# terra-render/Terra

Hardware: AMD Instinct MI355X
Metric: Msamples/s (higher is better)
Workload: dtype f32; 1 GPU; cornell_1080p_512spp; scene=cornell32, width=1920, height=1080, spp=512, bounces=8, integrator=simple, triangles=32, tree=auto, traversal=reference tree + leaf-box cull, tile=64, sample_split=8, parallelism=single

## Files before the change

### include/terra_amd.h

```cpp
#ifndef TERRA_AMD_H
#define TERRA_AMD_H

#include "Terra.h"

#ifdef __cplusplus
extern "C" {
#endif

typedef enum {
    kTerraAmdOk               = 0,
    kTerraAmdErrNoDevice      = -1,
    kTerraAmdErrNotCommitted  = -2,
    kTerraAmdErrUnsupported   = -3,
    kTerraAmdErrBadArgument   = -4,
    kTerraAmdErrLaunch        = -5
} TerraAmdStatus;

const char* terra_amd_last_error ( void );
void        terra_amd_clear_error ( void );
int         terra_amd_first_error ( char* buf, size_t capacity );
void        terra_amd_clear_first_error ( void );
size_t      terra_amd_thread_staging_bytes ( void );

int  terra_amd_init ( void );
void terra_amd_set_commit_timing ( int on );
int  terra_amd_set_build_threads ( int threads );
void terra_amd_set_azimuth_table ( int on );

int  terra_amd_device_count ( void );
int  terra_amd_set_device ( int device );
int  terra_amd_get_device ( void );

int  terra_amd_set_devices ( const int* devices, int count );
int  terra_amd_get_devices ( int* out, int capacity );
int  terra_amd_shard_owner ( size_t tile_index, int world );
int  terra_amd_render_multi ( const TerraCamera* camera, HTerraScene scene, const TerraFramebuffer* framebuffer,
                              size_t x, size_t y, size_t width, size_t height, size_t tile_size );
typedef struct {
    int      devices;
    int      device[16];
    int      replicas;
    uint64_t gathers;
    uint64_t last_gather_bytes;
    uint64_t process_collectives;
    int      rccl_version;
    int      communicator_ranks;
    char     rccl_library[64];
    uint64_t rehearsed_gathers;
} TerraAmdMultiInfo;
int  terra_amd_multi_info ( HTerraScene scene, TerraAmdMultiInfo* out );
int  terra_amd_debug_replicas_share_device ( int on );

int  terra_amd_scene_supported ( HTerraScene scene, char* why, size_t capacity );

void     terra_amd_set_frame_seed ( HTerraScene scene, uint64_t seed );
uint64_t terra_amd_get_frame_seed ( HTerraScene scene );

int  terra_amd_set_tree_mode ( HTerraScene scene, int mode );
int  terra_amd_get_tree_mode ( HTerraScene scene );
typedef struct {
    int   tree_mode;
    int   fast_tree;
    int   fast_tree_built_on_device;
    int   leaf_cull;
    int   lds_resident;
    float max_coordinate;
    float max_coordinate_allowed;
    char  note[256];
    int   last_call;
    float camera_limit;
} TerraAmdTraversalInfo;
typedef enum {
    kTerraAmdCallNone = 0,
    kTerraAmdCallReplica = 1,
    kTerraAmdCallLeafCull = 2,
    kTerraAmdCallFastTree = 3,
    kTerraAmdCallFastTreeReach = 4
} TerraAmdCallTraversal;
int  terra_amd_traversal_info ( HTerraScene scene, TerraAmdTraversalInfo* out );
int  terra_amd_set_tree_builder ( HTerraScene scene, int builder );
int  terra_amd_get_tree_builder ( HTerraScene scene );
int  terra_amd_debug_shrink_reference_boxes ( HTerraScene scene, float amount );
int  terra_amd_debug_pad_stack ( HTerraScene scene, int entries );
int  terra_amd_debug_fast_stack_lds ( HTerraScene scene, int entries );

int  terra_amd_set_sample_split ( HTerraScene scene, int split );
int  terra_amd_get_sample_split ( HTerraScene scene );
int  terra_amd_auto_sample_split ( size_t width, size_t height, size_t tile, int world, size_t spp, int job_ordered );

int  terra_amd_set_job_order ( HTerraScene scene, int on );
int  terra_amd_get_job_order ( HTerraScene scene );

int  terra_amd_set_empty_skip ( HTerraScene scene, int on );
int  terra_amd_get_empty_skip ( HTerraScene scene );
int  terra_amd_empty_skip_info ( HTerraScene scene, uint32_t out[2] );
int  terra_amd_empty_proof ( const float* cam_rot9, const float* cam_pos3, float tan_half_fov, float aspect, float jitter, uint32_t fb_w, uint32_t fb_h,
                             uint32_t x0, uint32_t y0, uint32_t x1, uint32_t y1, const float* tris9, size_t n_tris );

int  terra_amd_set_leaf_box_test ( HTerraScene scene, int on );
int  terra_amd_get_leaf_box_test ( HTerraScene scene );
int  terra_amd_leaf_box_info ( HTerraScene scene, uint32_t out[2] );
int  terra_amd_set_leaf_pairs ( HTerraScene scene, int on );
int  terra_amd_get_leaf_pairs ( HTerraScene scene );
int  terra_amd_leaf_pair_info ( HTerraScene scene, uint32_t out[2] );
int  terra_amd_set_leaf_nearest_first ( HTerraScene scene, int on );
int  terra_amd_get_leaf_nearest_first ( HTerraScene scene );

int  terra_amd_set_environment_lighting ( HTerraScene scene, int on );
int  terra_amd_get_environment_lighting ( HTerraScene scene );

// ... 283 lines not shown
TERRA_ABI_ASSERT ( sizeof ( TerraAmdAtlasTexel ) == 16 );
TERRA_ABI_ASSERT ( offsetof ( TerraAmdAtlasTexel, wb ) == 4 );
TERRA_ABI_ASSERT ( offsetof ( TerraAmdAtlasTexel, distance2 ) == 12 );
int terra_amd_atlas_points_device ( HTerraScene scene, const TerraAmdAtlas* atlas, const void* d_uvs, void* d_points, void* d_texels, void* stream );
int terra_amd_atlas_points ( HTerraScene scene, const TerraAmdAtlas* atlas, const float* uvs, TerraAmdPoint* points, TerraAmdAtlasTexel* texels );
int terra_amd_dilate_device ( void* d_data, int channels, void* d_valid, int width, int height, int passes, void* stream );
int terra_amd_dilate ( float* data, int channels, int* valid, int width, int height, int passes );

typedef struct {
    float c[9][3];
    int   cells;
} TerraAmdProbeSH;
typedef struct {
    float origin[3];
    int   nx;
    float spacing[3];
    int   ny, nz;
    int   reserved[3];
} TerraAmdProbeGrid;
TERRA_ABI_ASSERT ( sizeof ( TerraAmdProbeSH ) == 112 );
TERRA_ABI_ASSERT ( offsetof ( TerraAmdProbeSH, cells ) == 108 );
TERRA_ABI_ASSERT ( sizeof ( TerraAmdProbeGrid ) == 48 );
TERRA_ABI_ASSERT ( offsetof ( TerraAmdProbeGrid, nx ) == 12 );
TERRA_ABI_ASSERT ( offsetof ( TerraAmdProbeGrid, spacing ) == 16 );
TERRA_ABI_ASSERT ( offsetof ( TerraAmdProbeGrid, ny ) == 28 );
TERRA_ABI_ASSERT ( offsetof ( TerraAmdProbeGrid, nz ) == 32 );
TERRA_ABI_ASSERT ( offsetof ( TerraAmdProbeGrid, reserved ) == 36 );
int terra_amd_probe_rays_device ( const void* d_probes, size_t probes, int cells, const void* d_jitter, void* d_rays, void* stream );
int terra_amd_probe_rays ( const TerraAmdPoint* probes, size_t probes_n, int cells, const float* jitter, TerraAmdRay* rays );
int terra_amd_sh_project_device ( const void* d_results, const void* d_rays, size_t probes, int cells, int batch, void* d_sh, void* stream );
int terra_amd_sh_project ( const TerraFramebuffer* framebuffer, const TerraAmdRay* rays, size_t probes, int cells, int batch, TerraAmdProbeSH* sh );
int terra_amd_sh_irradiance_device ( const void* d_sh, size_t probes, const TerraAmdProbeGrid* grid, const void* d_points, const void* d_index, size_t n, void* d_out, void* stream );
int terra_amd_sh_irradiance ( const TerraAmdProbeSH* sh, size_t probes, const TerraAmdProbeGrid* grid, const TerraAmdPoint* points, const int* index, size_t n, float* out4 );
int terra_amd_probe_grid_points ( const TerraAmdProbeGrid* grid, TerraAmdPoint* out, int capacity );

int terra_amd_render_device_sharded ( const TerraCamera* camera, HTerraScene scene,
                                      void* d_pixels, void* d_results, size_t fb_width, size_t fb_height,
                                      size_t x, size_t y, size_t width, size_t height,
                                      size_t tile_size, int rank, int world,
                                      void* d_rand_calls, void* stream );

int    terra_amd_shard_tile_count ( size_t width, size_t height, size_t tile_size, int rank, int world );
size_t terra_amd_shard_packed_bytes ( size_t width, size_t height, size_t tile_size, int world );
int terra_amd_pack_tiles ( const void* d_pixels, const void* d_results, size_t fb_width, size_t fb_height,
                           size_t x, size_t y, size_t width, size_t height, size_t tile_size, int rank, int world,
                           void* d_packed, void* stream );
int terra_amd_unpack_tiles ( void* d_pixels, void* d_results, size_t fb_width, size_t fb_height,
                             size_t x, size_t y, size_t width, size_t height, size_t tile_size, int rank, int world,
                             const void* d_packed, void* stream );

int terra_amd_synchronize ( void* stream );

int terra_amd_time_render_device ( const TerraCamera* camera, HTerraScene scene,
                                   void* d_pixels, void* d_results, size_t fb_width, size_t fb_height,
                                   size_t x, size_t y, size_t width, size_t height,
                                   int launches, void* stream, float* ms_avg );


int terra_amd_unit_pcg ( const uint32_t* seeds, int nseeds, int n, float* out );
int terra_amd_unit_stream_keys ( uint64_t frame_seed, const uint64_t* pix, const uint64_t* samples_so_far, int n, uint64_t* out3 );
int terra_amd_unit_ray_aabb ( int n, const float* origins3, const float* dirs3, const float* boxes6, int* hit, float* tmin, float* tmax );
int terra_amd_unit_watertight ( int n, const float* origins3, const float* dirs3, const float* tris9, int* hit, float* out8 );
int terra_amd_unit_watertight_pair ( int n, const float* origins3, const float* dirs3, const float* quads12, int* hit2, float* depth2 );
int terra_amd_unit_moller_trumbore ( int n, const float* origins3, const float* dirs3, const float* tris9, int* hit, float* out4 );
int terra_amd_unit_bvh_traverse ( HTerraScene scene, int n, const float* origins3, const float* dirs3, int* found, uint32_t* prim, float* point3 );
int terra_amd_unit_bvh_traverse_fast ( HTerraScene scene, int n, const float* origins3, const float* dirs3, int* found, uint32_t* prim, float* point3, uint32_t* nodes_visited );
int terra_amd_unit_raycast ( HTerraScene scene, int n, const float* origins3, const float* dirs3, int* obj, int* tri, float* point3, float* surface47 );
int terra_amd_unit_trace ( HTerraScene scene, int n, const float* origins3, const float* dirs3, const uint64_t* stateB, const uint64_t* incB, float* radiance3, uint32_t* rand_calls );
int terra_amd_unit_bsdf ( int kind, int n, float* surfaces47, const float* e3, const float* wo3, float* wi3, float* pdf, float* f3 );
int terra_amd_unit_camera ( const TerraCamera* camera, size_t fb_width, size_t fb_height, int n, const uint32_t* xy2, float jitter, const float* r2, float* dirs3 );
int terra_amd_unit_tonemap ( int op, float gamma, int n, float* colors3 );
int terra_amd_unit_math ( int fn, int n, const float* x, const float* y, float* out );
int terra_amd_scene_lds_plan ( HTerraScene scene, uint32_t* out6 );
int terra_amd_unit_exact_div ( int op, const float* a, const float* b, const float* c, uint64_t first, uint64_t count, float denominator, float reciprocal, uint64_t seed,
                               uint32_t* helper_bits, uint32_t* plain_bits, uint64_t* mismatches, uint32_t* first_bad );
int terra_amd_unit_exact_sqrt ( int op, const float* a, const float* b, const float* c, uint64_t first, uint64_t count, uint64_t seed,
                                uint32_t* helper_bits, uint32_t* plain_bits, uint64_t* mismatches, uint32_t* first_bad );
int terra_amd_unit_half_outward ( const double* x, int n, int up, uint16_t* out );
int terra_amd_unit_stratified ( const uint32_t* seeds, int nseeds, int strata, int samples_per_stratum, int n, float* out2 );
int terra_amd_unit_halton ( int first, int n, float* out2 );
int terra_amd_unit_distribution_1d ( const float* f, size_t n, const float* e, int m, float* x, float* pdf, uint32_t* idx, float* cdf_out, float* integral_out );
int terra_amd_unit_distribution_2d ( const float* f, size_t nx, size_t ny, const float* e12, int m, float* xy2, float* pdf, float* marginal_cdf_out );
int terra_amd_unit_distribution_2d_pdf ( const float* f, size_t nx, size_t ny, const float* xy2, int m, float* pdf );
int terra_amd_unit_texture_sample ( const TerraTexture* texture, int n, const float* uv2, float* out3 );
int terra_amd_unit_texture_latlong ( const TerraTexture* texture, int n, const float* dir3, float* out3 );

#ifdef __cplusplus
}
#endif
#endif
```

### terra_amd/csrc/dev_math.h

```cpp
#pragma once
#include <stdint.h>
#include <math.h>

#if defined(__HIPCC__)
#define TDM_FN __host__ __device__ inline
#else
#define TDM_FN static inline
#endif

TDM_FN uint32_t tdm_bits ( float f ) { return __builtin_bit_cast ( uint32_t, f ); }
TDM_FN float    tdm_float ( uint32_t u ) { return __builtin_bit_cast ( float, u ); }
TDM_FN uint32_t tdm_top12 ( float f ) { return ( tdm_bits ( f ) >> 20 ) & 0x7ffu; }

TDM_FN float tdm_sincos_poly ( double x, double x2, int n, bool flip ) {
    if ( ( n & 1 ) == 0 ) {
        const double S1 = -0x1.555545995a603p-3, S2 = 0x1.1107605230bc4p-7, S3 = -0x1.994eb3774cf24p-13;
        double x3 = x * x2;
        double t = S2 + x2 * S3;
        double x7 = x3 * x2;
        double s = x + x3 * S1;
        return ( float ) ( s + x7 * t );
    }
    double k = flip ? -1.0 : 1.0;
    const double C0 = 0x1p0, C1 = -0x1.ffffffd0c621cp-2, C2 = 0x1.55553e1068f19p-5, C3 = -0x1.6c087e89a359dp-10, C4 = 0x1.99343027bf8c3p-16;
    double x4 = x2 * x2;
    double t2 = ( k * C3 ) + x2 * ( k * C4 );
    double t1 = ( k * C0 ) + x2 * ( k * C1 );
    double x6 = x4 * x2;
    double c = t1 + x4 * ( k * C2 );
    return ( float ) ( c + x6 * t2 );
}

TDM_FN float tdm_sincosf ( float y, int shift ) {
    double x = y;
    if ( tdm_top12 ( y ) < tdm_top12 ( 0x1.921FB6p-1f ) ) {
        if ( tdm_top12 ( y ) < tdm_top12 ( 0x1p-12f ) ) {
            return shift ? 1.0f : y;
        }
        return tdm_sincos_poly ( x, x * x, shift, false );
    }
    double r = x * 0x1.45F306DC9C883p+23;
    int n = ( ( int32_t ) r + 0x800000 ) >> 24;
    x = x - ( double ) n * 0x1.921FB54442D18p0;
    int m = n + shift;
    int q = m & 3;
    double sgn = ( q == 1 || q == 2 ) ? -1.0 : 1.0;
    return tdm_sincos_poly ( x * sgn, x * x, m, ( m & 2 ) != 0 );
}
TDM_FN void tdm_sincosf_pair ( float y, float& s, float& c ) {
    double x = y;
    if ( tdm_top12 ( y ) < tdm_top12 ( 0x1.921FB6p-1f ) ) {
        if ( tdm_top12 ( y ) < tdm_top12 ( 0x1p-12f ) ) { s = y; c = 1.0f; return; }
        double x2 = x * x;
        s = tdm_sincos_poly ( x, x2, 0, false );
        c = tdm_sincos_poly ( x, x2, 1, false );
        return;
    }
    double r = x * 0x1.45F306DC9C883p+23;
    int n = ( ( int32_t ) r + 0x800000 ) >> 24;
    x = x - ( double ) n * 0x1.921FB54442D18p0;
    double x2 = x * x;
    int qs = n & 3, m = n + 1, qc = m & 3;
    double sgn_s = ( qs == 1 || qs == 2 ) ? -1.0 : 1.0;
    double sgn_c = ( qc == 1 || qc == 2 ) ? -1.0 : 1.0;
    s = tdm_sincos_poly ( x * sgn_s, x2, n, ( n & 2 ) != 0 );
    c = tdm_sincos_poly ( x * sgn_c, x2, m, ( m & 2 ) != 0 );
}
TDM_FN float tdm_sinf ( float y ) { return tdm_sincosf ( y, 0 ); }
TDM_FN float tdm_cosf ( float y ) { return tdm_sincosf ( y, 1 ); }

TDM_FN uint64_t tdm_bits64 ( double f ) { return __builtin_bit_cast ( uint64_t, f ); }
TDM_FN double   tdm_double ( uint64_t u ) { return __builtin_bit_cast ( double, u ); }

TDM_FN double tdm_powf_log2 ( uint32_t ix ) {
    static const double T[16][2] = {
        { 0x1.661ec79f8f3bep+0, -0x1.efec65b963019p-2 }, { 0x1.571ed4aaf883dp+0, -0x1.b0b6832d4fca4p-2 },
        { 0x1.49539f0f010bp+0, -0x1.7418b0a1fb77bp-2 }, { 0x1.3c995b0b80385p+0, -0x1.39de91a6dcf7bp-2 },
        { 0x1.30d190c8864a5p+0, -0x1.01d9bf3f2b631p-2 }, { 0x1.25e227b0b8eap+0, -0x1.97c1d1b3b7afp-3 },
        { 0x1.1bb4a4a1a343fp+0, -0x1.2f9e393af3c9fp-3 }, { 0x1.12358f08ae5bap+0, -0x1.960cbbf788d5cp-4 },
        { 0x1.0953f419900a7p+0, -0x1.a6f9db6475fcep-5 }, { 0x1p+0, 0x0p+0 },
        { 0x1.e608cfd9a47acp-1, 0x1.338ca9f24f53dp-4 }, { 0x1.ca4b31f026aap-1, 0x1.476a9543891bap-3 },
        { 0x1.b2036576afce6p-1, 0x1.e840b4ac4e4d2p-3 }, { 0x1.9c2d163a1aa2dp-1, 0x1.40645f0c6651cp-2 },
        { 0x1.886e6037841edp-1, 0x1.88e9c2c1b9ff8p-2 }, { 0x1.767dcf5534862p-1, 0x1.ce0a44eb17bccp-2 } };
    const double A0 = 0x1.27616c9496e0bp-2, A1 = -0x1.71969a075c67ap-2, A2 = 0x1.ec70a6ca7baddp-2, A3 = -0x1.7154748bef6c8p-1, A4 = 0x1.71547652ab82bp0;
    uint32_t tmp = ix - 0x3f330000u;
    int i = ( int ) ( ( tmp >> 19 ) % 16u );
    uint32_t top = tmp & 0xff800000u;
    uint32_t iz = ix - top;
    int k = ( int32_t ) top >> 23;
    double z = ( double ) tdm_float ( iz );
    double r = z * T[i][0] - 1.0;
    double y0 = T[i][1] + ( double ) k;
    double r2 = r * r;
    double y = A0 * r + A1;
    double p = A2 * r + A3;
    double r4 = r2 * r2;
    double q = A4 * r + y0;
    q = p * r2 + q;
    return y * r4 + q;
}
TDM_FN float tdm_powf_exp2 ( double xd, uint32_t sign_bias ) {
    static const uint64_t T[32] = {
        0x3ff0000000000000ull, 0x3fefd9b0d3158574ull, 0x3fefb5586cf9890full, 0x3fef9301d0125b51ull,
        0x3fef72b83c7d517bull, 0x3fef54873168b9aaull, 0x3fef387a6e756238ull, 0x3fef1e9df51fdee1ull,
        0x3fef06fe0a31b715ull, 0x3feef1a7373aa9cbull, 0x3feedea64c123422ull, 0x3feece086061892dull,
        0x3feebfdad5362a27ull, 0x3feeb42b569d4f82ull, 0x3feeab07dd485429ull, 0x3feea47eb03a5585ull,
        0x3feea09e667f3bcdull, 0x3fee9f75e8ec5f74ull, 0x3feea11473eb0187ull, 0x3feea589994cce13ull,
        0x3feeace5422aa0dbull, 0x3feeb737b0cdc5e5ull, 0x3feec49182a3f090ull, 0x3feed503b23e255dull,
        0x3feee89f995ad3adull, 0x3feeff76f2fb5e47ull, 0x3fef199bdd85529cull, 0x3fef3720dcef9069ull,
        0x3fef5818dcfba487ull, 0x3fef7c97337b9b5full, 0x3fefa4afa2a490daull, 0x3fefd0765b6e4540ull };
    const double C0 = 0x1.c6af84b912394p-5, C1 = 0x1.ebfce50fac4f3p-3, C2 = 0x1.62e42ff0c52d6p-1, SHIFT = 0x1.8p+47;
    double kd = xd + SHIFT;
    uint64_t ki = tdm_bits64 ( kd );
    kd = kd - SHIFT;
    double r = xd - kd;
    uint64_t t = T[ki % 32u];
    uint64_t ski = ki + sign_bias;
    t += ski << 47;
    double s = tdm_double ( t );
    double z = C0 * r + C1;
    double r2 = r * r;
    double y = C2 * r + 1.0;
    y = z * r2 + y;
    y = y * s;
    return ( float ) y;
}
TDM_FN int tdm_powf_checkint ( uint32_t iy ) {
    int e = ( int ) ( iy >> 23 & 0xff );
    if ( e < 0x7f ) return 0;
    if ( e > 0x7f + 23 ) return 2;
    if ( iy & ( ( 1u << ( 0x7f + 23 - e ) ) - 1 ) ) return 0;
    if ( iy & ( 1u << ( 0x7f + 23 - e ) ) ) return 1;
    return 2;
}
TDM_FN bool tdm_zeroinfnan ( uint32_t ix ) { return 2 * ix - 1 >= 2u * 0x7f800000u - 1; }

TDM_FN float tdm_powf ( float x, float y ) {
    uint32_t sign_bias = 0;
    uint32_t ix = tdm_bits ( x ), iy = tdm_bits ( y );
    if ( ix - 0x00800000u >= 0x7f800000u - 0x00800000u || tdm_zeroinfnan ( iy ) ) {
        if ( tdm_zeroinfnan ( iy ) ) {
            if ( 2 * iy == 0 ) return 1.0f;
            if ( ix == 0x3f800000u ) return 1.0f;
            if ( 2 * ix > 2u * 0x7f800000u || 2 * iy > 2u * 0x7f800000u ) return x + y;
            if ( 2 * ix == 2 * 0x3f800000u ) return 1.0f;
            if ( ( 2 * ix < 2 * 0x3f800000u ) == ! ( iy & 0x80000000u ) ) return 0.0f;
            return y * y;
        }
        if ( tdm_zeroinfnan ( ix ) ) {
            float x2 = x * x;
            if ( ( ix & 0x80000000u ) && tdm_powf_checkint ( iy ) == 1 ) x2 = -x2;
            return ( iy & 0x80000000u ) ? 1 / x2 : x2;
// ... 118 lines not shown
```

### terra_amd/csrc/integrators_device.h

```cpp
#pragma once
#include "shading_device.h"

TD float randf ( Pcg32& b, Counters& c, int count ) { if ( count == 2 ) ++c.rand_calls; return trng_b_float ( b ); }
TD uint32_t randf_bits ( Pcg32& b, Counters& c, int count ) { if ( count == 2 ) ++c.rand_calls; return trng_b_bits ( b ); }

TD float triangle_area ( V3 a, V3 b, V3 cc ) { return length ( cross ( b - a, cc - a ) ) / 2; }

struct LightSample { uint32_t light_object; uint32_t tri_in_object; uint32_t tri; float pick_pdf; V3 pos, norm; };

template <int COUNT, int MODE = 0>
TD LightSample draw_light_sample ( const DevScene& sc, Pcg32& rb, Counters& c, const Tracer* T = nullptr ) {
    LightSample ls;
    float e = ( float ) ( ( double ) randf ( rb, c, COUNT ) - 1e-4 );
    double xl = ( double ) e * ( double ) sc.n_lights;
    uint32_t li = xl < 0 ? 0u : ( uint32_t ) xl;
    ls.pick_pdf = 1.f / ( float ) sc.lights_triangles_count;
    DevLight l = ( MODE == 1 && T ) ? T->l_lights[li] : sc.lights[li];
    float e_t = randf ( rb, c, COUNT );
    uint32_t k = ( uint32_t ) ( e_t * ( float ) l.tri_count );
    if ( k >= l.tri_count ) k = l.tri_count - 1;
    ls.light_object = l.object; ls.tri_in_object = k; ls.tri = l.first_tri + k;
    float e1 = randf ( rb, c, COUNT ), e2 = randf ( rb, c, COUNT );
    const float4* tris = ( MODE == 1 && T ) ? reinterpret_cast<const float4*> ( T->l_tris ) : reinterpret_cast<const float4*> ( sc.tris );
    const float4* props = ( MODE == 1 && T ) ? T->l_props : reinterpret_cast<const float4*> ( sc.props );
// ... 46 lines not shown
    float p_row = 0.f, p_col = 0.f; uint32_t row = 0, col = 0;
    DevDistribution1D rows = { sc.env_row_f, sc.env_row_cdf, sc.env_ny, sc.env_integral, sc.env_monotone };
    const float sv = distribution_sample ( rows, e1, &p_row, &row );
    if ( sv == FLT_MAX ) return zero;
    DevDistribution1D cols = { sc.env_f + ( size_t ) sc.env_nx * row, sc.env_cdf + ( size_t ) sc.env_nx * row, sc.env_nx, sc.env_row_f[row], sc.env_monotone };
    const float su = distribution_sample ( cols, e2, &p_col, &col );
    if ( su == FLT_MAX ) return zero;
    const float theta = sv * TERRA_PI_F, phi = su * ( 2 * TERRA_PI_F ) - TERRA_PI_F;
    const float st = tdm_sinf ( theta ), ct = tdm_cosf ( theta ), sp = tdm_sinf ( phi ), cp = tdm_cosf ( phi );
    if ( ! ( st > 0.f ) ) return zero;
    const V3 wi = v3 ( st * cp, ct, st * sp );
    const float cosine = dot ( wi, sf.normal );
    if ( ! ( cosine > 0.f ) ) return zero;
    const float pdf = ( p_row * p_col ) * ( ( float ) sc.env_nx * ( float ) sc.env_ny ) / ( 2 * TERRA_PI_F * TERRA_PI_F * st );
    if ( ! ( pdf > 0.f ) ) return zero;
    Surface lsf;
    Ray r = surface_ray ( sf, p, wi );
    RaycastResult h = scene_raycast<COUNT, MODE, KINDS> ( T, r, lsf, c );
    if ( h.hit ) return zero;
    const V3 L = texture_read ( sc.textures[sc.env_tex], col, row );
    const V3 f = bsdf_eval<KINDS> ( sf, wi, wo );
    if constexpr ( MIS && ( KINDS & TERRA_KIND_ENV_MIS ) != 0 ) if ( !bsdf_is_singular<KINDS> ( sf ) ) {
        const float b = bsdf_pdf<KINDS> ( sf, wi, wo ), bpdf = b > 0.f ? b : 0.f;
        const float r = bpdf / pdf, weight = 1.f / ( 1.f + r * r );
        return had ( L, f ) * ( cosine * weight / pdf );
    }
    return had ( L, f ) * ( cosine / pdf );
}

template <int COUNT, int MODE, int KINDS>
TD V3 integrate_direct ( const Tracer& T, Surface& sf, V3 p, V3 wo, V3 throughput, uint32_t bounce, Pcg32& rb, Counters& c ) {
    const DevScene& sc = T.sc;
    V3 Lo = v3 ( 0, 0, 0 );
    if ( bounce == 0 && dot ( wo, sf.normal ) > 0 ) Lo = Lo + sf.emissive;
    LightSample ls = draw_light_sample<COUNT, MODE> ( sc, rb, c, &T );
    V3 p_to_light = ls.pos - p;
    V3 wi = normalize ( p_to_light );
    Surface lsf;
    Ray r = surface_ray ( sf, p, wi );
    RaycastResult h = scene_raycast<COUNT, MODE, KINDS> ( T, r, lsf, c );
    if ( h.hit && h.object == ls.light_object && h.tri_in_object == ls.tri_in_object ) {
        float cosv = dot ( neg ( wi ), ls.norm );
        if ( cosv > 0 ) {
            V3 f = bsdf_eval<KINDS> ( sf, wi, wo );
            float pdf = dot ( p_to_light, p_to_light ) / fabsf ( cosv * T.l_area[h.tri] );
            V3 Ld = had ( lsf.emissive, f );
            Ld = Ld * ( dot ( wi, sf.normal ) / ( pdf * ls.pick_pdf ) );
            Lo = Lo + Ld;
        }
    }
    if constexpr ( ( KINDS & TERRA_KIND_SAMPLER ) != 0 ) { if ( env_sampling_active ( sc ) ) Lo = Lo + environment_light_sample<COUNT, MODE, KINDS> ( T, sf, p, wo, rb, c ); }
    return had ( Lo, throughput );
}

struct DirectPending { V3 vis, hid; uint32_t expected; };
template <int COUNT, int KINDS, int MODE = 0>
TD DirectPending direct_prepare ( const Tracer& T, Surface& sf, V3 p, V3 wo, V3 throughput, uint32_t bounce, Pcg32& rb, Counters& c, Ray& shadow_ray ) {
    const DevScene& sc = T.sc;
    V3 Lo = v3 ( 0, 0, 0 );
    if ( bounce == 0 && dot ( wo, sf.normal ) > 0 ) Lo = Lo + sf.emissive;
    LightSample ls = draw_light_sample<COUNT, MODE> ( sc, rb, c, &T );
    V3 p_to_light = ls.pos - p;
    V3 wi = normalize ( p_to_light );
    shadow_ray = surface_ray ( sf, p, wi );
    DirectPending d;
    d.hid = had ( Lo, throughput ); d.vis = d.hid; d.expected = ls.tri;
    float cosv = dot ( neg ( wi ), ls.norm );
    if ( cosv > 0 ) {
        V3 f = bsdf_eval<KINDS> ( sf, wi, wo );
        float pdf = dot ( p_to_light, p_to_light ) / fabsf ( cosv * T.l_area[ls.tri] );
        V3 Ld = had ( v3p ( T.l_mats[ls.light_object].emissive ), f );
        Ld = Ld * ( dot ( wi, sf.normal ) / ( pdf * ls.pick_pdf ) );
        d.vis = had ( Lo + Ld, throughput );
    }
    return d;
}

struct MisPending { V3 a_vis, a_hid; uint32_t expected; V3 f2; float bpdf2, cos2; V3 p; uint32_t light_object; V3 t_before; };
template <int COUNT, int KINDS, int MODE = 0>
TD MisPending mis_prepare ( const Tracer& T, Surface& sf, V3 p, V3 wo, V3 throughput, uint32_t bounce, Pcg32& rb, Counters& c, Ray& ray_a, V3& dir_b ) {
    const DevScene& sc = T.sc;
    V3 Lo = v3 ( 0, 0, 0 );
    if ( bounce == 0 && dot ( wo, sf.normal ) > 0 ) Lo = Lo + sf.emissive;
    float e1 = randf ( rb, c, COUNT ), e2 = randf ( rb, c, COUNT ), e3 = randf ( rb, c, COUNT );
    V3 bsdf_dir = bsdf_sample<KINDS> ( sf, e1, e2, e3, wo, azimuth_fetch ( sc.sincos24, e2 ) );
    LightSample ls = draw_light_sample<COUNT, MODE> ( sc, rb, c, &T );
    MisPending m;
    m.a_hid = Lo; m.a_vis = Lo; m.expected = ls.tri; m.p = p; m.light_object = ls.light_object; m.t_before = throughput;
    {
        V3 p_to_light = ls.pos - p;
        V3 wi = normalize ( p_to_light );
        ray_a = surface_ray ( sf, p, wi );
        float cosv = dot ( ls.norm, neg ( wi ) );
        if ( cosv > 0 ) {
            float bpdf = bsdf_pdf<KINDS> ( sf, wi, wo );
            float lpdf = dot ( p_to_light, p_to_light ) / fabsf ( cosv * T.l_area[ls.tri] );
            float weight = ( lpdf * lpdf ) / ( lpdf * lpdf + bpdf * bpdf );
            if ( lpdf != 0 ) {
                V3 f = bsdf_eval<KINDS> ( sf, wi, wo );
                V3 L = had ( v3p ( T.l_mats[ls.light_object].emissive ), f );
                L = L * ( dot ( wi, sf.normal ) * weight / ( lpdf * ls.pick_pdf ) );
                m.a_vis = Lo + L;
            }
        }
    }
    dir_b = bsdf_dir;
    m.f2 = bsdf_eval<KINDS> ( sf, bsdf_dir, wo );
    m.bpdf2 = bsdf_pdf<KINDS> ( sf, bsdf_dir, wo );
    m.cos2 = dot ( bsdf_dir, sf.normal );
    return m;
}
template <int MODE>
TD V3 mis_finish_b ( const Tracer& T, const MisPending& m, V3 Lo, bool hit, uint32_t hit_object, uint32_t hit_tri, V3 hit_point, const Surface& lsf, V3 wi ) {
    if ( hit && hit_object == m.light_object ) {
        float NoW = dot ( lsf.normal, neg ( wi ) );
        if ( NoW > 0 ) {
            V3 dl = m.p - hit_point;
            float dist = dot ( dl, dl );
            const float4* tris = MODE == 1 ? reinterpret_cast<const float4*> ( T.l_tris ) : reinterpret_cast<const float4*> ( T.sc.tris );
            V3 ta, tb, tc; tri_vertices ( tris, hit_tri, ta, tb, tc );
            float area = triangle_area ( ta, tb, tc );
            float lpdf = dist / ( NoW * area );
            float weight = ( m.bpdf2 * m.bpdf2 ) / ( lpdf * lpdf + m.bpdf2 * m.bpdf2 );
            if ( m.bpdf2 != 0 ) {
                V3 L = had ( lsf.emissive, m.f2 );
                L = L * ( m.cos2 * weight / m.bpdf2 );
                Lo = Lo + L;
            }
        }
    }
    return had ( Lo, m.t_before );
}

template <int COUNT, int MODE, int KINDS, bool DEBUG_WEIGHTS>
TD V3 integrate_mis ( const Tracer& T, Surface& sf, V3 p, V3 wo, V3 throughput, uint32_t bounce, Pcg32& rb, Counters& c ) {
    const DevScene& sc = T.sc;
    V3 Lo = v3 ( 0, 0, 0 );
    if ( DEBUG_WEIGHTS ) { if ( bounce != 0 ) return Lo; }
    else if ( bounce == 0 && dot ( wo, sf.normal ) > 0 ) Lo = Lo + sf.emissive;
    float e1 = randf ( rb, c, COUNT ), e2 = randf ( rb, c, COUNT ), e3 = randf ( rb, c, COUNT );
    V3 bsdf_dir = bsdf_sample<KINDS> ( sf, e1, e2, e3, wo, azimuth_fetch ( sc.sincos24, e2 ) );
    LightSample ls = draw_light_sample<COUNT, MODE> ( sc, rb, c, &T );
    {
        V3 p_to_light = ls.pos - p;
        V3 wi = normalize ( p_to_light );
        Surface lsf;
        Ray r = surface_ray ( sf, p, wi );
        RaycastResult h = scene_raycast<COUNT, MODE, KINDS> ( T, r, lsf, c );
        if ( h.hit && h.object == ls.light_object && h.tri_in_object == ls.tri_in_object ) {
            float cosv = dot ( ls.norm, neg ( wi ) );
            if ( cosv > 0 ) {
                float bpdf = bsdf_pdf<KINDS> ( sf, wi, wo );
                float lpdf = dot ( p_to_light, p_to_light ) / fabsf ( cosv * T.l_area[h.tri] );
                if ( DEBUG_WEIGHTS ) {
                    float weight = ( bpdf * bpdf ) / ( lpdf * lpdf + bpdf * bpdf );
                    Lo = Lo + v3 ( 0, 0, weight );
                } else {
                    float weight = ( lpdf * lpdf ) / ( lpdf * lpdf + bpdf * bpdf );
                    if ( lpdf != 0 ) {
                        V3 f = bsdf_eval<KINDS> ( sf, wi, wo );
                        V3 L = had ( lsf.emissive, f );
                        L = L * ( dot ( wi, sf.normal ) * weight / ( lpdf * ls.pick_pdf ) );
                        Lo = Lo + L;
                    }
                }
            }
        }
    }
    {
        V3 wi = bsdf_dir;
        V3 f = bsdf_eval<KINDS> ( sf, wi, wo );
        float bpdf = bsdf_pdf<KINDS> ( sf, wi, wo );
        V3 light_wo = neg ( wi );
        Surface lsf;
        Ray r = surface_ray ( sf, p, wi );
        RaycastResult h = scene_raycast<COUNT, MODE, KINDS> ( T, r, lsf, c );
        if ( h.hit && h.object == ls.light_object ) {
            float NoW = dot ( lsf.normal, light_wo );
            if ( NoW > 0 ) {
                V3 dl = p - h.point;
                float dist = dot ( dl, dl );
                const float4* tris = reinterpret_cast<const float4*> ( sc.tris );
                V3 ta, tb, tc; tri_vertices ( tris, h.tri, ta, tb, tc );
                float area = triangle_area ( ta, tb, tc );
                float lpdf = dist / ( NoW * area );
                float weight = ( bpdf * bpdf ) / ( lpdf * lpdf + bpdf * bpdf );
                if ( DEBUG_WEIGHTS ) {
                    Lo = Lo + v3 ( weight, 0, 0 );
                } else if ( bpdf != 0 ) {
                    V3 L = had ( lsf.emissive, f );
                    L = L * ( dot ( wi, sf.normal ) * weight / bpdf );
                    Lo = Lo + L;
                }
            }
        }
        if constexpr ( ( KINDS & TERRA_KIND_ENV_MIS ) != 0 && !DEBUG_WEIGHTS ) {
            if ( !h.hit && bpdf > 0.f ) {
                uint32_t col, row; float st;
                environment_texel ( sc, wi, col, row, st );
                const float epdf = ( !bsdf_is_singular<KINDS> ( sf ) && dot ( wi, sf.normal ) > 0 ) ? environment_texel_pdf ( sc, col, row, st ) : 0.f;
                const float r = epdf / bpdf, weight = 1.f / ( 1.f + r * r );
                V3 L = had ( texture_read ( sc.textures[sc.env_tex], col, row ), f );
                L = L * ( dot ( wi, sf.normal ) * weight / bpdf );
                Lo = Lo + L;
            }
        }
    }
    if constexpr ( ( KINDS & TERRA_KIND_SAMPLER ) != 0 && !DEBUG_WEIGHTS ) { if ( env_sampling_active ( sc ) ) Lo = Lo + environment_light_sample<COUNT, MODE, KINDS, true> ( T, sf, p, wo, rb, c ); }
    return had ( Lo, throughput );
}

TD V3 integrate_debug_normals ( const Surface& sf, uint32_t bounce ) {
    if ( bounce != 0 ) return v3 ( 0, 0, 0 );
    V3 n = sf.normal;
    V3 pp = v3 ( sel_min ( n.x > 0 ? n.x : 0.f, 1.f ), sel_min ( n.y > 0 ? n.y : 0.f, 1.f ), sel_min ( n.z > 0 ? n.z : 0.f, 1.f ) );
    V3 nn = v3 ( sel_min ( n.x > -1 ? n.x : -1.f, 0.f ), sel_min ( n.y > -1 ? n.y : -1.f, 0.f ), sel_min ( n.z > -1 ? n.z : -1.f, 0.f ) );
    nn = nn * -1.f;
    V3 col = v3 ( 0, 0, 0 );
    col = col + v3 ( 1, 0, 0 ) * pp.x;
    col = col + v3 ( 0, 1, 0 ) * pp.y;
    col = col + v3 ( 0, 0, 1 ) * pp.z;
    col = col + v3 ( 0, 1, 1 ) * nn.x;
    col = col + v3 ( 1, 0, 1 ) * nn.y;
    col = col + v3 ( 1, 1, 0 ) * nn.z;
    return col;
}

template <int INTEGRATOR, int COUNT, int MODE, int KINDS>
TD V3 integrate ( const Tracer& T, const Ray& ray, Surface& sf, V3 p, V3 wo, V3 throughput, uint32_t bounce, Pcg32& rb, Counters& c ) {
    if ( INTEGRATOR == 0 ) {
        if ( dot ( wo, sf.normal ) > 0 ) return had ( sf.emissive, throughput );
        return v3 ( 0, 0, 0 );
    } else if ( INTEGRATOR == 1 ) {
        return integrate_direct<COUNT, MODE, KINDS> ( T, sf, p, wo, throughput, bounce, rb, c );
    } else if ( INTEGRATOR == 2 ) {
        return integrate_mis<COUNT, MODE, KINDS, false> ( T, sf, p, wo, throughput, bounce, rb, c );
    } else if ( INTEGRATOR == 3 ) {
        return bounce != 0 ? v3 ( 0, 0, 0 ) : v3 ( 1, 1, 1 );
    } else if ( INTEGRATOR == 4 ) {
        if ( bounce != 0 ) return v3 ( 0, 0, 0 );
        float d = length ( ray.o - p ) / 500.f;
        return v3 ( d, d, d );
    } else if ( INTEGRATOR == 5 ) {
        return integrate_debug_normals ( sf, bounce );
    } else {
        return integrate_mis<COUNT, MODE, KINDS, true> ( T, sf, p, wo, throughput, bounce, rb, c );
    }
}

template <int COUNT, bool INDEX>
TD PathDraws path_draw ( const float2* sincos24, Pcg32& rb, Counters& c ) {
    PathDraws d;
    if constexpr ( INDEX ) {
        d.e0 = randf ( rb, c, COUNT );
        const uint32_t k1 = randf_bits ( rb, c, COUNT );
        d.e1 = trng_b_from_bits ( k1 );
        d.e2 = randf ( rb, c, COUNT );
        d.az = azimuth_fetch_index ( sincos24, k1 );
        d.e3 = randf ( rb, c, COUNT );
    } else {
        d.e0 = randf ( rb, c, COUNT ); d.e1 = randf ( rb, c, COUNT ); d.e2 = randf ( rb, c, COUNT );
        d.az = azimuth_fetch ( sincos24, d.e1 );
        d.e3 = randf ( rb, c, COUNT );
    }
    return d;
}
template <int KINDS>
TD bool path_continue ( Surface& sf, V3 wo, V3& throughput, uint32_t& bounce, uint32_t max_bounces, const PathDraws& d, V3& wi ) {
    wi = bsdf_sample<KINDS> ( sf, d.e0, d.e1, d.e2, wo, d.az );
    float pdf = sel_max ( bsdf_pdf<KINDS> ( sf, wi, wo ), ( float ) 1e-4 );
    V3 f = bsdf_eval<KINDS> ( sf, wi, wo ) * rcp_exact ( pdf );
    throughput = had ( throughput, f );
    throughput = throughput * dot ( sf.normal, wi );
    float pr = sel_max ( throughput.x, sel_max ( throughput.y, throughput.z ) );
    if ( d.e3 > pr ) return false;
        throughput = throughput * roulette_scale ( pr );
    ++bounce;
    return bounce <= max_bounces;
}
struct SamplerPair { float u0, u1; bool on; };
TD SamplerPair sampler_pair_none() { SamplerPair s; s.u0 = s.u1 = 0.f; s.on = false; return s; }
TD void path_apply_sampler ( PathDraws& d, const SamplerPair& sp, uint32_t bounce ) {
    if ( sp.on && bounce == 0 ) { d.e0 = sp.u0; d.e1 = sp.u1; d.az = azimuth_none(); }
}
TD SamplerPair sampler_pair_draw ( uint32_t mode, uint32_t strata, uint64_t n, Pcg32& stream_a ) {
    SamplerPair s = sampler_pair_none();
    if ( mode == 1 ) { s.u0 = radical_inverse ( 3, n ); s.u1 = radical_inverse ( 2, n ); s.on = true; }
    else if ( mode == 2 && strata > 0 ) {
        const uint64_t cap = ( uint64_t ) strata * strata * 16ull, m = n % cap, stratum = m / 16ull;
        const float stratum_size = 1.f / ( float ) strata;
        s.u0 = sd_below_one ( ( ( float ) ( uint32_t ) ( stratum % strata ) + trng_a_float ( stream_a ) ) * stratum_size );
        s.u1 = sd_below_one ( ( ( float ) ( uint32_t ) ( stratum / strata ) + trng_a_float ( stream_a ) ) * stratum_size );
        s.on = true;
    }
    return s;
}
template <int COUNT, int KINDS>
TD bool path_continue ( const DevScene& sc, Surface& sf, V3 wo, V3& throughput, uint32_t& bounce, uint32_t max_bounces, Pcg32& rb, Counters& c, V3& wi, const SamplerPair& sp = sampler_pair_none() ) {
    PathDraws d = path_draw<COUNT> ( sc.sincos24, rb, c );
    if ( KINDS & TERRA_KIND_SAMPLER ) path_apply_sampler ( d, sp, bounce );
    return path_continue<KINDS> ( sf, wo, throughput, bounce, max_bounces, d, wi );
}

template <int INTEGRATOR, int COUNT, int MODE, int KINDS>
TD V3 trace_path ( const Tracer& T, Ray ray, uint32_t bounces, Pcg32& rb, Counters& c ) {
    V3 Lo = v3 ( 0, 0, 0 ), throughput = v3 ( 1, 1, 1 );
    for ( uint32_t bounce = 0; bounce <= bounces; ++bounce ) {
        Surface sf;
        RaycastResult h = scene_raycast<COUNT, MODE, KINDS> ( T, ray, sf, c );
        if ( !h.hit ) {
            if ( ( KINDS & TERRA_KIND_ENV ) && T.sc.env_mode && !env_reaches_by_samples<INTEGRATOR, KINDS> ( T.sc, bounce ) ) { throughput = had ( throughput, environment_eval ( T.sc, ray.d ) ); Lo = Lo + throughput; }
            break;
        }
        V3 wo = neg ( ray.d );
        Lo = Lo + integrate<INTEGRATOR, COUNT, MODE, KINDS> ( T, ray, sf, h.point, wo, throughput, bounce, rb, c );
        V3 wi;
        uint32_t next_bounce = bounce;
        if ( !path_continue<COUNT, KINDS> ( T.sc, sf, wo, throughput, next_bounce, bounces, rb, c, wi ) ) break;
        ray = surface_ray ( sf, h.point, wi );
    }
    return Lo;
}

TD V3 uncharted2 ( V3 x ) {
    const float A = 0.15f, B = 0.5f, C = 0.1f, D = 0.2f, E = 0.02f, F = 0.3f;
    V3 r;
    r.x = ( ( x.x * ( A * x.x + C * B ) + D * E ) / ( x.x * ( A * x.x + B ) + D * F ) ) - E / F;
    r.y = ( ( x.y * ( A * x.y + C * B ) + D * E ) / ( x.y * ( A * x.y + B ) + D * F ) ) - E / F;
    r.z = ( ( x.z * ( A * x.z + C * B ) + D * E ) / ( x.z * ( A * x.z + B ) + D * F ) ) - E / F;
    return r;
}
TD V3 powv ( V3 c, float e ) { return v3 ( tdm_powf ( c.x, e ), tdm_powf ( c.y, e ), tdm_powf ( c.z, e ) ); }
TD V3 tonemap ( V3 c, int op, float gamma ) {
    switch ( op ) {
        case 1: c = powv ( c, 1.f / gamma ); break;
        case 2:
            c.x = c.x / ( 1.f + c.x ); c.y = c.y / ( 1.f + c.y ); c.z = c.z / ( 1.f + c.z );
            c = powv ( c, 1.f / gamma ); break;
        case 3: {
            V3 x = v3 ( sel_max ( 0.f, c.x - 0.004f ), sel_max ( 0.f, c.y - 0.004f ), sel_max ( 0.f, c.z - 0.004f ) );
            c.x = ( x.x * ( 6.2f * x.x + 0.5f ) ) / ( x.x * ( 6.2f * x.x + 1.7f ) + 0.06f );
            c.y = ( x.y * ( 6.2f * x.y + 0.5f ) ) / ( x.y * ( 6.2f * x.y + 1.7f ) + 0.06f );
            c.x = ( x.z * ( 6.2f * x.z + 0.5f ) ) / ( x.z * ( 6.2f * x.z + 1.7f ) + 0.06f );
            break;
        }
        case 4: {
            V3 ws = uncharted2 ( v3 ( 11.2f, 11.2f, 11.2f ) );
// ... 10 lines not shown
```

### terra_amd/csrc/kernels.h

```cpp
#pragma once
#include <hip/hip_runtime.h>
#include "dev_types.h"

hipError_t terra_launch_render ( const DevRenderParams& p, hipStream_t stream );
hipError_t terra_launch_job_streams ( const DevRenderParams& p, hipStream_t stream );
hipError_t terra_launch_block_order ( const DevRenderParams& p, uint32_t* cls, hipStream_t stream, const DevLaunchMask* mask, bool classify, bool prove );
hipError_t terra_launch_render_mode0 ( const DevRenderParams& p, size_t lds, hipStream_t stream );
hipError_t terra_launch_render_mode1 ( const DevRenderParams& p, size_t lds, hipStream_t stream );
hipError_t terra_launch_render_mode2 ( const DevRenderParams& p, size_t lds, hipStream_t stream );
hipError_t terra_launch_render_mode3 ( const DevRenderParams& p, size_t lds, hipStream_t stream );
hipError_t terra_launch_render_rays ( const DevRenderParams& p, const void* rays, hipStream_t stream );
hipError_t terra_launch_render_rays_mode0 ( const DevRayRenderParams& p, size_t lds, hipStream_t stream );
hipError_t terra_launch_render_rays_mode1 ( const DevRayRenderParams& p, size_t lds, hipStream_t stream );
hipError_t terra_launch_render_rays_mode2 ( const DevRayRenderParams& p, size_t lds, hipStream_t stream );
hipError_t terra_launch_render_rays_mode3 ( const DevRayRenderParams& p, size_t lds, hipStream_t stream );
hipError_t terra_launch_render_lens ( const DevRenderParams& p, const DevLens& lens, hipStream_t stream );
hipError_t terra_launch_render_lens_mode0 ( const DevLensRenderParams& p, size_t lds, hipStream_t stream );
hipError_t terra_launch_render_lens_mode1 ( const DevLensRenderParams& p, size_t lds, hipStream_t stream );
hipError_t terra_launch_render_lens_mode2 ( const DevLensRenderParams& p, size_t lds, hipStream_t stream );
hipError_t terra_launch_render_lens_mode3 ( const DevLensRenderParams& p, size_t lds, hipStream_t stream );
hipError_t terra_launch_render_points ( const DevRenderParams& p, const void* points, const DevPointSampling& sampling, hipStream_t stream );
hipError_t terra_launch_render_points_mode0 ( const DevPointRenderParams& p, size_t lds, hipStream_t stream );
hipError_t terra_launch_render_points_mode1 ( const DevPointRenderParams& p, size_t lds, hipStream_t stream );
hipError_t terra_launch_render_points_mode2 ( const DevPointRenderParams& p, size_t lds, hipStream_t stream );
hipError_t terra_launch_render_points_mode3 ( const DevPointRenderParams& p, size_t lds, hipStream_t stream );
hipError_t terra_launch_resolve ( const DevRenderParams& p, hipStream_t stream, const uint32_t* live_blocks );
hipError_t terra_launch_tiles ( bool pack, float* pixels, void* results, uint32_t fb_w, uint32_t x, uint32_t y, uint32_t w, uint32_t h,
                                uint32_t tile, uint32_t rank, uint32_t world, float* packed, hipStream_t stream );

hipError_t terra_launch_aov ( DevRenderParams p, void* aov, hipStream_t stream, const uint32_t* mask );
hipError_t terra_launch_aov_rays ( DevRenderParams p, const void* rays, void* aov, hipStream_t stream );
hipError_t terra_launch_aov_lens ( DevRenderParams p, const DevLens& lens, void* aov, hipStream_t stream );
hipError_t terra_launch_aov_points ( DevRenderParams p, const void* points, const DevPointSampling& sampling, void* aov, hipStream_t stream );

hipError_t terra_launch_denoise ( const void* results, const void* aov, uint32_t fb_w, uint32_t x, uint32_t y, uint32_t w, uint32_t h, int iterations,
                                  float exposure, int op, float gamma, float* radiance, float* pixels, hipStream_t stream );
hipError_t terra_launch_denoise_variance ( const void* results, const void* aov, const void* moments, uint32_t fb_w, uint32_t x, uint32_t y, uint32_t w, uint32_t h, int iterations,
                                           float exposure, int op, float gamma, float* radiance, float* pixels, hipStream_t stream );

hipError_t terra_launch_moments_accumulate ( const void* results, void* moments, uint32_t fb_w, uint32_t x, uint32_t y, uint32_t w, uint32_t h, hipStream_t stream );
hipError_t terra_launch_tile_error ( const void* moments, uint32_t fb_w, uint32_t x, uint32_t y, uint32_t w, uint32_t h, uint32_t tile, float* errors, hipStream_t stream );
hipError_t terra_launch_error_mask ( const float* errors, uint32_t w, uint32_t h, uint32_t tile, float target, int all, uint32_t* mask, hipStream_t stream );

struct DevTemporalParams {
    float cam_pos[3], cam_rot[9], tan_half_fov, aspect;
    float prev_pos[3], prev_rot[9], prev_tan_half_fov;
    uint32_t fb_w, fb_h, x, y, w, h;
    float alpha, depth_tolerance, normal_cos, max_length;
    uint32_t same_camera;
    float inv_fb_w, inv_fb_h;
};
hipError_t terra_launch_temporal_reproject ( const DevTemporalParams& p, const void* results, const void* aov, const void* history_in, void* history_out,
                                             void* out_results, void* out_moments, hipStream_t stream );

struct DevQueryParams {
    DevScene scene;
    uint32_t fast, stack_depth, leaf_cap, spill_cap, leaf_cull;
    float    origin_limit;
};
hipError_t terra_launch_query ( DevQueryParams p, const void* rays, size_t n, void* out, bool anyhit, hipStream_t stream );

struct DevAtlas {
    uint32_t width, height;
    float    uv_scale[2], uv_offset[2], margin;
};
hipError_t terra_launch_atlas_points ( const DevScene& sc, const DevAtlas& atlas, const float* uvs, void* points, void* texels, hipStream_t stream );
hipError_t terra_launch_dilate ( float* data, int channels, int* valid, uint32_t width, uint32_t height, int passes, hipStream_t stream );

struct DevProbeGrid {
    int32_t on;
    int32_t count[3];
    float   origin[3], spacing[3];
};
hipError_t terra_launch_probe_rays ( const void* probes, uint32_t count, uint32_t cells, const float* jitter, void* rays, hipStream_t stream );
hipError_t terra_launch_sh_project ( const void* results, const void* rays, uint32_t count, uint32_t cells, int batch, void* sh, hipStream_t stream );
hipError_t terra_launch_sh_irradiance ( const void* sh, uint32_t probes, const DevProbeGrid& grid, const void* points, const int* index, uint32_t n, void* out, hipStream_t stream );

hipError_t terra_fill_sincos24 ( float2* table, hipStream_t stream );

hipError_t terra_unit_pcg ( const uint32_t* seeds, int nseeds, int n, float* out );
hipError_t terra_unit_stream_keys ( uint64_t frame_seed, const uint64_t* pix, const uint64_t* k, int n, uint64_t* out3 );
hipError_t terra_unit_ray_aabb ( int n, const float* o, const float* d, const float* boxes, int* hit, float* tmin, float* tmax );
hipError_t terra_unit_watertight ( int n, const float* o, const float* d, const float* tris, int* hit, float* out8 );
hipError_t terra_unit_watertight_pair ( int n, const float* o, const float* d, const float* quads, int* hit, float* depth );
hipError_t terra_unit_moller_trumbore ( int n, const float* o, const float* d, const float* tris, int* hit, float* out4 );
hipError_t terra_unit_bvh_traverse ( const DevScene& sc, int n, const float* o, const float* d, int* found, uint32_t* prim, float* point );
hipError_t terra_unit_bvh_traverse_fast ( const DevScene& sc, int n, const float* o, const float* d, int* found, uint32_t* prim, float* point, uint32_t* nodes_visited );
hipError_t terra_unit_raycast ( const DevScene& sc, int n, const float* o, const float* d, int* obj, int* tri, float* point, float* surface47 );
hipError_t terra_unit_trace ( const DevScene& sc, int integrator, uint32_t bounces, int n, const float* o, const float* d,
                              const uint64_t* stateB, const uint64_t* incB, float* radiance, uint32_t* rand_calls );
hipError_t terra_unit_bsdf ( int kind, int n, float* surfaces47, const float* e3, const float* wo3, float* wi3, float* pdf, float* f3 );
hipError_t terra_unit_camera ( const DevRenderParams& p, int n, const uint32_t* xy2, const float* r2, float* dirs3 );
hipError_t terra_unit_lens_rays ( const DevRenderParams& p, const DevLens& lens, int n, const uint32_t* xy2, const float* r4, float* rays8 );
hipError_t terra_unit_point_rays ( const DevPointSampling& sampling, int n, const float* points8, const float* g2, float* rays8 );
hipError_t terra_unit_tonemap ( int op, float gamma, int n, float* colors3 );
hipError_t terra_unit_math ( int fn, int n, const float* x, const float* y, float* out );
hipError_t terra_unit_exact_div ( int op, const float* a, const float* b, const float* c, uint64_t first, uint64_t count, float D, float R, uint64_t seed,
                                  uint32_t* helper_bits, uint32_t* plain_bits, unsigned long long* mismatches, uint32_t* first_bad );
hipError_t terra_unit_exact_sqrt ( int op, const float* a, const float* b, const float* c, uint64_t first, uint64_t count, uint64_t seed,
                                   uint32_t* helper_bits, uint32_t* plain_bits, unsigned long long* mismatches, uint32_t* first_bad );
hipError_t terra_unit_texture_sample ( const DevTexture* t, int n, const float* uv2, float* out3 );
hipError_t terra_unit_texture_latlong ( const DevTexture* t, int n, const float* dir3, float* out3 );
hipError_t terra_unit_stratified ( const uint32_t* seeds, int nseeds, int strata, int samples, int n, float* out2 );
hipError_t terra_unit_halton ( int first, int n, float* out2 );
hipError_t terra_unit_distribution_1d ( const float* f, uint32_t n, float* cdf, float* integral, uint32_t* monotone, const float* e, int m, float* x, float* pdf, uint32_t* idx );
hipError_t terra_unit_distribution_2d ( const float* f, uint32_t nx, uint32_t ny, float* cdf, float* integrals, float* mcdf, uint32_t* monotone, const float* e12, int m, float* xy2, float* pdf );
hipError_t terra_unit_distribution_2d_pdf ( const float* f, uint32_t nx, uint32_t ny, float* cdf, float* integrals, float* mcdf, uint32_t* monotone, const float* xy2, int m, float* pdf );
hipError_t terra_build_fast_tree_device ( const DevTri* tris, const uint32_t* rank, uint32_t n, float extra_margin, DevNode* out_nodes, DevTri* out_tris, uint32_t* n_nodes_out, int* max_stack_out, hipStream_t stream );
```

### terra_amd/csrc/render_kernels.hip

```cpp
#include <hip/hip_runtime.h>
#include "trace_device.h"
#include "kernels.h"
#include "launch_plan.h"
#include "empty_proof.h"

#ifdef TERRA_TU
#define TERRA_TU_HAS(k) ( TERRA_TU == ( k ) )
#define TERRA_TU_MODE(k) ( TERRA_TU == ( k ) || TERRA_TU == ( k ) + 4 || TERRA_TU == ( k ) + 8 || TERRA_TU == ( k ) + 12 )
#else
#define TERRA_TU_HAS(k) ( !TERRA_RAY_SOURCE )
#define TERRA_TU_MODE(k) 1
#endif
#if TERRA_RAY_SOURCE == 3
typedef DevPointRenderParams RenderKernelParams;
#elif TERRA_RAY_SOURCE == 2
typedef DevLensRenderParams RenderKernelParams;
#elif TERRA_RAY_SOURCE == 1
typedef DevRayRenderParams RenderKernelParams;
#else
typedef DevRenderParams RenderKernelParams;
#endif

struct DevResult { float acc[3]; int samples; };

// ... 489 lines not shown
                        cont = path_continue<COUNT, KINDS> ( T.sc, sf, wo, throughput, bounce, p.bounces, rs.b, c, cont_d, sp );
                        cont_o = surface_origin ( sf, point );
                        ro = ray_a.o; rd = ray_a.d; job = 1; start = true;
                    } else {
                        if ( ( KINDS & TERRA_KIND_ENV ) && T.sc.env_mode ) { throughput = had ( throughput, environment_eval ( T.sc, ray.d ) ); Lo = Lo + throughput; }
                        deposit ( acc_lds, Lo ); have_ray = false;
                    }
                }
                if ( !start ) {
                    if ( jb.s == p.chunk_spp ) { TERRA_JOB_NEXT(); if ( jb.exhausted ) done = true; }
                    if ( jb.s != p.chunk_spp ) {
                        float r1 = trng_a_float ( rs.a ), r2 = trng_a_float ( rs.a );
                        TERRA_PRIMARY_RAY ( ro, rd, r1, r2 );
                        if constexpr ( ( KINDS & TERRA_KIND_SAMPLER ) != 0 ) sp = sampler_pair_draw ( p.sampler_mode, p.sampler_strata, ( uint64_t ) jb.base + jb.s, rs.a );
                        TERRA_LENS_RAY ( ro, rd, r1, r2 );
                        Lo = v3 ( 0, 0, 0 ); throughput = v3 ( 1, 1, 1 ); bounce = 0; ++jb.s; job = 0; start = true;
                    }
                }
                if ( start ) { ray = make_ray ( ro, rd ); lane_traversal_start<COUNT, MODE> ( T, ray, lt, c ); have_ray = true; }
            }
            if ( !lane_traversal_run<COUNT, MODE> ( T, ray, lt, c ) && __all ( done ) ) break;
        }
    } else if constexpr ( terra_decoupled_direct ( INTEGRATOR, MODE, KINDS ) ) {
        LaneTraversal lt = lane_traversal_idle ( T, ray );
        bool done = false, have_ray = false, shadow = false, cont = false;
        DirectPending pend; pend.vis = pend.hid = v3 ( 0, 0, 0 ); pend.expected = 0;
        V3 cont_o = v3 ( 0, 0, 0 ), cont_d = v3 ( 0, 0, 1 );
        for ( ;; ) {
            if ( !lt.traversing && !done && ! ( have_ray && lane_traversal_recheck<MODE> ( T, ray, lt ) ) ) {
                bool start = false;
                V3 ro = v3 ( 0, 0, 0 ), rd = v3 ( 0, 0, 1 );
                if ( have_ray && shadow ) {
                    const uint32_t tri_s = ( MODE == 2 && COUNT == 0 && lt.best.tri == TERRA_TRI_EXPECTED ) ? pend.expected : hit_soup_index<MODE> ( T, lt.best.tri );
                    if ( tri_s != 0xffffffffu ) {
                        if ( COUNT ) ++c.hits;
                        if ( COUNT == 2 ) { const float4 t0 = reinterpret_cast<const float4*> ( T.sc.tris ) [3 * tri_s]; c.attr_fetches += T.sc.mats[__float_as_uint ( t0.w )].attributes_count + 1; }
                    }
                    Lo = Lo + ( tri_s == pend.expected ? pend.vis : pend.hid );
                    shadow = false;
                    if ( cont ) { ro = cont_o; rd = cont_d; start = true; }
                    else { deposit ( acc_lds, Lo ); have_ray = false; }
                } else if ( have_ray ) {
                    if ( lt.best.tri != 0xffffffffu ) {
                        Surface sf;
                        V3 point = shade_surface<COUNT, MODE, KINDS> ( T, ray, lt.best, sf, c );
                        V3 wo = neg ( ray.d );
                        Ray shadow_ray;
                        pend = direct_prepare<COUNT, KINDS, MODE> ( T, sf, point, wo, throughput, bounce, rs.b, c, shadow_ray );
                        cont = path_continue<COUNT, KINDS> ( T.sc, sf, wo, throughput, bounce, p.bounces, rs.b, c, cont_d, sp );
                        cont_o = surface_origin ( sf, point );
                        ro = shadow_ray.o; rd = shadow_ray.d; shadow = true; start = true;
                    } else {
                        if ( ( KINDS & TERRA_KIND_ENV ) && T.sc.env_mode ) { throughput = had ( throughput, environment_eval ( T.sc, ray.d ) ); Lo = Lo + throughput; }
                        deposit ( acc_lds, Lo ); have_ray = false;
                    }
                }
                if ( !start ) {
                    if ( jb.s == p.chunk_spp ) { TERRA_JOB_NEXT(); if ( jb.exhausted ) done = true; }
                    if ( jb.s != p.chunk_spp ) {
                        float r1 = trng_a_float ( rs.a ), r2 = trng_a_float ( rs.a );
                        TERRA_PRIMARY_RAY ( ro, rd, r1, r2 );
                        if constexpr ( ( KINDS & TERRA_KIND_SAMPLER ) != 0 ) sp = sampler_pair_draw ( p.sampler_mode, p.sampler_strata, ( uint64_t ) jb.base + jb.s, rs.a );
                        TERRA_LENS_RAY ( ro, rd, r1, r2 );
                        Lo = v3 ( 0, 0, 0 ); throughput = v3 ( 1, 1, 1 ); bounce = 0; ++jb.s; start = true;
                    }
                }
                if ( start ) {
                    ray = make_ray ( ro, rd ); lane_traversal_start<COUNT, MODE> ( T, ray, lt, c ); have_ray = true;
                    if ( shadow ) lane_traversal_expect<COUNT, MODE> ( T, ray, lt, pend.expected );
                }
            }
            if ( !lane_traversal_run<COUNT, MODE> ( T, ray, lt, c ) && __all ( done ) ) break;
        }
    } else if constexpr ( terra_decoupled ( INTEGRATOR, MODE ) ) {
        LaneTraversal lt = lane_traversal_idle ( T, ray );
        bool done = false, have_ray = false;
        for ( ;; ) {
            if ( !lt.traversing && !done && ! ( have_ray && lane_traversal_recheck<MODE> ( T, ray, lt ) ) ) {
                bool next = false;
                V3 ro = v3 ( 0, 0, 0 ), rd = v3 ( 0, 0, 1 );
                if ( have_ray ) {
                    if ( lt.best.tri != 0xffffffffu ) {
                        Surface sf;
                        PathDraws pd = path_draw<COUNT> ( T.sc.sincos24, rs.b, c );
                        if constexpr ( ( KINDS & TERRA_KIND_SAMPLER ) != 0 ) path_apply_sampler ( pd, sp, bounce );
                        V3 point = shade_surface<COUNT, MODE, KINDS> ( T, ray, lt.best, sf, c );
                        V3 wo = neg ( ray.d ), wi;
                        Lo = Lo + integrate<INTEGRATOR, COUNT, MODE, KINDS> ( T, ray, sf, point, wo, throughput, bounce, rs.b, c );
                        next = path_continue<KINDS> ( sf, wo, throughput, bounce, p.bounces, pd, wi );
                        if ( next ) { ro = surface_origin ( sf, point ); rd = wi; }
                    } else if ( ( KINDS & TERRA_KIND_ENV ) && T.sc.env_mode ) {
                        throughput = had ( throughput, environment_eval ( T.sc, ray.d ) );
                        Lo = Lo + throughput;
                    }
                    if ( !next ) { deposit ( acc_lds, Lo ); have_ray = false; }
                }
                if ( !next ) {
                    if ( jb.s == p.chunk_spp ) { TERRA_JOB_NEXT(); if ( jb.exhausted ) done = true; }
                    if ( jb.s != p.chunk_spp ) {
                        float r1 = trng_a_float ( rs.a ), r2 = trng_a_float ( rs.a );
                        TERRA_PRIMARY_RAY ( ro, rd, r1, r2 );
                        if constexpr ( ( KINDS & TERRA_KIND_SAMPLER ) != 0 ) sp = sampler_pair_draw ( p.sampler_mode, p.sampler_strata, ( uint64_t ) jb.base + jb.s, rs.a );
                        TERRA_LENS_RAY ( ro, rd, r1, r2 );
                        Lo = v3 ( 0, 0, 0 ); throughput = v3 ( 1, 1, 1 ); bounce = 0; ++jb.s; next = true;
                    }
                }
                if ( next ) { ray = make_ray ( ro, rd ); lane_traversal_start<COUNT, MODE> ( T, ray, lt, c ); have_ray = true; }
            }
            if ( !lane_traversal_run<COUNT, MODE> ( T, ray, lt, c ) && __all ( done ) ) break;
        }
    } else {
    bool alive = false;
    V3 ro = v3 ( 0, 0, 0 ), rd = v3 ( 0, 0, 1 );
    constexpr bool LO_LDS = MODE == 1;
    float* lo_lds = acc_lds + 6 * 256;
    auto lo_reset = [&] () { if ( LO_LDS ) { lo_lds[0] = 0.f; lo_lds[256] = 0.f; lo_lds[512] = 0.f; } else Lo = v3 ( 0, 0, 0 ); };
    auto lo_add = [&] ( V3 t ) {
        if ( LO_LDS ) { if ( t.x != 0.f || t.y != 0.f || t.z != 0.f ) { lo_lds[0] = lo_lds[0] + t.x; lo_lds[256] = lo_lds[256] + t.y; lo_lds[512] = lo_lds[512] + t.z; } }
        else Lo = Lo + t;
    };
    auto lo_deposit = [&] () { if ( LO_LDS ) deposit ( acc_lds, v3 ( lo_lds[0], lo_lds[256], lo_lds[512] ) ); else deposit ( acc_lds, Lo ); };
#ifndef TERRA_REGEN_MIN
#define TERRA_REGEN_MIN 1
#endif
    while ( true ) {
        const bool any_alive = __any ( alive );
        if ( !alive && ( TERRA_REGEN_MIN <= 1 || !any_alive || __popcll ( __ballot ( !alive ) ) >= TERRA_REGEN_MIN ) ) {
            if ( jb.s == p.chunk_spp && ( TERRA_JOB_FETCH_MIN <= 1 || !any_alive || __popcll ( __ballot ( jb.s == p.chunk_spp ) ) >= TERRA_JOB_FETCH_MIN ) ) TERRA_JOB_NEXT();
            if ( jb.exhausted ) break;
            if ( jb.s != p.chunk_spp ) {
                PS_WAVE ( c, kPsCamIter ); PS_LANE ( c, kPsCamLanes );
                float r1 = trng_a_float ( rs.a ), r2 = trng_a_float ( rs.a );
                TERRA_PRIMARY_RAY ( ro, rd, r1, r2 );
                if constexpr ( ( KINDS & TERRA_KIND_SAMPLER ) != 0 ) sp = sampler_pair_draw ( p.sampler_mode, p.sampler_strata, ( uint64_t ) jb.base + jb.s, rs.a );
                TERRA_LENS_RAY ( ro, rd, r1, r2 );
                lo_reset(); throughput = v3 ( 1, 1, 1 ); bounce = 0; alive = true; ++jb.s;
            }
        }
        if ( alive ) {
            bool guarded = false;
            if constexpr ( ray_start_masks_for ( COUNT, MODE, KINDS ) ) ray = make_ray_guarded ( ro, rd, guarded ); else
            ray = make_ray ( ro, rd );
            Surface sf;
            PS_WAVE ( c, kPsRayIter ); PS_LANE ( c, kPsRayLanes );
            constexpr bool pre_draw = !TERRA_IS_LIGHT ( INTEGRATOR );
            PathDraws pd;
            RaycastResult h = scene_raycast<COUNT, MODE, KINDS> ( T, ray, sf, c, pre_draw ? &pd : nullptr, pre_draw ? &rs.b : nullptr, guarded );
            bool end = !h.hit;
            if ( h.hit ) {
                PS_WAVE ( c, kPsShadeIter ); PS_LANE ( c, kPsShadeLanes );
                V3 wo = neg ( ray.d ), wi;
                constexpr bool SPLIT_DIRECT = INTEGRATOR == 1 && ( KINDS & ( TERRA_KIND_TEX | TERRA_KIND_SAMPLER ) ) == 0;
                if constexpr ( SPLIT_DIRECT ) {
                    Ray shadow_ray;
                    const DirectPending pend = direct_prepare<COUNT, KINDS, MODE> ( T, sf, h.point, wo, throughput, bounce, rs.b, c, shadow_ray );
                    pd = path_draw<COUNT, ray_start_masks_for ( COUNT, MODE, KINDS )> ( T.sc.sincos24, rs.b, c );
                    end = !path_continue<KINDS> ( sf, wo, throughput, bounce, p.bounces, pd, wi );
                    if ( !end ) { ro = surface_origin ( sf, h.point ); rd = wi; }
                    const uint32_t tri = scene_raycast_triangle<COUNT, MODE, ray_start_masks_for ( COUNT, MODE, KINDS )> ( T, shadow_ray, c, pend.expected );
                    lo_add ( tri == pend.expected ? pend.vis : pend.hid );
                } else if constexpr ( INTEGRATOR == 2 && ( KINDS & ( TERRA_KIND_TEX | TERRA_KIND_SAMPLER ) ) == 0 ) {
                    Ray ray_a; V3 b_d;
                    const MisPending pend = mis_prepare<COUNT, KINDS, MODE> ( T, sf, h.point, wo, throughput, bounce, rs.b, c, ray_a, b_d );
                    const V3 next_o = surface_origin ( sf, h.point );
                    end = !path_continue<COUNT, KINDS> ( T.sc, sf, wo, throughput, bounce, p.bounces, rs.b, c, wi, sp );
                    if ( !end ) { ro = next_o; rd = wi; }
                    const uint32_t tri_a = scene_raycast_triangle<COUNT, MODE, ray_start_masks_for ( COUNT, MODE, KINDS )> ( T, ray_a, c, pend.expected );
                    const V3 lo_a = tri_a == pend.expected ? pend.a_vis : pend.a_hid;
                    Surface lsf;
                    const RaycastResult hb = scene_raycast<COUNT, MODE, KINDS> ( T, make_ray ( next_o, b_d ), lsf, c );
                    lo_add ( mis_finish_b<MODE> ( T, pend, lo_a, hb.hit, hb.object, hb.tri, hb.point, lsf, b_d ) );
                } else {
                lo_add ( integrate<INTEGRATOR, COUNT, MODE, KINDS> ( T, ray, sf, h.point, wo, throughput, bounce, rs.b, c ) );
                if ( !pre_draw ) pd = path_draw<COUNT, ray_start_masks_for ( COUNT, MODE, KINDS )> ( T.sc.sincos24, rs.b, c );
                if constexpr ( ( KINDS & TERRA_KIND_SAMPLER ) != 0 ) path_apply_sampler ( pd, sp, bounce );
                end = !path_continue<KINDS> ( sf, wo, throughput, bounce, p.bounces, pd, wi );
                if ( !end ) { ro = surface_origin ( sf, h.point ); rd = wi; }
                }
            } else if ( ( KINDS & TERRA_KIND_ENV ) && T.sc.env_mode && !env_reaches_by_samples<INTEGRATOR, KINDS> ( T.sc, bounce ) ) {
                throughput = had ( throughput, environment_eval ( T.sc, ray.d ) );
                lo_add ( throughput );
            }
            if ( end ) { lo_deposit(); alive = false; }
        }
    }
    }

    if ( COUNT ) wave_flush_counters ( c, p.counters );
    if ( COUNT == 2 && p.leaf_cull ) {
        unsigned long long x = c.tri_culled;
        for ( int off = 32; off > 0; off >>= 1 ) x += __shfl_xor ( x, off, 64 );
        if ( ( threadIdx.x & 63 ) == 0 && x ) atomicAdd ( &p.counters[kCtrTriCulled], x );
    }
#if TERRA_PHASE_STATS
    for ( int k = 0; k < 16; ++k ) {
        unsigned long long x = c.ps[k];
        for ( int off = 32; off > 0; off >>= 1 ) x += __shfl_xor ( x, off, 64 );
        if ( ( threadIdx.x & 63 ) == 0 && x ) atomicAdd ( &p.counters[kCtrDbg0 + k], x );
    }
#endif
}


static uint32_t resident_blocks ( const void* fn, size_t lds ) {
    struct Key { const void* fn; size_t lds; int dev; uint32_t blocks; };
    static thread_local Key cache[8]; static thread_local int used = 0;
    int dev = 0; ( void ) hipGetDevice ( &dev );
    for ( int i = 0; i < used; ++i ) if ( cache[i].fn == fn && cache[i].lds == lds && cache[i].dev == dev ) return cache[i].blocks;
    int per_cu = 0;
    if ( hipOccupancyMaxActiveBlocksPerMultiprocessor ( &per_cu, fn, 256, lds ) != hipSuccess || per_cu < 1 ) { ( void ) hipGetLastError(); per_cu = 1; }
    const uint32_t blocks = ( uint32_t ) per_cu * terra_cu_count();
    Key& k = cache[used < 8 ? used++ : 7]; k.fn = fn; k.lds = lds; k.dev = dev; k.blocks = blocks;
    return blocks;
}
template <int I, int COUNT, int MODE, int KINDS>
static hipError_t launch_instance ( const RenderKernelParams& p, size_t lds, hipStream_t stream ) {
    auto fn = terra_render_kernel<I, COUNT, MODE, KINDS>;
    if ( lds > ( size_t ) 64 * 1024 ) {
        if ( lds > terra_lds_block_limit() ) return hipErrorInvalidValue;
        static thread_local size_t opted[8] = { 0 }; int dev = 0; ( void ) hipGetDevice ( &dev );
        if ( opted[dev & 7] < lds ) {
            const hipError_t e = hipFuncSetAttribute ( reinterpret_cast<const void*> ( fn ), hipFuncAttributeMaxDynamicSharedMemorySize, ( int ) lds );
            if ( e != hipSuccess ) return e;
            opted[dev & 7] = lds;
        }
    }
    uint32_t grid = p.job_blocks;
    if ( p.job_queue ) { const uint32_t cap = resident_blocks ( reinterpret_cast<const void*> ( fn ), lds ); if ( grid > cap ) grid = cap; }
    if ( MODE >= 2 && p.spill_cap && ( !p.stack_spill || terra_spill_bytes ( grid, p.spill_cap ) > terra_fast_spill_bytes ( p ) ) ) return hipErrorInvalidValue;
    hipLaunchKernelGGL ( fn, dim3 ( grid ), dim3 ( 256 ), lds, stream, p );
    return hipGetLastError();
}
template <int I, int MODE, int KINDS>
static hipError_t launch_kinds ( const RenderKernelParams& p, size_t lds, hipStream_t stream ) {
    if ( p.count_level == 0 ) return launch_instance<I, 0, MODE, KINDS> ( p, lds, stream );
    return launch_instance<I, 2, MODE, KINDS> ( p, lds, stream );
}
template <int I, int MODE>
static hipError_t launch_mode ( const RenderKernelParams& p, size_t lds, hipStream_t stream ) {
    if ( p.bsdf_kinds == 1 ) return launch_kinds<I, MODE, 1> ( p, lds, stream );
    if ( ( p.bsdf_kinds & ~3u ) == 0 ) return launch_kinds<I, MODE, 3> ( p, lds, stream );
    if constexpr ( I <= 2 && MODE != 0 ) {
        if ( ( p.bsdf_kinds & ~15u ) == 0 ) return launch_kinds<I, MODE, 15> ( p, lds, stream );
    }
    if ( ( p.bsdf_kinds & TERRA_KIND_SAMPLER ) == 0 ) return launch_kinds<I, MODE, TERRA_KINDS_ALL & ~TERRA_KIND_SAMPLER> ( p, lds, stream );
    if constexpr ( I == 2 ) {
        if ( p.bsdf_kinds & TERRA_KIND_ENV_MIS ) return launch_kinds<I, MODE, TERRA_KINDS_ALL | TERRA_KIND_ENV_MIS> ( p, lds, stream );
    }
    return launch_kinds<I, MODE, TERRA_KINDS_ALL> ( p, lds, stream );
}
template <int MODE>
static hipError_t launch_integrator ( const RenderKernelParams& p, size_t lds, hipStream_t stream ) {
    switch ( p.integrator ) {
        case 0: return launch_mode<0, MODE> ( p, lds, stream );
        case 1: return launch_mode<1, MODE> ( p, lds, stream );
        case 2: return launch_mode<2, MODE> ( p, lds, stream );
        case 3: return launch_mode<3, MODE> ( p, lds, stream );
// ... 252 lines not shown
```

### terra_amd/csrc/scene_host.cpp

```cpp
#include <hip/hip_runtime.h>
#include <algorithm>
#include <cfloat>
#include <cmath>
#include <cstdarg>
#include <cstdio>
#include <cstdlib>
#include <cstring>
#include <mutex>
#include <string>
#include <unordered_set>
#include <atomic>
#include <chrono>
#include <vector>

#include "../../include/terra_amd.h"
#include "../../include/TerraPresets.h"
#include "dev_types.h"
#include "kernels.h"
#include "launch_plan.h"
#include "empty_proof.h"
#include "tree_build.h"
#include "multi_gpu.h"

static thread_local std::string g_last_error;
// ... 205 lines not shown
extern "C" void terra_framebuffer_destroy ( TerraFramebuffer* fb ) {
    if ( !fb ) return;
    fb_free ( fb->results ); fb_free ( fb->pixels );
    fb->results = nullptr; fb->pixels = nullptr;
}

struct HostLight { uint32_t object; float area; TerraFloat3 power; };

#ifndef TERRA_REACH_CAMERA_FACTOR
#define TERRA_REACH_CAMERA_FACTOR 8.f
#endif
#define TERRA_REACH_MAX_COORD 1e6f
#define TERRA_CULL_MAX_COORD 13.0f
#ifndef TERRA_SCRATCH_MAX_GB
#define TERRA_SCRATCH_MAX_GB 64
#endif
#define TERRA_FAST_STACK_MAX 2048
struct TreeChoice {
    bool use_fast = false;
    bool fast_on_device = false;
    bool cull_ok = false;
    bool reach = false;
    bool reach_cull = false;
    float reach_limit = 0.f;
    float coord_max = 0.f;
    uint32_t fast_nodes = 0; int fast_max_stack = 1;
    std::string note;
    bool resident = false;
    float reach_margin = 0.f, fast_extra = 0.f, fast_scale = 1.f;
};
static float shortcut_limit ( const TreeChoice& c ) { return ( c.reach || c.reach_cull ) ? c.reach_limit : TERRA_CULL_MAX_COORD; }
enum { kSecNodes, kSecTris, kSecProps, kSecMats, kSecLights, kSecArea, kSecFastBin, kSecFastWide, kSecFastTris, kSecReplay, kSecLeafParent, kSecLeafMask, kSecLeafBoxes, kSecLeafPairs, kSecTexDesc, kSecTextures };
struct Section { size_t offset = 0, bytes = 0; const void* host = nullptr; size_t host_bytes = 0; };
struct BlobLayout { std::vector<Section> sec; std::vector<DevTexture> tdesc; size_t total = 0; };
struct Staging {
    int device = -1; hipStream_t stream = nullptr; void* d_pixels = nullptr; void* d_results = nullptr; size_t cap_px = 0;
    int prepare ( int dev, size_t npx ) {
        int current = -1;
        if ( hipGetDevice ( &current ) != hipSuccess || current != dev ) HIP_TRY ( hipSetDevice ( dev ), kTerraAmdErrNoDevice );
        if ( device != dev ) { if ( device >= 0 ) { release(); HIP_TRY ( hipSetDevice ( dev ), kTerraAmdErrNoDevice ); } device = dev; }
        if ( !stream ) HIP_TRY ( hipStreamCreateWithFlags ( &stream, hipStreamNonBlocking ), kTerraAmdErrNoDevice );
        if ( cap_px < npx ) {
            if ( d_pixels ) ( void ) hipFree ( d_pixels );
            if ( d_results ) ( void ) hipFree ( d_results );
            d_pixels = d_results = nullptr; cap_px = 0;
            HIP_TRY ( hipMalloc ( &d_pixels, npx * 12 ), kTerraAmdErrNoDevice );
            HIP_TRY ( hipMalloc ( &d_results, npx * 16 ), kTerraAmdErrNoDevice );
            cap_px = npx;
        }
        return 0;
    }
    void release() {
        if ( device >= 0 && hipSetDevice ( device ) == hipSuccess ) {
            if ( stream ) { ( void ) hipStreamSynchronize ( stream ); ( void ) hipStreamDestroy ( stream ); }
            if ( d_pixels ) ( void ) hipFree ( d_pixels );
            if ( d_results ) ( void ) hipFree ( d_results );
        }
        device = -1; stream = nullptr; d_pixels = d_results = nullptr; cap_px = 0;
    }
};
struct Scene {
    TerraSceneOptions opts, new_opts;
    TerraObject* objects = nullptr; size_t objects_pop = 0, objects_cap = 0;
    bool dirty_objects = true, dirty_lights = true, committed = false, device_ok = false;
    uint64_t frame_seed = 0x5EED0001ull;
    std::vector<HostNode> nodes; int max_stack = 1;
    std::vector<HostLight> lights; size_t lights_triangles_count = 0;
    std::vector<uint32_t> first_tri;
    struct Replica {
        int device = -1; DevScene dev {}; void* d_blob = nullptr; unsigned long long* d_counters = nullptr; float* d_env_dist = nullptr;
        Staging staging; float* d_packed = nullptr; size_t packed_floats = 0; float* d_recv = nullptr; size_t recv_floats = 0;
    };
    std::vector<Replica> replicas;
    BlobLayout blob; size_t d_bytes = 0, env_dist_floats = 0;
    std::mutex multi_lock;
    uint64_t gathers = 0, last_gather_bytes = 0;
    std::atomic<uint64_t> launches { 0 }, stat_pixels { 0 }, stat_samples { 0 };
    int uniform_attr_count = -1;
    uint32_t bsdf_kinds = 0;
    int tree_mode = 2;
    int tree_builder = 0;
    TreeChoice tree;
    std::atomic<int> last_call { 0 };
    uint32_t sample_split = 1;
    bool env_lighting = false;
    bool work_counters = false;
    bool env_sampling = false;
    bool env_mis = false;
    int job_order = 1;
    int empty_skip = 1;
    std::atomic<uint32_t> skip_last_blocks { 0 }; std::atomic<int> skip_last_device { -1 };
    int leaf_box_test = 1;
    std::vector<DevLeafBox> leaf_boxes;
    std::atomic<uint32_t> flat_last { 0 };
    int leaf_pair_form = 1;
    std::vector<uint32_t> leaf_pairs;
    std::atomic<uint32_t> pairs_last { 0 };
    int leaf_nearest_first = 1;
    bool pair_per_box = false;
    bool sampler_integration = false;
    std::string commit_error;
    std::atomic<bool> warned_camera { false };
    int test_pad_stack = 0;
    int test_fast_stack_lds = 0;
    float test_shrink_reference_boxes = 0.f;
};

static Scene* S ( HTerraScene h ) { return ( Scene* ) h; }
static const Scene::Replica& primary ( const Scene* s ) { static const Scene::Replica none; return s->replicas.empty() ? none : s->replicas[0]; }
static std::vector<int> devices_of ( const Scene* s ) { std::vector<int> d; for ( const Scene::Replica& r : s->replicas ) d.push_back ( r.device ); return d; }

static std::atomic<bool> g_commit_timing { false };
static bool timing_on() { return g_commit_timing.load ( std::memory_order_relaxed ); }
bool terra_commit_timing_on() { return timing_on(); }
extern "C" void terra_amd_set_commit_timing ( int on ) { g_commit_timing.store ( on != 0, std::memory_order_relaxed ); }
static std::atomic<int> g_build_threads { 0 };
int terra_build_threads() { return g_build_threads.load ( std::memory_order_relaxed ); }
extern "C" int terra_amd_set_build_threads ( int threads ) {
    if ( threads < 0 || threads > 256 ) return fail ( kTerraAmdErrBadArgument, "build threads must be 0 (automatic) .. 256" );
    g_build_threads.store ( threads, std::memory_order_relaxed );
    return 0;
}
static double now_s() { return std::chrono::duration<double> ( std::chrono::steady_clock::now().time_since_epoch() ).count(); }
static void phase ( const char* what, double& t0 ) { if ( !timing_on() ) return; double t = now_s(); fprintf ( stderr, "[terra_amd timing] %-28s %8.2f ms\n", what, ( t - t0 ) * 1e3 ); t0 = t; }

extern "C" HTerraScene terra_scene_create ( void ) {
    Scene* s = new Scene();
    memset ( &s->opts, 0, sizeof s->opts ); memset ( &s->new_opts, 0, sizeof s->new_opts );
    s->objects_cap = 64;
    s->objects = ( TerraObject* ) malloc ( sizeof ( TerraObject ) * s->objects_cap );
    return s;
}
extern "C" TerraObject* terra_scene_add_object ( HTerraScene h, size_t n ) {
    Scene* s = S ( h );
    if ( s->objects_pop == s->objects_cap ) {
        s->objects_cap *= 2;
        s->objects = ( TerraObject* ) realloc ( s->objects, sizeof ( TerraObject ) * s->objects_cap );
    }
    TerraObject* o = &s->objects[s->objects_pop++];
    memset ( o, 0, sizeof *o );
    o->triangles = ( TerraTriangle* ) malloc ( sizeof ( TerraTriangle ) * ( n ? n : 1 ) );
    o->properties = ( TerraTriangleProperties* ) malloc ( sizeof ( TerraTriangleProperties ) * ( n ? n : 1 ) );
    o->triangles_count = n;
    s->dirty_objects = true; s->dirty_lights = true; s->committed = false;
    return o;
}
extern "C" size_t terra_scene_count_objects ( HTerraScene h ) { return S ( h )->objects_pop; }
extern "C" TerraSceneOptions* terra_scene_get_options ( HTerraScene h ) { return &S ( h )->new_opts; }
extern "C" int terra_amd_set_tree_mode ( HTerraScene h, int mode ) {
    if ( mode != 0 && mode != 1 && mode != 2 ) return fail ( kTerraAmdErrBadArgument, "tree mode %d (0 = reference tree, 1 = fast tree, 2 = automatic)", mode );
    Scene* s = S ( h );
    if ( s->tree_mode != mode ) { s->tree_mode = mode; s->dirty_objects = true; s->committed = false; }
    return 0;
}
extern "C" int terra_amd_get_tree_mode ( HTerraScene h ) { return S ( h )->tree_mode; }
extern "C" int terra_amd_set_tree_builder ( HTerraScene h, int builder ) {
    if ( builder != 0 && builder != 1 ) return fail ( kTerraAmdErrBadArgument, "tree builder %d (0 = host binned SAH, 1 = device LBVH)", builder );
    Scene* s = S ( h );
    if ( s->tree_builder != builder ) { s->tree_builder = builder; s->dirty_objects = true; s->committed = false; }
    return 0;
}
extern "C" int terra_amd_get_tree_builder ( HTerraScene h ) { return S ( h )->tree_builder; }
extern "C" int terra_amd_debug_shrink_reference_boxes ( HTerraScene h, float amount ) {
    if ( ! ( amount >= 0.f ) ) return fail ( kTerraAmdErrBadArgument, "shrink amount must be >= 0" );
    Scene* s = S ( h );
    if ( s->test_shrink_reference_boxes != amount ) { s->test_shrink_reference_boxes = amount; s->dirty_objects = true; s->committed = false; }
// ... 236 lines not shown
            const uint32_t t1 = flip ? j : i, t2 = flip ? i : j;
            if ( !fan ( t1, t2 ) ) continue;
            std::vector<uint32_t> rest;
            for ( size_t m = 1; m < left.size(); ++m ) if ( m != k ) rest.push_back ( left[m] );
            out.push_back ( DevLeafPair { { t1, t2 }, { tris[t1].pad, tris[t2].pad } } );
            if ( match_fans ( tris, rest, out ) ) return true;
            out.pop_back();
        }
    }
    return false;
}
static std::vector<uint32_t> leaf_pair_table ( const std::vector<DevLeafBox>& boxes, const std::vector<DevTri>& tris, size_t ntri ) {
    const size_t kPairBoxMax = 8;
    std::vector<uint32_t> none;
    if ( ntri == 0 || ntri > TERRA_LEAF_RANK_MAX || ( ntri & 1 ) || boxes.empty() ) return none;
    std::vector<uint32_t> tri_of_rank ( ntri, 0u );
    for ( size_t i = 0; i < ntri; ++i ) { if ( tris[i].pad >= ntri ) return none; tri_of_rank[tris[i].pad] = ( uint32_t ) i; }
    std::vector<DevLeafPair> pairs; std::vector<uint32_t> box_of_pair;
    for ( size_t b = 0; b < boxes.size(); ++b ) {
        std::vector<uint32_t> left;
        for ( uint32_t r = 0; r < ntri; ++r ) if ( boxes[b].mask >> r & 1u ) left.push_back ( tri_of_rank[r] );
        if ( left.empty() || ( left.size() & 1 ) || left.size() > kPairBoxMax ) return none;
        if ( !match_fans ( tris, left, pairs ) ) return none;
        box_of_pair.resize ( pairs.size(), ( uint32_t ) b );
    }
    if ( pairs.size() * 2 != ntri ) return none;
    std::vector<uint32_t> order ( pairs.size() );
    for ( size_t e = 0; e < order.size(); ++e ) order[e] = ( uint32_t ) e;
    auto low = [&] ( uint32_t e ) { return std::min ( pairs[e].rank[0], pairs[e].rank[1] ); };
    std::sort ( order.begin(), order.end(), [&] ( uint32_t x, uint32_t y ) { return low ( x ) < low ( y ); } );
    std::vector<uint32_t> t ( terra_leaf_pair_words_masks ( ( uint32_t ) ntri ) + boxes.size(), 0u );
    for ( size_t e = 0; e < order.size(); ++e ) {
        const DevLeafPair& p = pairs[order[e]];
        memcpy ( &t[4 * e], &p, sizeof p );
        t[terra_leaf_pair_words_entry_of ( ( uint32_t ) ntri ) + p.tri[0]] = ( uint32_t ) e; t[terra_leaf_pair_words_entry_of ( ( uint32_t ) ntri ) + p.tri[1]] = ( uint32_t ) e;
        t[terra_leaf_pair_words_masks ( ( uint32_t ) ntri ) + box_of_pair[order[e]]] |= 1u << e;
    }
    return t;
}
static bool leaf_pairs_one_per_box ( const std::vector<uint32_t>& table, size_t n_boxes, size_t ntri ) {
    if ( table.empty() || n_boxes * 2 != ntri ) return false;
    for ( size_t k = 0; k < n_boxes; ++k ) if ( table[terra_leaf_pair_words_masks ( ( uint32_t ) ntri ) + k] != 1u << k ) return false;
    return true;
}

struct ReachTables { std::vector<DevReplay> replay; std::vector<uint32_t> leaf_parent, leaf_mask; uint64_t levels = 0, replayed = 0; };
static void build_reach_tables ( const std::vector<DevNode>& nodes, const std::vector<DevTri>& tris, const std::vector<uint32_t>& soup_of_fast, float margin, ReachTables& out ) {
    const size_t nn = nodes.size(), nt = soup_of_fast.size();
    out.replay.assign ( nn ? nn : 1, DevReplay{} );
    std::vector<uint32_t> leaf_parent_of_soup ( tris.size(), 0u );
    for ( size_t k = 0; k < nn; ++k ) for ( int c = 0; c < 2; ++c ) {
        const uint32_t w = nodes[k].child[c];
        if ( w == DEV_CHILD_EMPTY ) continue;
        if ( w & DEV_CHILD_LEAF ) { leaf_parent_of_soup[w & 0x7fffffffu] = ( uint32_t ) k; continue; }
        DevReplay& r = out.replay[w];
        memcpy ( r.bmin, c ? nodes[k].min1 : nodes[k].min0, 12 ); memcpy ( r.bmax, c ? nodes[k].max1 : nodes[k].max0, 12 );
        r.parent = ( uint32_t ) k; r.pad = 0;
    }
    auto contains = [&] ( const DevReplay & outer, const DevReplay & inner ) {
        bool ok = true;
        for ( int a = 0; a < 3; ++a ) ok = ok && outer.bmin[a] <= inner.bmin[a] && outer.bmax[a] >= inner.bmax[a];
        return ok;
    };
    out.leaf_parent.resize ( nt ); out.leaf_mask.resize ( nt );
    for ( size_t k = 0; k < nt; ++k ) {
        const uint32_t soup = soup_of_fast[k];
        out.leaf_parent[k] = leaf_parent_of_soup[soup];
        float lo[3], hi[3];
        for ( int a = 0; a < 3; ++a ) { lo[a] = std::min ( tris[soup].a[a], std::min ( tris[soup].b[a], tris[soup].c[a] ) ); hi[a] = std::max ( tris[soup].a[a], std::max ( tris[soup].b[a], tris[soup].c[a] ) ); }
        uint32_t mask = 0, level = 0, below = 0;
        for ( uint32_t q = leaf_parent_of_soup[soup]; q != 0u; ++level ) {
            const DevReplay& r = out.replay[q];
            bool clear = true;
            for ( int a = 0; a < 3; ++a ) clear = clear && ( lo[a] - r.bmin[a] >= margin ) && ( r.bmax[a] - hi[a] >= margin );
            if ( !clear && level > 0 ) clear = contains ( r, out.replay[below] );
            if ( !clear ) { mask |= 1u << ( level < 31u ? level : 31u ); ++out.replayed; }
            ++out.levels;
            below = q; q = r.parent;
        }
        out.leaf_mask[k] = mask;
    }
}

static std::atomic<bool> g_azimuth_table { true };
extern "C" void terra_amd_set_azimuth_table ( int on ) { g_azimuth_table.store ( on != 0, std::memory_order_relaxed ); }
static const float2* sincos_table_of ( int device ) {
    static std::mutex lock; static const float2* tables[64]; static bool tried[64];
    if ( device < 0 || device >= 64 || !g_azimuth_table.load ( std::memory_order_relaxed ) ) return nullptr;
    std::lock_guard<std::mutex> g ( lock );
    if ( tried[device] ) return tables[device];
    tried[device] = true;
    float2* t = nullptr;
    if ( hipMalloc ( ( void** ) &t, sizeof ( float2 ) << 24 ) != hipSuccess ) { ( void ) hipGetLastError(); return nullptr; }
    if ( terra_fill_sincos24 ( t, nullptr ) != hipSuccess || hipDeviceSynchronize() != hipSuccess ) { ( void ) hipGetLastError(); ( void ) hipFree ( t ); return nullptr; }
    tables[device] = t;
    return t;
}


static std::string format ( const char* fmt, ... ) {
    char buf[512];
    va_list a; va_start ( a, fmt ); vsnprintf ( buf, sizeof buf, fmt, a ); va_end ( a );
    return buf;
}
static bool texture_ok ( const TerraTexture* t ) { return t->pixels && t->width && t->height && ( t->depth == 1 || t->depth == 4 ) && t->components != 0; }
static int check_materials ( const Scene* s, const TerraSceneOptions& opts, std::string& why ) {
    if ( s->objects_pop > 256 ) { why = format ( "%zu objects: the primitive reference holds 8 bits of object index (include/Terra.h:195-198)", s->objects_pop ); return kTerraAmdErrUnsupported; }
    for ( size_t j = 0; j < s->objects_pop; ++j ) {
        const TerraMaterial& m = s->objects[j].material;
        if ( ! ( is_diffuse ( m.bsdf ) || is_phong ( m.bsdf ) || is_ggx ( m.bsdf ) || is_glass ( m.bsdf ) ) ) {
            why = format ( "object %zu: BSDF function pointers are not a terra_bsdf_*_init preset of this library; host callbacks cannot run on the device", j ); return kTerraAmdErrUnsupported;
        }
        if ( m.attributes_count > TERRA_MATERIAL_MAX_ATTRIBUTES ) { why = format ( "object %zu: attributes_count %zu > %d", j, m.attributes_count, TERRA_MATERIAL_MAX_ATTRIBUTES ); return kTerraAmdErrBadArgument; }
        for ( size_t i = 0; i <= m.attributes_count; ++i ) {
            const TerraAttribute& at = i == 0 ? m.emissive : m.attributes[i - 1];
            if ( at.state == nullptr ) continue;
            const std::string what = i == 0 ? "emissive" : format ( "attribute %zu", i - 1 );
            if ( at.eval != terra_texture_sample ) { why = format ( "object %zu %s: attribute callbacks other than terra_texture_sample cannot run on the device (lat-long lookups of a material attribute read past the texcoord in the reference, src/Terra.c:468-471)", j, what.c_str() ); return kTerraAmdErrUnsupported; }
            if ( !texture_ok ( ( const TerraTexture* ) at.state ) ) { why = format ( "object %zu %s: invalid texture", j, what.c_str() ); return kTerraAmdErrBadArgument; }
        }
    }
    const TerraAttribute& env = opts.environment_map;
    if ( s->env_lighting && env.state != nullptr ) {
        if ( env.eval != terra_texture_sample_latlong ) { why = "environment: with environment lighting on, the attribute must be a constant or terra_attribute_init_cubemap (a lat-long lookup by direction)"; return kTerraAmdErrUnsupported; }
        if ( !texture_ok ( ( const TerraTexture* ) env.state ) ) { why = "environment: invalid texture"; return kTerraAmdErrBadArgument; }
    }
    return 0;
}
extern "C" int terra_amd_scene_supported ( HTerraScene h, char* why, size_t capacity ) {
    std::string w;
    int st = check_materials ( S ( h ), S ( h )->new_opts, w );
    if ( st == 0 && terra_amd_device_count() <= 0 ) { w = "no HIP device visible"; st = kTerraAmdErrNoDevice; }
    if ( why && capacity ) snprintf ( why, capacity, "%s", w.c_str() );
    return st;
}

struct Flat {
    size_t ntri = 0;
    std::vector<DevMaterial> mats; std::vector<DevTri> tris; std::vector<DevProps> props; std::vector<DevLight> lights; std::vector<float> tri_area;
    std::vector<DevNode> nodes; std::vector<uint32_t> rank;
    std::vector<DevLeafBox> leaf_boxes;
    std::vector<uint32_t> leaf_pairs;
    std::vector<const TerraTexture*> textures;
    int32_t env_mode = 0, env_tex = -1; float env_color[3] = { 0.f, 0.f, 0.f };
};
static int32_t texture_slot ( std::vector<const TerraTexture*>& textures, const void* state ) {
    auto it = std::find ( textures.begin(), textures.end(), ( const TerraTexture* ) state );
    if ( it == textures.end() ) it = textures.insert ( it, ( const TerraTexture* ) state );
    return ( int32_t ) ( it - textures.begin() );
}
static void flatten_materials ( Scene* s, Flat& f ) {
    const size_t nobj = s->objects_pop;
    f.mats.resize ( nobj ? nobj : 1 );
    memset ( f.mats.data(), 0, f.mats.size() * sizeof ( DevMaterial ) );
    s->bsdf_kinds = 0;
    for ( size_t j = 0; j < nobj; ++j ) {
        const TerraMaterial& m = s->objects[j].material;
        DevMaterial& d = f.mats[j];
        d.bsdf = is_diffuse ( m.bsdf ) ? kDevBsdfDiffuse : is_phong ( m.bsdf ) ? kDevBsdfPhong : is_ggx ( m.bsdf ) ? kDevBsdfGGX : kDevBsdfGlass;
        for ( int a = 0; a <= TERRA_DEV_MAX_ATTR; ++a ) d.tex[a] = -1;
        if ( m.emissive.state ) { d.tex[TERRA_DEV_MAX_ATTR] = texture_slot ( f.textures, m.emissive.state ); d.any_texture = 1; }
        for ( size_t a = 0; a < m.attributes_count; ++a ) {
            if ( m.attributes[a].state ) { d.tex[a] = texture_slot ( f.textures, m.attributes[a].state ); d.any_texture = 1; }
            d.attributes[a][0] = m.attributes[a].value.x; d.attributes[a][1] = m.attributes[a].value.y; d.attributes[a][2] = m.attributes[a].value.z;
        }
        d.attributes_count = ( uint32_t ) m.attributes_count;
        d.ior = m.ior;
        d.first_tri = s->first_tri[j]; d.tri_count = ( uint32_t ) s->objects[j].triangles_count;
// ... 520 lines not shown
    s->launches = 0; s->stat_pixels = 0; s->stat_samples = 0;
    return 0;
}

static uint32_t effective_spp ( const TerraSceneOptions& o ) {
    size_t spp = o.samples_per_pixel;
    if ( o.sampling_method == kTerraSamplingMethodStratified ) {
        size_t cur = o.strata * o.strata;
        while ( spp > cur && cur > 1 ) cur *= cur;
        if ( cur >= spp ) spp = cur;
    }
    return ( uint32_t ) spp;
}

static void fill_camera ( const TerraCamera* cam, size_t fb_w, size_t fb_h, DevRenderParams& p ) {
    TerraFloat3 z = terra_normf3 ( &cam->direction );
    TerraFloat3 xa = terra_crossf3 ( &cam->up, &z ); xa = terra_normf3 ( &xa );
    TerraFloat3 ya = terra_crossf3 ( &z, &xa );
    p.cam_rot[0] = xa.x; p.cam_rot[1] = ya.x; p.cam_rot[2] = z.x;
    p.cam_rot[3] = xa.y; p.cam_rot[4] = ya.y; p.cam_rot[5] = z.y;
    p.cam_rot[6] = xa.z; p.cam_rot[7] = ya.z; p.cam_rot[8] = z.z;
    p.cam_pos[0] = cam->position.x; p.cam_pos[1] = cam->position.y; p.cam_pos[2] = cam->position.z;
    p.tan_half_fov = ( float ) tan ( ( double ) ( ( cam->fov * 0.0174533f ) / 2 ) );
    p.aspect = ( float ) fb_w / ( float ) fb_h;
    p.inv_fb_w = 1.f / ( float ) fb_w; p.inv_fb_h = 1.f / ( float ) fb_h;
}

static int scene_check ( const Scene* s ) {
    if ( !s->committed ) return fail ( kTerraAmdErrNotCommitted, "terra_scene_commit has not run since the scene changed" );
    if ( !s->device_ok ) return fail ( kTerraAmdErrNoDevice, "scene has no device replica: %s", s->commit_error.c_str() );
    return 0;
}
static void apply_stack_hooks ( const Scene* s, DevRenderParams& p ) {
    if ( s->test_fast_stack_lds > 0 && p.lds_mode == 2 ) {
        const uint32_t need = p.stack_depth + p.spill_cap;
        p.stack_depth = need < ( uint32_t ) s->test_fast_stack_lds ? need : ( uint32_t ) s->test_fast_stack_lds; p.spill_cap = need - p.stack_depth;
    }
    if ( s->test_pad_stack > 0 && p.lds_mode != 1 ) {
        p.stack_depth += ( uint32_t ) s->test_pad_stack;
        p.leaf_cap = terra_clamp_leaf_cap ( p.stack_depth, p.leaf_cap, terra_lds_bytes ( p ) - ( size_t ) ( p.stack_depth + p.leaf_cap ) * 1024 );
    }
}
static int fill_params ( Scene* s, const Scene::Replica& r, const TerraCamera* cam, size_t fb_w, size_t fb_h, size_t x, size_t y, size_t w, size_t h,
                         size_t tile, int rank, int world, DevRenderParams& p, const bool* ray_origins_ok = nullptr ) {
    if ( int rc = scene_check ( s ) ) return rc;
    if ( ( !cam && !ray_origins_ok ) || w == 0 || h == 0 || x + w > fb_w || y + h > fb_h ) return fail ( kTerraAmdErrBadArgument, "bad tile rectangle %zu,%zu %zux%zu in %zux%zu", x, y, w, h, fb_w, fb_h );
    if ( tile == 0 || tile % 16 != 0 ) return fail ( kTerraAmdErrBadArgument, "tile_size %zu must be a positive multiple of 16", tile );
    if ( world < 1 || rank < 0 || rank >= world ) return fail ( kTerraAmdErrBadArgument, "bad shard %d/%d", rank, world );
    memset ( &p, 0, sizeof p );
    p.scene = r.dev;
    if ( cam ) fill_camera ( cam, fb_w, fb_h, p );
    p.jitter = s->opts.subpixel_jitter; p.exposure = s->opts.manual_exposure; p.gamma = s->opts.gamma;
    p.fb_w = ( uint32_t ) fb_w; p.fb_h = ( uint32_t ) fb_h;
    p.x = ( uint32_t ) x; p.y = ( uint32_t ) y; p.w = ( uint32_t ) w; p.h = ( uint32_t ) h;
    p.tile_size = ( uint32_t ) tile; p.rank = ( uint32_t ) rank; p.world = ( uint32_t ) world;
    p.st_x = 0; p.st_y = 0; p.st_pitch = ( uint32_t ) fb_w;
    p.spp = effective_spp ( s->opts );
    p.split = 1; p.split_log2 = 0; p.chunk_spp = p.spp; p.partials = nullptr; p.job_blocks = 0; p.job_queue = nullptr;
    p.bounces = ( uint32_t ) s->opts.bounces;
    p.integrator = ( int32_t ) s->opts.integrator; p.tonemap = ( int32_t ) s->opts.tonemapping_operator;
    if ( p.integrator < 0 || p.integrator > 6 ) return fail ( kTerraAmdErrBadArgument, "unknown integrator %d", p.integrator );
    if ( ( p.integrator == kTerraIntegratorDirect || p.integrator == kTerraIntegratorDirectMis || p.integrator == kTerraIntegratorDebugMisWeights ) && s->lights.empty() )
        return fail ( kTerraAmdErrBadArgument, "integrator %d needs at least one emissive object (the reference asserts, src/Terra.c:1617)", p.integrator );
    p.frame_seed = s->frame_seed;
    p.counters = r.d_counters;
    terra_plan_lds ( p );
    const TreeChoice& c = s->tree;
    const bool cam_ok = ray_origins_ok ? *ray_origins_ok : ( c.reach || c.reach_cull ) ? ( fabsf ( p.cam_pos[0] ) <= c.reach_limit && fabsf ( p.cam_pos[1] ) <= c.reach_limit && fabsf ( p.cam_pos[2] ) <= c.reach_limit ) : coords_within_margin ( p.cam_pos, 3 );
    if ( c.use_fast && r.dev.fast_nodes_h && ( s->tree_mode == 1 || cam_ok ) ) terra_plan_fast_tree ( p );
    else if ( ( c.use_fast || c.cull_ok ) && !cam_ok && !ray_origins_ok && !s->warned_camera.exchange ( true ) )
        fprintf ( stderr, "[terra_amd] warning: camera at (%g, %g, %g) lies outside the range (+-%g) for which this scene's traversal shortcut is proven: this call runs the reference "
                  "tree's replica traversal (same image, typically 10-20 x slower on large scenes); terra_amd_traversal_info() reports camera_limit and last_call\n",
                  ( double ) p.cam_pos[0], ( double ) p.cam_pos[1], ( double ) p.cam_pos[2], ( double ) shortcut_limit ( c ) );
    apply_stack_hooks ( s, p );
    p.leaf_cull = ( c.cull_ok && cam_ok && p.lds_mode != 2 ) ? 1u : 0u;
    p.fused_slab = ( p.leaf_cull && !c.reach_cull ) ? 1u : 0u;
    if ( s->leaf_box_test && r.d_blob && terra_leaf_boxes_fit ( p, ( uint32_t ) s->leaf_boxes.size() ) ) {
        p.leaf_boxes = ( const DevLeafBox* ) ( ( const char* ) r.d_blob + s->blob.sec[kSecLeafBoxes].offset ); p.n_leaf_boxes = ( uint32_t ) s->leaf_boxes.size();
    }
    p.leaf_pairs = 0;
    if ( s->leaf_pair_form && r.d_blob && !s->leaf_pairs.empty() && p.lds_mode == 1 && p.leaf_rank ) p.leaf_pairs = ( uint32_t ) ( s->blob.sec[kSecLeafPairs].offset - s->blob.sec[kSecTris].offset );
    if ( p.leaf_pairs && ! ( p.leaf_pairs & 3u ) && p.n_leaf_boxes && s->leaf_nearest_first && s->pair_per_box ) p.leaf_pairs |= TERRA_LEAF_PAIRS_NEAREST;
    if ( p.lds_mode != 1 ) p.scene.sincos24 = nullptr;
    s->last_call.store ( p.lds_mode == 2 ? ( r.dev.reach ? kTerraAmdCallFastTreeReach : kTerraAmdCallFastTree ) : ( p.leaf_cull ? kTerraAmdCallLeafCull : kTerraAmdCallReplica ), std::memory_order_relaxed );
    p.bsdf_kinds = s->bsdf_kinds;
    p.sampler_mode = 0; p.sampler_strata = ( uint32_t ) s->opts.strata;
    if ( s->sampler_integration && s->opts.sampling_method == kTerraSamplingMethodHalton ) p.sampler_mode = 1;
    if ( s->sampler_integration && s->opts.sampling_method == kTerraSamplingMethodStratified && s->opts.strata > 0 ) p.sampler_mode = 2;
    if ( p.sampler_mode ) p.bsdf_kinds |= TERRA_KIND_SAMPLER;
    if ( r.dev.env_nx && ( p.integrator == kTerraIntegratorDirect || p.integrator == kTerraIntegratorDirectMis ) ) p.bsdf_kinds |= TERRA_KIND_SAMPLER;
    else { p.scene.env_nx = 0; p.scene.env_ny = 0; }
    if ( s->env_mis && p.scene.env_nx && p.scene.env_monotone && p.integrator == kTerraIntegratorDirectMis ) p.bsdf_kinds |= TERRA_KIND_ENV_MIS;
    p.count_level = s->work_counters ? 2 : 0;
    return 0;
}

static uint64_t shard_pixels ( const DevRenderParams& p ) {
    uint64_t n = 0;
    const uint32_t tx = ( p.w + p.tile_size - 1 ) / p.tile_size, ty = ( p.h + p.tile_size - 1 ) / p.tile_size;
    for ( uint32_t t = p.rank; t < tx * ty; t += p.world ) {
        uint32_t x0 = ( t % tx ) * p.tile_size, y0 = ( t / tx ) * p.tile_size;
        n += ( uint64_t ) std::min ( p.tile_size, p.w - x0 ) * std::min ( p.tile_size, p.h - y0 );
    }
    return n;
}
static void account_launch ( Scene* s, const DevRenderParams& p ) {
    uint64_t px = shard_pixels ( p );
    s->launches.fetch_add ( 1, std::memory_order_relaxed ); s->stat_pixels.fetch_add ( px, std::memory_order_relaxed ); s->stat_samples.fetch_add ( px * p.spp, std::memory_order_relaxed );
}

struct ThreadSlot;
static void* slot_scratch ( ThreadSlot* slot, size_t bytes );
static uint32_t auto_sample_split ( uint32_t blocks, uint32_t spp, bool ordered ) {
    const uint64_t enough = ordered ? 61440u : 245760u;
    uint32_t split = 1;
    while ( split < 32 && ( uint64_t ) blocks * split < enough && spp / ( split * 2 ) >= 16 ) split *= 2;
    return split;
}
static uint32_t launch_split ( const Scene* s, DevRenderParams& p, uint32_t blocks, bool ray_source = false ) {
    uint32_t split = s->sample_split;
    p.job_blocks = blocks;
    if ( split == 0 ) split = auto_sample_split ( blocks, p.spp, s->job_order && terra_block_order_bytes ( p, s->job_order == 2, ray_source ) != 0 );
    while ( split > 1 && p.spp % split ) split >>= 1;
    if ( split < 1 ) split = 1;
    return split;
}
struct RaySource {
    enum Kind { kCamera = 0, kRays = 1, kLens = 2, kPoints = 3 };
    Kind kind;
    const void* d_records;
    DevLens lens = {};
    DevPointSampling points = {};
    RaySource ( Kind k = kCamera, const void* d = nullptr ) : kind ( k ), d_records ( d ) {}
    bool camera() const { return kind == kCamera; }
};
static int masked_plan_check ( const void* d_mask, const DevRenderParams& p ) {
    if ( d_mask && p.lds_mode != 1 )
        return fail ( kTerraAmdErrUnsupported, "masked rendering needs an LDS-resident launch (TerraAmdTraversalInfo::lds_resident, terra_amd_set_tree_mode other than 1): this scene's kernels key their streams in place and cannot skip pixel blocks" );
    return 0;
}
static int launch_render ( Scene* s, DevRenderParams& p, int device, hipStream_t stream, const RaySource& src, ThreadSlot* slot = nullptr, const uint32_t* d_mask = nullptr ) {
    const uint32_t blocks = terra_render_blocks ( p );
    if ( blocks == 0 ) return 0;
    if ( p.count_level != 0 || p.rand_calls ) { p.leaf_boxes = nullptr; p.n_leaf_boxes = 0; p.leaf_pairs = 0; }
    const bool ray_source = !src.camera();
    const uint32_t split = launch_split ( s, p, blocks, ray_source );
    static thread_local uint64_t pool_kept = 0;
    if ( device < 64 && ! ( pool_kept >> device & 1ull ) ) {
        hipMemPool_t pool;
        if ( hipDeviceGetDefaultMemPool ( &pool, device ) == hipSuccess ) { uint64_t keep = ~0ull; ( void ) hipMemPoolSetAttribute ( pool, hipMemPoolAttrReleaseThreshold, &keep ); }
        pool_kept |= 1ull << device;
    }
    const size_t header = d_mask ? 512 : 256;
    const size_t partial_bytes = ( size_t ) split * blocks * 256 * sizeof ( float4 );
    p.job_blocks = blocks * split;
    const size_t stream_bytes = terra_job_streams_bytes ( p );
    if ( stream_bytes && ( p.fb_w > 65535u || p.fb_h > 65535u ) ) return fail ( kTerraAmdErrBadArgument, "framebuffer of %u x %u: at most 65,535 pixels per side (the job table packs a pixel into 32 bits)", p.fb_w, p.fb_h );
    const size_t spill_bytes = terra_fast_spill_bytes ( p );
    const size_t order_own = s->job_order ? terra_block_order_bytes ( p, s->job_order == 2, ray_source ) : 0;
    if ( d_mask && ray_source ) return fail ( kTerraAmdErrUnsupported, "masked launches: camera launches only" );
    if ( int rc = masked_plan_check ( d_mask, p ) ) return rc;
    const size_t order_bytes = d_mask ? ( ( size_t ) blocks * 3 * sizeof ( uint32_t ) + 255 ) & ~size_t ( 255 ) : order_own;
    const size_t scratch_bytes = header + partial_bytes + stream_bytes + spill_bytes + order_bytes;
    if ( scratch_bytes > ( size_t ) TERRA_SCRATCH_MAX_GB << 30 )
        return fail ( kTerraAmdErrBadArgument, "this launch needs %.1f GB of scratch (%u blocks x sample split %u: 16 B of job sums%s per job), more than the %d GB a launch may take: lower terra_amd_set_sample_split or render the frame in several calls",
                      ( double ) scratch_bytes / ( 1 << 30 ), blocks, split, stream_bytes ? " + 32 B of job streams" : "", TERRA_SCRATCH_MAX_GB );
// ... 1362 lines not shown
extern "C" int terra_amd_unit_math ( int fn, int n, const float* x, const float* y, float* out ) {
    if ( need_device() ) return kTerraAmdErrNoDevice;
    Unit u; auto a = u.in ( x, n ); auto b = u.in ( y ? y : x, n ); auto o = u.out ( out, n );
    return u.finish ( u.ok ? terra_unit_math ( fn, n, a, b, o ) : hipSuccess );
}
extern "C" int terra_amd_unit_exact_div ( int op, const float* a, const float* b, const float* c, uint64_t first, uint64_t count, float denominator, float reciprocal, uint64_t seed,
                                           uint32_t* helper_bits, uint32_t* plain_bits, uint64_t* mismatches, uint32_t* first_bad ) {
    if ( need_device() ) return kTerraAmdErrNoDevice;
    if ( op < 0 || op > 4 || !mismatches || !first_bad ) return fail ( kTerraAmdErrBadArgument, "exact_div unit: op %d, or no place for the mismatch count and records", op );
    const bool explicit_set = a != nullptr;
    if ( explicit_set && ( op == 3 || !helper_bits || !plain_bits || ( ( op == 2 || op == 4 ) && !b ) || ( op == 4 && !c ) || count > ( 1ull << 28 ) ) )
        return fail ( kTerraAmdErrBadArgument, "exact_div unit: the explicit form of op %d needs its input and output arrays (op 3 has none), at most 2^28 elements", op );
    const size_t n = explicit_set ? ( size_t ) count : 0, per = op == 4 ? 3 : 1;
    Unit u;
    const float* da = explicit_set ? u.in ( a, n ) : nullptr; const float* db = explicit_set && ( op == 2 || op == 4 ) ? u.in ( b, n ) : nullptr; const float* dc = explicit_set && op == 4 ? u.in ( c, n ) : nullptr;
    uint32_t* dh = explicit_set ? u.out ( helper_bits, per * n ) : nullptr; uint32_t* dp = explicit_set ? u.out ( plain_bits, per * n ) : nullptr;
    *mismatches = 0;
    unsigned long long* dm = reinterpret_cast<unsigned long long*> ( u.inout ( mismatches, 1 ) ); uint32_t* dr = u.out ( first_bad, 9 * 16 );
    return u.finish ( u.ok ? terra_unit_exact_div ( op, da, db, dc, first, count, denominator, reciprocal, seed, dh, dp, dm, dr ) : hipSuccess );
}
extern "C" int terra_amd_unit_exact_sqrt ( int op, const float* a, const float* b, const float* c, uint64_t first, uint64_t count, uint64_t seed,
                                            uint32_t* helper_bits, uint32_t* plain_bits, uint64_t* mismatches, uint32_t* first_bad ) {
    if ( need_device() ) return kTerraAmdErrNoDevice;
    if ( op < 0 || op > 4 || !mismatches || !first_bad ) return fail ( kTerraAmdErrBadArgument, "exact_sqrt unit: op %d, or no place for the mismatch count and records", op );
    const bool explicit_set = a != nullptr, three = op == 2 || op == 4;
    if ( explicit_set && ( !helper_bits || !plain_bits || ( three && ( !b || !c ) ) || count > ( 1ull << 26 ) ) )
        return fail ( kTerraAmdErrBadArgument, "exact_sqrt unit: the explicit form of op %d needs its input and output arrays, at most 2^26 elements", op );
    const size_t n = explicit_set ? ( size_t ) count : 0, per = op == 2 ? 9 : ( op == 4 ? 3 : 1 );
    Unit u;
    const float* da = explicit_set ? u.in ( a, n ) : nullptr; const float* db = explicit_set && three ? u.in ( b, n ) : nullptr; const float* dc = explicit_set && three ? u.in ( c, n ) : nullptr;
    uint32_t* dh = explicit_set ? u.out ( helper_bits, per * n ) : nullptr; uint32_t* dp = explicit_set ? u.out ( plain_bits, per * n ) : nullptr;
    *mismatches = 0;
    unsigned long long* dm = reinterpret_cast<unsigned long long*> ( u.inout ( mismatches, 1 ) ); uint32_t* dr = u.out ( first_bad, 21 * 16 );
    return u.finish ( u.ok ? terra_unit_exact_sqrt ( op, da, db, dc, first, count, seed, dh, dp, dm, dr ) : hipSuccess );
}

extern "C" int terra_amd_unit_half_outward ( const double* x, int n, int up, uint16_t* out ) {
    if ( n < 0 || ( n && ( !x || !out ) ) ) return fail ( kTerraAmdErrBadArgument, "null array" );
    for ( int i = 0; i < n; ++i ) out[i] = fastbvh::half_outward ( x[i], up != 0 );
    return 0;
}

extern "C" int terra_amd_unit_stratified ( const uint32_t* seeds, int nseeds, int strata, int samples_per_stratum, int n, float* out2 ) {
    if ( need_device() ) return kTerraAmdErrNoDevice;
    if ( nseeds < 0 || n < 0 || strata < 1 || samples_per_stratum < 1 ) return fail ( kTerraAmdErrBadArgument, "stratified sampler: strata and samples per stratum must be positive" );
    if ( ( long long ) n > ( long long ) strata * strata * samples_per_stratum ) return fail ( kTerraAmdErrBadArgument, "stratified sampler: %d pairs requested but strata^2 * samples = %lld (the reference asserts, src/Terra.c:716)", n, ( long long ) strata * strata * samples_per_stratum );
    Unit u; auto ds = u.in ( seeds, nseeds ); auto o = u.out ( out2, ( size_t ) nseeds * n * 2 );
    return u.finish ( u.ok ? terra_unit_stratified ( ds, nseeds, strata, samples_per_stratum, n, o ) : hipSuccess );
}
extern "C" int terra_amd_unit_halton ( int first, int n, float* out2 ) {
    if ( need_device() ) return kTerraAmdErrNoDevice;
    if ( first < 0 || n < 0 ) return fail ( kTerraAmdErrBadArgument, "halton: negative index" );
    Unit u; auto o = u.out ( out2, ( size_t ) n * 2 );
    return u.finish ( u.ok ? terra_unit_halton ( first, n, o ) : hipSuccess );
}
extern "C" int terra_amd_unit_distribution_1d ( const float* f, size_t n, const float* e, int m, float* x, float* pdf, uint32_t* idx, float* cdf_out, float* integral_out ) {
    if ( need_device() ) return kTerraAmdErrNoDevice;
    if ( n == 0 || n > 0x7fffffffu || m < 0 ) return fail ( kTerraAmdErrBadArgument, "distribution: empty table" );
    std::vector<float> cdf_tmp ( cdf_out ? 0 : n ); float integral_tmp = 0.f; uint32_t mono = 0;
    Unit u; auto df = u.in ( f, n ); auto de = u.in ( e, ( size_t ) m );
    auto dc = u.out ( cdf_out ? cdf_out : cdf_tmp.data(), n ); auto di = u.out ( integral_out ? integral_out : &integral_tmp, 1 ); auto dm = u.out ( &mono, 1 );
    auto dx = u.out ( x, ( size_t ) m ); auto dp = u.out ( pdf, ( size_t ) m ); auto dk = u.out ( idx, ( size_t ) m );
    return u.finish ( u.ok ? terra_unit_distribution_1d ( df, ( uint32_t ) n, dc, di, dm, de, m, dx, dp, dk ) : hipSuccess );
}
extern "C" int terra_amd_unit_distribution_2d ( const float* f, size_t nx, size_t ny, const float* e12, int m, float* xy2, float* pdf, float* marginal_cdf_out ) {
    if ( need_device() ) return kTerraAmdErrNoDevice;
    if ( nx == 0 || ny == 0 || nx * ny > 0x7fffffffu || m < 0 ) return fail ( kTerraAmdErrBadArgument, "distribution: empty table" );
    std::vector<float> cdf ( nx * ny ), integrals ( ny + 1 ), mcdf_tmp ( marginal_cdf_out ? 0 : ny ); std::vector<uint32_t> mono ( ny + 1 );
    Unit u; auto df = u.in ( f, nx * ny ); auto de = u.in ( e12, ( size_t ) m * 2 );
    auto dc = u.out ( cdf.data(), nx * ny ); auto di = u.out ( integrals.data(), ny + 1 ); auto dmc = u.out ( marginal_cdf_out ? marginal_cdf_out : mcdf_tmp.data(), ny ); auto dm = u.out ( mono.data(), ny + 1 );
    auto dxy = u.out ( xy2, ( size_t ) m * 2 ); auto dp = u.out ( pdf, ( size_t ) m );
    return u.finish ( u.ok ? terra_unit_distribution_2d ( df, ( uint32_t ) nx, ( uint32_t ) ny, dc, di, dmc, dm, de, m, dxy, dp ) : hipSuccess );
}
extern "C" int terra_amd_unit_distribution_2d_pdf ( const float* f, size_t nx, size_t ny, const float* xy2, int m, float* pdf ) {
    if ( need_device() ) return kTerraAmdErrNoDevice;
    if ( nx == 0 || ny == 0 || nx * ny > 0x7fffffffu || m < 0 ) return fail ( kTerraAmdErrBadArgument, "distribution: empty table" );
    std::vector<float> cdf ( nx * ny ), integrals ( ny + 1 ), mcdf ( ny ); std::vector<uint32_t> mono ( ny + 1 );
    Unit u; auto df = u.in ( f, nx * ny ); auto dxy = u.in ( xy2, ( size_t ) m * 2 );
    auto dc = u.out ( cdf.data(), nx * ny ); auto di = u.out ( integrals.data(), ny + 1 ); auto dmc = u.out ( mcdf.data(), ny ); auto dm = u.out ( mono.data(), ny + 1 );
    auto dp = u.out ( pdf, ( size_t ) m );
    return u.finish ( u.ok ? terra_unit_distribution_2d_pdf ( df, ( uint32_t ) nx, ( uint32_t ) ny, dc, di, dmc, dm, dxy, m, dp ) : hipSuccess );
}

static int unit_texture ( const TerraTexture* t, int n, const float* in, int in_width, float* out3, hipError_t ( *launch ) ( const DevTexture*, int, const float*, float* ) ) {
    if ( need_device() ) return kTerraAmdErrNoDevice;
    if ( !t || !texture_ok ( t ) || n < 0 || ( n && ( !in || !out3 ) ) ) return fail ( kTerraAmdErrBadArgument, "unit texture lookup: invalid texture or null array" );
    BlobLayout L { std::vector<Section> ( kSecTextures + 1 ), std::vector<DevTexture> ( 1 ) };
    layout_textures ( L, { t } );
    void* d_blob = nullptr;
    int rc = new_blob ( L, &d_blob );
    if ( !rc ) {
        Unit u; auto a = u.in ( in, ( size_t ) in_width * n ); auto o = u.out ( out3, 3 * ( size_t ) n );
        rc = u.finish ( u.ok ? launch ( ( const DevTexture* ) ( ( char* ) d_blob + L.sec[kSecTexDesc].offset ), n, a, o ) : hipSuccess );
    }
    ( void ) hipFree ( d_blob );
    return rc;
}
extern "C" int terra_amd_unit_texture_sample ( const TerraTexture* t, int n, const float* uv2, float* out3 ) { return unit_texture ( t, n, uv2, 2, out3, terra_unit_texture_sample ); }
extern "C" int terra_amd_unit_texture_latlong ( const TerraTexture* t, int n, const float* dir3, float* out3 ) { return unit_texture ( t, n, dir3, 3, out3, terra_unit_texture_latlong ); }
```

### terra_amd/csrc/shading_device.h

```cpp
#pragma once
#include "traverse_fast.h"

TD float texture_coord ( float u ) { return u > -1.f ? fminf ( u, 4294967040.f ) : 0.f; }
TD V3 texture_read ( const DevTexture& t, uint32_t x, uint32_t y ) {
    const uint32_t W = t.width, H = t.height;
    if ( t.address_mode == 2 ) { x = x < W - 1 ? x : W - 1; y = y < H - 1 ? y : H - 1; }
    else if ( t.address_mode == 0 ) { x %= W; y %= H; }
    else if ( ( x / W ) % 2 == 0 ) { x %= W; y %= H; }
    else { x = W - ( x % W ); y = H - ( y % H ); x = x < W - 1 ? x : W - 1; y = y < H - 1 ? y : H - 1; }
    const size_t e = ( ( size_t ) y * W + x ) * t.components;
    if ( t.depth == 1 ) {
        const uint8_t* p = reinterpret_cast<const uint8_t*> ( t.data ) + e;
        return v3 ( p[0] / 255.f, p[1] / 255.f, p[2] / 255.f );
    }
    const float* p = reinterpret_cast<const float*> ( t.data ) + e;
    return v3 ( p[0], p[1], p[2] );
}
TD V3 texture_sample ( const DevTexture& t, float u, float v ) {
    u = texture_coord ( u ); v = texture_coord ( v );
    uint32_t ix = ( uint32_t ) u, iy = ( uint32_t ) v;
    if ( t.filter == 0 ) return texture_read ( t, ix, iy );
    if ( t.filter != 1 ) return v3 ( 0, 0, 0 );
    uint32_t x2 = ix + 1 < t.width - 1 ? ix + 1 : t.width - 1, y2 = iy + 1 < t.height - 1 ? iy + 1 : t.height - 1;
    V3 n1 = texture_read ( t, ix, iy ), n2 = texture_read ( t, x2, iy ), n3 = texture_read ( t, ix, y2 ), n4 = texture_read ( t, x2, y2 );
// ... 3 lines not shown
                ( n1.z * wou + n2.z * wu ) * wov + ( n3.z * wou + n4.z * wu ) * wv );
}

#define TERRA_PI_F 3.1416926535f
#define TERRA_INV_PI_F 0x1.45f06p-2f
static_assert ( TERRA_INV_PI_F == 1.f / TERRA_PI_F, "the literal is the compiler's own correctly rounded quotient" );
TD V3 environment_eval ( const DevScene& sc, V3 dir ) {
    if ( sc.env_mode == 1 ) return v3 ( sc.env_color[0], sc.env_color[1], sc.env_color[2] );
    const DevTexture& t = sc.textures[sc.env_tex];
    V3 d = normalize ( dir );
    float theta = tdm_acosf ( d.y );
    float phi = tdm_atan2f ( d.z, d.x ) + TERRA_PI_F;
    uint32_t u = ( uint32_t ) texture_coord ( ( phi / ( 2 * TERRA_PI_F ) ) * ( float ) t.width );
    uint32_t v = ( uint32_t ) texture_coord ( ( theta / TERRA_PI_F ) * ( float ) t.height );
    return texture_read ( t, u, v );
}

struct Surface {
    V3    normal;
    V3    emissive;
    V3    attr[4];
    float ior;
    int   bsdf;
};

template <int MODE, int KINDS>
TD void surface_init ( const Tracer& T, uint32_t ti, V3 point, Surface& sf, uint32_t& object_out, uint32_t& tri_in_object_out, uint32_t& nattr_out ) {
    float4 t0, t1, t2, p0, p1, p2, p3x;
    if ( MODE == 1 ) {
        const float4* lt = reinterpret_cast<const float4*> ( T.l_tris );
        t0 = lt[3 * ti]; t1 = lt[3 * ti + 1]; t2 = lt[3 * ti + 2];
        p0 = T.l_props[4 * ti]; p1 = T.l_props[4 * ti + 1]; p2 = T.l_props[4 * ti + 2]; p3x = T.l_props[4 * ti + 3];
    } else {
        const float4* tris = reinterpret_cast<const float4*> ( MODE >= 2 ? T.sc.fast_tris : T.sc.tris );
        const float4* props = reinterpret_cast<const float4*> ( T.sc.props );
        t0 = tris[3 * ti]; t1 = tris[3 * ti + 1]; t2 = tris[3 * ti + 2];
        uint32_t pi = ti;
        if ( MODE >= 2 ) pi = T.sc.mats[__float_as_uint ( t0.w )].first_tri + __float_as_uint ( t1.w );
        p0 = props[4 * pi]; p1 = props[4 * pi + 1]; p2 = props[4 * pi + 2]; p3x = props[4 * pi + 3];
    }
    uint32_t object = __float_as_uint ( t0.w );
    object_out = object; tri_in_object_out = __float_as_uint ( t1.w );
    float u, v;
    if ( MODE == 1 && T.l_consts ) {
        const float4 c0 = T.l_consts[3 * ti], c1 = T.l_consts[3 * ti + 1], c2 = T.l_consts[3 * ti + 2];
        const V3 e0 = v3 ( c0.x, c0.y, c0.z ), e1 = v3 ( c0.w, c1.x, c1.y ), p = point - v3 ( t0.x, t0.y, t0.z );
        const float d00 = c1.z, d11 = c1.w, d01 = c2.x, div = c2.y;
        const float dp0 = dot ( p, e0 ), dp1 = dot ( p, e1 );
        const float nu = d11 * dp0 - d01 * dp1, nv = d00 * dp1 - d01 * dp0;
        if ( ( int ) __float_as_uint ( c2.w ) & xd_in_range ( nu ) & xd_in_range ( nv ) ) { u = xd_div_short ( nu, div, c2.z ); v = xd_div_short ( nv, div, c2.z ); }
        else { u = nu / div; v = nv / div; }
    } else {
        V3 ta, tb, tc; tri_vertices ( t0, t1, t2, ta, tb, tc );
        V3 e0 = tb - ta, e1 = tc - ta, p = point - ta;
        float d00 = dot ( e0, e0 ), d11 = dot ( e1, e1 ), d01 = dot ( e0, e1 );
        float dp0 = dot ( p, e0 ), dp1 = dot ( p, e1 );
        float div = d00 * d11 - d01 * d01;
        div2_exact ( d11 * dp0 - d01 * dp1, d00 * dp1 - d01 * dp0, div, u, v );
    }
    float w = 1 - u - v;
    V3 na = v3 ( p0.x, p0.y, p0.z ), nb = v3 ( p0.w, p1.x, p1.y ), nc = v3 ( p1.z, p1.w, p2.x );
    sf.normal = normalize ( ( nc * v + nb * u ) + na * w );
    const DevMaterial& m = T.l_mats[object];
    sf.emissive = v3p ( m.emissive );
    #pragma unroll
    for ( int i = 0; i < 4; ++i ) sf.attr[i] = v3p ( m.attributes[i] );
    if ( ( KINDS & TERRA_KIND_TEX ) && m.any_texture ) {
        V3 pa2 = v3 ( p2.y, p2.z, 0.f );
        V3 pb2 = v3 ( p2.w, p3x.x, 0.f );
        V3 pc2 = v3 ( p3x.y, p3x.z, 0.f );
        float tx = ( pc2.x * v + pb2.x * u ) + pa2.x * w;
        float ty = ( pc2.y * v + pb2.y * u ) + pa2.y * w;
        #pragma unroll
        for ( int i = 0; i < 4; ++i ) if ( m.tex[i] >= 0 ) sf.attr[i] = texture_sample ( T.sc.textures[m.tex[i]], tx, ty );
        if ( m.tex[TERRA_DEV_MAX_ATTR] >= 0 ) sf.emissive = texture_sample ( T.sc.textures[m.tex[TERRA_DEV_MAX_ATTR]], tx, ty );
    }
    sf.bsdf = m.bsdf;
    sf.ior = m.ior;
    nattr_out = m.attributes_count;
}

struct RaycastResult { bool hit; uint32_t object, tri_in_object, tri; V3 point; };

struct Azimuth { float sn, cs; bool have; };
struct PathDraws { float e0, e1, e2, e3; Azimuth az; };
template <int COUNT, bool INDEX = false> TD PathDraws path_draw ( const float2* sincos24, Pcg32& rb, Counters& c );

template <int COUNT, int MODE, int KINDS>
TD RaycastResult scene_raycast ( const Tracer& T, const Ray& in, Surface& sf, Counters& c, PathDraws* pre = nullptr, Pcg32* rb = nullptr, bool guarded = false ) {
    Ray r = in;
    r.o = r.o + r.d * 0.001f;
    constexpr bool MASKS = ray_start_masks_for ( COUNT, MODE, KINDS );
    if ( COUNT ) ++c.rays;
    Closest best;
    if constexpr ( MASKS ) { V3 o_perm; const RayStateMasks st = ray_start_masks ( r, o_perm ); best = bvh_traverse_from<COUNT, MODE> ( T, r, st, o_perm, c, __all ( guarded ) != 0 ); }
    else {
    RayState st = ray_state_init ( r );
    if ( MODE >= 2 ) { ClosestRanked b2 = bvh_traverse_fast<COUNT, MODE == 3> ( T, r, st, c ); best.depth = b2.depth; best.tri = b2.tri; }
    else best = bvh_traverse<COUNT, MODE> ( T, r, st, c );
    }
    RaycastResult res; res.hit = best.tri != 0xffffffffu; res.tri = best.tri; res.object = 0; res.tri_in_object = 0;
    res.point = res.hit ? r.o + r.d * best.depth : v3 ( FLT_MAX, FLT_MAX, FLT_MAX );
    if ( res.hit ) {
        uint32_t nattr;
        if ( pre ) *pre = path_draw<COUNT, MASKS> ( T.sc.sincos24, *rb, c );
        surface_init<MODE, KINDS> ( T, best.tri, res.point, sf, res.object, res.tri_in_object, nattr );
        if ( MODE >= 2 ) res.tri = T.sc.mats[res.object].first_tri + res.tri_in_object;
        if ( COUNT ) ++c.hits;
        if ( COUNT == 2 ) c.attr_fetches += nattr + 1;
    }
    return res;
}

template <int COUNT, int MODE, bool MASKS = false>
TD uint32_t scene_raycast_triangle ( const Tracer& T, const Ray& in, Counters& c, uint32_t expected ) {
    Ray r = in;
    r.o = r.o + r.d * 0.001f;
    V3 o_masks = v3 ( 0, 0, 0 );
    const auto st = [&] { if constexpr ( MASKS ) return ray_start_masks ( r, o_masks ); else return ray_state_init ( r ); } ();
    if ( COUNT ) ++c.rays;
    if constexpr ( MODE == 2 && COUNT == 0 ) {
        const V3 o_perm = permuted ( r.o, st );
        ClosestRanked best;
        if ( !fast_expect ( T, st, o_perm, expected, best ) ) return 0xffffffffu;
        int* top = T.stack; uint32_t hand = TERRA_FAST_ROOT_IN_HAND, held = 0u;
        traverse_fast_resume<COUNT> ( T, r, st, o_perm, best, top, hand, held, 0, c, false, true );
        return best.tri == TERRA_TRI_EXPECTED ? expected : 0xffffffffu;
    }
    if constexpr ( MODE == 1 && COUNT == 0 ) {
        const V3 o_perm = MASKS ? o_masks : permuted ( r.o, st );
        float depth;
        if ( !watertight_permuted ( tri_perm_lds ( T.l_tris + 12 * expected, st ), o_perm, st, depth ) ) return 0xffffffffu;
        Closest best; best.depth = __uint_as_float ( __float_as_uint ( depth + 0.f ) + 1u ); best.tri = 0xffffffffu;
        if ( T.pairs ) { best.depth = depth; best.tri = terra_pair_key ( __float_as_uint ( T.l_tris[12 * expected + 11] ), expected ); }
        if ( T.fused && __all ( ray_is_tame ( r ) ) ) traverse_loops<COUNT, MODE, true, true, true> ( T, r, st, o_perm, best, c, expected );
        else if ( __all ( ray_is_regular ( r ) ) ) traverse_loops<COUNT, MODE, true, false, true> ( T, r, st, o_perm, best, c, expected );
        else traverse_loops<COUNT, MODE, false, false, true> ( T, r, st, o_perm, best, c, expected );
        if ( T.pairs ) return best.tri != 0u ? expected : 0xffffffffu;
        return best.tri;
    }
    uint32_t tri;
    if ( MODE >= 2 ) { const ClosestRanked b2 = bvh_traverse_fast<COUNT, MODE == 3> ( T, r, st, c ); tri = b2.tri; }
    else tri = bvh_traverse<COUNT, MODE> ( T, r, st, c ).tri;
    if ( tri == 0xffffffffu ) return tri;
    uint32_t object;
    if ( MODE == 1 ) object = __float_as_uint ( T.l_tris[12 * tri + 3] );
    else {
        const float4* tris = reinterpret_cast<const float4*> ( MODE >= 2 ? T.sc.fast_tris : T.sc.tris );
        const float4 t0 = tris[3 * tri];
        object = __float_as_uint ( t0.w );
        if ( MODE >= 2 ) tri = T.sc.mats[object].first_tri + __float_as_uint ( tris[3 * tri + 1].w );
    }
    if ( COUNT ) ++c.hits;
    if ( COUNT == 2 ) c.attr_fetches += T.l_mats[object].attributes_count + 1;
    return tri;
}

TD V3 surface_origin ( const Surface& sf, V3 p ) { return p + sf.normal * 0.0001f; }
TD Ray surface_ray ( const Surface& sf, V3 p, V3 d ) { return make_ray ( surface_origin ( sf, p ), d ); }


TD Azimuth azimuth_none() { Azimuth a; a.sn = 0.f; a.cs = 1.f; a.have = false; return a; }
TD Azimuth azimuth_fetch ( const float2* tab, float e ) {
    Azimuth a = azimuth_none();
    const float x = e * 16777216.f;
    if ( tab && e >= 0.f && x < 16777216.f ) {
        const uint32_t k = ( uint32_t ) x;
        if ( ( float ) k == x ) { const float2 v = tab[k]; a.cs = v.x; a.sn = v.y; a.have = true; }
    }
    return a;
}
TD Azimuth azimuth_fetch_index ( const float2* tab, uint32_t k ) {
    Azimuth a = azimuth_none();
    if ( tab ) { const float2 v = tab[k]; a.cs = v.x; a.sn = v.y; a.have = true; }
    return a;
}
TD void azimuth_sincos ( const Azimuth& az, float e, float& sn, float& cs ) {
    if ( az.have ) { sn = az.sn; cs = az.cs; }
    else tdm_sincosf_pair ( 2 * TERRA_PI_F * e, sn, cs );
}

TD V3 diffuse_sample ( const Surface& sf, float e1, float e2, const Azimuth& az ) {
    float r = sqrt_exact ( e1 );
    float sn, cs;
    azimuth_sincos ( az, e2, sn, cs );
    float x = r * cs;
    float z = r * sn;
    V3 wi = v3 ( x, sqrt_exact ( sel_max ( 0.f, 1 - e1 ) ), z );
    return normalize ( basis_apply ( make_basis ( sf.normal ), wi ) );
}
TD float diffuse_pdf ( const Surface& sf, V3 wi ) { return div_exact_rk ( sel_max ( 0.f, dot ( sf.normal, wi ) ), TERRA_PI_F, TERRA_INV_PI_F ); }
TD V3 diffuse_eval ( const Surface& sf ) { return sf.attr[0] * ( float ) ( 1. / ( double ) TERRA_PI_F ); }

TD void phong_kd_ks ( const Surface& sf, float& kd, float& ks ) {
    V3 al = sf.attr[1], sp = sf.attr[0];
    float diffuse = sel_max ( al.x + al.y + al.z, ( float ) 1e-4 );
    float specular = sp.x + sp.y + sp.z;
    if ( specular > diffuse ) { kd = 0.5f * diffuse / specular; ks = 1.f - kd; }
    else { ks = 0.5f * specular / diffuse; kd = 1.f - ks; }
}
TD V3 phong_reflect ( const Surface& sf, V3 wo ) { return sf.normal * ( 2.f * dot ( wo, sf.normal ) ) - wo; }

TD V3 phong_sample ( Surface& sf, float e1, float e2, float e3, V3 wo, const Azimuth& az ) {
    float kd, ks; phong_kd_ks ( sf, kd, ks );
    if ( e3 < kd ) { sf.attr[3].x = 1.f; return diffuse_sample ( sf, e1, e2, az ); }
    sf.attr[3].x = -1.f;
    V3 wr = phong_reflect ( sf, wo );
    Basis b = make_basis ( wr );
    float phi = 2 * TERRA_PI_F * e1;
    float theta = tdm_acosf ( tdm_powf ( 1.f - e2, 1.f / ( sf.attr[2].x + 1 ) ) );
    float sin_theta = tdm_sinf ( theta );
    V3 wi = v3 ( sin_theta * tdm_cosf ( phi ), tdm_cosf ( theta ), sin_theta * tdm_sinf ( phi ) );
    return normalize ( basis_apply ( b, wi ) );
}
TD float phong_pdf ( const Surface& sf, V3 wi, V3 wo ) {
    if ( sf.attr[3].x == 1.f ) return diffuse_pdf ( sf, wi );
    V3 wr = phong_reflect ( sf, wo );
    float cos_alpha = dot ( wi, wr );
    float n = sf.attr[2].x;
    return ( n + 1 ) / ( 2 * TERRA_PI_F ) * tdm_powf ( cos_alpha, n );
}
TD V3 phong_eval ( const Surface& sf, V3 wi, V3 wo ) {
    float kd, ks; phong_kd_ks ( sf, kd, ks );
    float n = sf.attr[2].x;
    V3 diffuse_term = sf.attr[1] * ( kd * 1.f / TERRA_PI_F );
    V3 wr = phong_reflect ( sf, wo );
    float cos_alpha = dot ( wi, wr );
    float cos_n_alpha = tdm_powf ( cos_alpha, n );
    V3 specular_term = sf.attr[0] * ( ks * cos_n_alpha * ( n + 2 ) / ( 2 * TERRA_PI_F ) );
    return diffuse_term + specular_term;
}

TD float ggx_D ( float NoH, float alpha2 ) {
    if ( NoH <= 0.f ) return 0.f;
    float NoH2 = NoH * NoH;
    float den = NoH2 * alpha2 + ( 1 - NoH2 );
    return alpha2 / ( TERRA_PI_F * den * den );
}
TD float ggx_G1 ( V3 v, V3 n, V3 h, float alpha2 ) {
    float VoH = dot ( v, h ), VoN = dot ( v, n );
    if ( VoH / VoN <= 0.f ) return 0.f;
    float VoN2 = VoN * VoN;
    float tan2 = ( 1.f - VoN2 ) / VoN2;
    return 2.f / ( sqrt_exact ( 1 + alpha2 * tan2 ) + 1 );
}
TD V3 ggx_sample ( const Surface& sf, float e1, float e2, V3 wo, const Azimuth& az ) {
    float alpha = sf.attr[1].x;
    float t2 = alpha * alpha * e1 / ( 1.f - e1 );
    float cos_t = 1.f / sqrt_exact ( 1.f + t2 );
    float sin_t = sqrt_exact ( sel_max ( 0.f, 1.f - cos_t * cos_t ) );
    float sn, cs;
    azimuth_sincos ( az, e2, sn, cs );
    V3 h = v3 ( sin_t * cs, cos_t, sin_t * sn );
    h = normalize ( basis_apply ( make_basis ( sf.normal ), h ) );
    float HoV = sel_max ( 0.f, dot ( h, wo ) );
    return h * ( 2 * HoV ) - wo;
}
TD float ggx_pdf ( const Surface& sf, V3 wi, V3 wo ) {
    float alpha = sf.attr[1].x;
    V3 h = normalize ( wi + wo );
    float NoH = dot ( sf.normal, h ), HoV = dot ( h, wo );
// ... 73 lines not shown
```

### terra_amd/csrc/unit_kernels.hip

```cpp
#include <hip/hip_runtime.h>
#include "trace_device.h"
#include "sampling_device.h"
#include "kernels.h"

#define UNIT_GRID(n) dim3 ( ( ( n ) + 255 ) / 256 ), dim3 ( 256 )

__global__ void k_pcg ( const uint32_t* seeds, int nseeds, int n, float* out ) {
    int i = blockIdx.x * blockDim.x + threadIdx.x;
    if ( i >= nseeds ) return;
    Pcg32 a; a.state = 0; a.inc = 1;
    trng_next ( a ); a.state += seeds[i]; trng_next ( a );
    for ( int j = 0; j < n; ++j ) out[ ( size_t ) i * n + j] = trng_a_float ( a );
}
hipError_t terra_unit_pcg ( const uint32_t* seeds, int nseeds, int n, float* out ) {
    hipLaunchKernelGGL ( k_pcg, UNIT_GRID ( nseeds ), 0, 0, seeds, nseeds, n, out );
    return hipGetLastError();
}

__global__ void k_stream_keys ( uint64_t seed, const uint64_t* pix, const uint64_t* k, int n, uint64_t* out3 ) {
    int i = blockIdx.x * blockDim.x + threadIdx.x;
    if ( i >= n ) return;
    PixelStreams s = trng_pixel_streams ( seed, pix[i], k[i] );
    out3[3 * i] = s.seedA; out3[3 * i + 1] = s.b.state; out3[3 * i + 2] = s.b.inc;
}
// ... 106 lines not shown
    ClosestRanked b = bvh_traverse_fast<1> ( T, r, s, c );
    bool f = b.tri != 0xffffffffu;
    found[i] = f ? 1 : 0;
    prim[i] = f ? ( sc.fast_tris[b.tri].object | ( sc.fast_tris[b.tri].tri_in_object << 8 ) ) : 0u;
    V3 pt = f ? r.o + r.d * b.depth : v3 ( FLT_MAX, FLT_MAX, FLT_MAX );
    point[3 * i] = pt.x; point[3 * i + 1] = pt.y; point[3 * i + 2] = pt.z;
    nodes_visited[i] = c.nodes;
}
hipError_t terra_unit_bvh_traverse_fast ( const DevScene& sc, int n, const float* o, const float* d, int* found, uint32_t* prim, float* point, uint32_t* nodes_visited ) {
    const uint32_t need = ( uint32_t ) ( sc.fast_max_stack < 1 ? 1 : sc.fast_max_stack ), lds_entries = need < UNIT_FAST_STACK_LDS ? need : UNIT_FAST_STACK_LDS, spill_cap = need - lds_entries;
    uint32_t* spill = nullptr;
    if ( spill_cap ) { const hipError_t e = hipMalloc ( ( void** ) &spill, ( size_t ) ( ( n + 255 ) / 256 ) * 256 * spill_cap * sizeof ( uint32_t ) ); if ( e != hipSuccess ) return e; }
    hipLaunchKernelGGL ( k_bvh_traverse_fast, UNIT_GRID ( n ), ( size_t ) lds_entries * 256 * sizeof ( int ), 0, sc, n, o, d, found, prim, point, nodes_visited, spill, spill_cap, lds_entries );
    hipError_t e = hipGetLastError();
    if ( spill ) { const hipError_t e2 = hipDeviceSynchronize(); if ( e == hipSuccess ) e = e2; ( void ) hipFree ( spill ); }
    return e;
}

__device__ void surface_to_floats ( const DevScene& sc, const Surface& sf, uint32_t object, float* q ) {
    Basis bs = make_basis ( sf.normal );
    q[0] = bs.r0[0]; q[1] = bs.r0[1]; q[2] = bs.r0[2]; q[3] = 0.f;
    q[4] = bs.r1[0]; q[5] = bs.r1[1]; q[6] = bs.r1[2]; q[7] = 0.f;
    q[8] = bs.r2[0]; q[9] = bs.r2[1]; q[10] = bs.r2[2]; q[11] = 0.f;
    q[12] = 0.f; q[13] = 0.f; q[14] = 0.f; q[15] = 1.f;
    q[16] = sf.normal.x; q[17] = sf.normal.y; q[18] = sf.normal.z;
    q[19] = sf.emissive.x; q[20] = sf.emissive.y; q[21] = sf.emissive.z;
    q[22] = sc.mats[object].ior;
    for ( int a = 0; a < 8; ++a ) for ( int k = 0; k < 3; ++k ) q[23 + 3 * a + k] = a < 4 ? pick ( sf.attr[a], k ) : sc.mats[object].attributes[a][k];
}
__global__ __launch_bounds__ ( 256 ) void k_raycast ( DevScene sc, int n, const float* o, const float* d, int* obj, int* tri, float* point, float* surface47 ) {
    extern __shared__ int lds_stack[];
    int i = blockIdx.x * blockDim.x + threadIdx.x;
    if ( i >= n ) return;
    Ray r = make_ray ( v3p ( o + 3 * i ), v3p ( d + 3 * i ) );
    Counters c = counters_zero();
    Surface sf;
    Tracer T = unit_tracer ( sc, lds_stack );
    RaycastResult h = scene_raycast<0, 0, TERRA_KINDS_ALL> ( T, r, sf, c );
    obj[i] = h.hit ? ( int ) h.object : -1;
    tri[i] = h.hit ? ( int ) h.tri_in_object : 0;
    point[3 * i] = h.point.x; point[3 * i + 1] = h.point.y; point[3 * i + 2] = h.point.z;
    float* q = surface47 + 47 * ( size_t ) i;
    if ( h.hit ) surface_to_floats ( sc, sf, h.object, q );
    else for ( int j = 0; j < 47; ++j ) q[j] = 0.f;
}
hipError_t terra_unit_raycast ( const DevScene& sc, int n, const float* o, const float* d, int* obj, int* tri, float* point, float* surface47 ) {
    hipLaunchKernelGGL ( k_raycast, UNIT_GRID ( n ), stack_lds ( sc ), 0, sc, n, o, d, obj, tri, point, surface47 );
    return hipGetLastError();
}

template <int I>
__global__ __launch_bounds__ ( 256 ) void k_trace ( DevScene sc, uint32_t bounces, int n, const float* o, const float* d, const uint64_t* stateB, const uint64_t* incB, float* radiance, uint32_t* rand_calls ) {
    extern __shared__ int lds_stack[];
    int i = blockIdx.x * blockDim.x + threadIdx.x;
    if ( i >= n ) return;
    Ray r = make_ray ( v3p ( o + 3 * i ), v3p ( d + 3 * i ) );
    Pcg32 b; b.state = stateB[i]; b.inc = incB[i];
    Counters c = counters_zero();
    Tracer T = unit_tracer ( sc, lds_stack );
    V3 L = trace_path<I, 2, 0, TERRA_KINDS_ALL> ( T, r, bounces, b, c );
    radiance[3 * i] = L.x; radiance[3 * i + 1] = L.y; radiance[3 * i + 2] = L.z;
    rand_calls[i] = c.rand_calls;
}
hipError_t terra_unit_trace ( const DevScene& sc, int integrator, uint32_t bounces, int n, const float* o, const float* d,
                              const uint64_t* stateB, const uint64_t* incB, float* radiance, uint32_t* rand_calls ) {
#define TRACE_CASE(I) case I: hipLaunchKernelGGL ( k_trace<I>, UNIT_GRID ( n ), stack_lds ( sc ), 0, sc, bounces, n, o, d, stateB, incB, radiance, rand_calls ); break;
    switch ( integrator ) {
        TRACE_CASE ( 0 ) TRACE_CASE ( 1 ) TRACE_CASE ( 2 ) TRACE_CASE ( 3 ) TRACE_CASE ( 4 ) TRACE_CASE ( 5 ) TRACE_CASE ( 6 )
        default: return hipErrorInvalidValue;
    }
#undef TRACE_CASE
    return hipGetLastError();
}

__global__ void k_bsdf ( int kind, int n, float* surfaces47, const float* e3, const float* wo3, float* wi3, float* pdf, float* f3 ) {
    int i = blockIdx.x * blockDim.x + threadIdx.x;
    if ( i >= n ) return;
    float* q = surfaces47 + 47 * ( size_t ) i;
    Surface sf;
    sf.normal = v3p ( q + 16 ); sf.emissive = v3p ( q + 19 );
    for ( int a = 0; a < 4; ++a ) sf.attr[a] = v3p ( q + 23 + 3 * a );
    sf.bsdf = kind; sf.ior = q[22];
    V3 wo = v3p ( wo3 + 3 * i );
    V3 wi = bsdf_sample<TERRA_KINDS_ALL> ( sf, e3[3 * i], e3[3 * i + 1], e3[3 * i + 2], wo, azimuth_none() );
    float p = bsdf_pdf<TERRA_KINDS_ALL> ( sf, wi, wo );
    V3 f = bsdf_eval<TERRA_KINDS_ALL> ( sf, wi, wo );
    wi3[3 * i] = wi.x; wi3[3 * i + 1] = wi.y; wi3[3 * i + 2] = wi.z;
    pdf[i] = p;
    f3[3 * i] = f.x; f3[3 * i + 1] = f.y; f3[3 * i + 2] = f.z;
    q[23 + 6] = sf.attr[2].x; q[23 + 7] = sf.attr[2].y; q[23 + 8] = sf.attr[2].z; q[23 + 9] = sf.attr[3].x;
}
hipError_t terra_unit_bsdf ( int kind, int n, float* surfaces47, const float* e3, const float* wo3, float* wi3, float* pdf, float* f3 ) {
    hipLaunchKernelGGL ( k_bsdf, UNIT_GRID ( n ), 0, 0, kind, n, surfaces47, e3, wo3, wi3, pdf, f3 );
    return hipGetLastError();
}

__global__ void k_camera ( DevRenderParams p, int n, const uint32_t* xy2, const float* r2, float* dirs3 ) {
    int i = blockIdx.x * blockDim.x + threadIdx.x;
    if ( i >= n ) return;
    V3 d = camera_sample ( p, xy2[2 * i], xy2[2 * i + 1], r2[2 * i], r2[2 * i + 1] );
    dirs3[3 * i] = d.x; dirs3[3 * i + 1] = d.y; dirs3[3 * i + 2] = d.z;
}
hipError_t terra_unit_camera ( const DevRenderParams& p, int n, const uint32_t* xy2, const float* r2, float* dirs3 ) {
    hipLaunchKernelGGL ( k_camera, UNIT_GRID ( n ), 0, 0, p, n, xy2, r2, dirs3 );
    return hipGetLastError();
}

__global__ void k_tonemap ( int op, float gamma, int n, float* c3 ) {
    int i = blockIdx.x * blockDim.x + threadIdx.x;
    if ( i >= n ) return;
    V3 c = tonemap ( v3p ( c3 + 3 * i ), op, gamma );
    c3[3 * i] = c.x; c3[3 * i + 1] = c.y; c3[3 * i + 2] = c.z;
}
hipError_t terra_unit_tonemap ( int op, float gamma, int n, float* colors3 ) {
    hipLaunchKernelGGL ( k_tonemap, UNIT_GRID ( n ), 0, 0, op, gamma, n, colors3 );
    return hipGetLastError();
}

__global__ void k_math ( int fn, int n, const float* x, const float* y, float* out ) {
    int i = blockIdx.x * blockDim.x + threadIdx.x;
    if ( i >= n ) return;
    float r;
    switch ( fn ) {
        case 0: r = tdm_sinf ( x[i] ); break;
        case 1: r = tdm_cosf ( x[i] ); break;
        case 2: r = tdm_powf ( x[i], y[i] ); break;
        case 3: r = tdm_acosf ( x[i] ); break;
        default: r = tdm_atan2f ( x[i], y[i] ); break;
    }
    out[i] = r;
}
hipError_t terra_unit_math ( int fn, int n, const float* x, const float* y, float* out ) {
    hipLaunchKernelGGL ( k_math, UNIT_GRID ( n ), 0, 0, fn, n, x, y, out );
    return hipGetLastError();
}

struct XdSink { unsigned long long* mismatches; uint32_t* first_bad; };
TD uint64_t xd_hash ( uint64_t x ) { x += 0x9e3779b97f4a7c15ull; x = ( x ^ ( x >> 30 ) ) * 0xbf58476d1ce4e5b9ull; x = ( x ^ ( x >> 27 ) ) * 0x94d049bb133111ebull; return x ^ ( x >> 31 ); }
TD float xd_float_in ( uint32_t h, uint32_t lo, uint32_t span ) { return __uint_as_float ( ( h & 0x807fffffu ) | ( ( lo + ( ( h >> 23 ) & 0xffu ) % span ) << 23 ) ); }
TD bool xd_same ( float h, float p ) { return __float_as_uint ( h ) == __float_as_uint ( p ) || ( h != h && p != p ); }
TD void xd_check ( const XdSink& s, V3 in, V3 h, V3 p ) {
    if ( xd_same ( h.x, p.x ) && xd_same ( h.y, p.y ) && xd_same ( h.z, p.z ) ) return;
    const unsigned long long slot = atomicAdd ( s.mismatches, 1ull );
    if ( slot < 16ull ) {
        uint32_t* r = s.first_bad + 9 * slot;
        r[0] = __float_as_uint ( in.x ); r[1] = __float_as_uint ( in.y ); r[2] = __float_as_uint ( in.z );
        r[3] = __float_as_uint ( h.x ); r[4] = __float_as_uint ( h.y ); r[5] = __float_as_uint ( h.z );
        r[6] = __float_as_uint ( p.x ); r[7] = __float_as_uint ( p.y ); r[8] = __float_as_uint ( p.z );
    }
}
TD void xd_pair ( const XdSink& s, float x, float d ) { xd_check ( s, v3 ( x, d, 0.f ), v3 ( div_exact_r ( x, d, rcp_exact ( d ) ), 0.f, 0.f ), v3 ( x / d, 0.f, 0.f ) ); }
template <int OP>
__global__ __launch_bounds__ ( 256 ) void k_exact_div ( const float* a, const float* b, const float* c, unsigned long long first, unsigned long long count, float D, float R, unsigned long long seed,
                                                        uint32_t* helper_bits, uint32_t* plain_bits, XdSink s ) {
    const unsigned long long stride = ( unsigned long long ) gridDim.x * blockDim.x;
    for ( unsigned long long i = ( unsigned long long ) blockIdx.x * blockDim.x + threadIdx.x; i < count; i += stride ) {
        const unsigned long long k = first + i;
        const uint64_t h0 = xd_hash ( seed ^ ( k * 0xd1342543de82ef95ull ) ), h1 = xd_hash ( h0 );
        if ( OP == 3 ) {
            const float d = xd_float_in ( ( uint32_t ) h0, 107u, 40u ), q = xd_float_in ( ( uint32_t ) ( h0 >> 32 ), 107u, 40u );
            const double half_ulp = ( double ) __uint_as_float ( ( __float_as_uint ( q ) & 0x7f800000u ) - ( 24u << 23 ) );
            const double target = ( double ) q + ( double ) ( ( int ) ( k % 3ull ) - 1 ) * half_ulp;
            const float x = ( float ) ( ( double ) d * target );
            xd_pair ( s, x, d );
            xd_pair ( s, __uint_as_float ( __float_as_uint ( x ) + 1u ), d );
            xd_pair ( s, __uint_as_float ( __float_as_uint ( x ) - 1u ), d );
            continue;
// ... 127 lines not shown
    int i = blockIdx.x * blockDim.x + threadIdx.x;
    if ( i >= nseeds ) return;
    StratifiedSampler s; stratified_init ( s, seeds[i], strata, samples );
    for ( int j = 0; j < n; ++j ) { float a, b; stratified_next_pair ( s, a, b ); out2[ ( ( size_t ) i * n + j ) * 2] = a; out2[ ( ( size_t ) i * n + j ) * 2 + 1] = b; }
}
hipError_t terra_unit_stratified ( const uint32_t* seeds, int nseeds, int strata, int samples, int n, float* out2 ) {
    hipLaunchKernelGGL ( k_stratified, UNIT_GRID ( nseeds ), 0, 0, seeds, nseeds, strata, samples, n, out2 );
    return hipGetLastError();
}
__global__ void k_halton ( int first, int n, float* out2 ) {
    int i = blockIdx.x * blockDim.x + threadIdx.x;
    if ( i >= n ) return;
    float a, b; halton_pair ( first + i, a, b );
    out2[2 * i] = a; out2[2 * i + 1] = b;
}
hipError_t terra_unit_halton ( int first, int n, float* out2 ) {
    hipLaunchKernelGGL ( k_halton, UNIT_GRID ( n ), 0, 0, first, n, out2 );
    return hipGetLastError();
}
__global__ void k_dist_rows ( const float* f, uint32_t nx, uint32_t ny, float* cdf, float* integrals, uint32_t* monotone ) {
    uint32_t r = blockIdx.x * blockDim.x + threadIdx.x;
    if ( r >= ny ) return;
    integrals[r] = distribution_row_init ( f + ( size_t ) nx * r, nx, cdf + ( size_t ) nx * r, monotone + r );
}
__global__ void k_dist_marginal ( uint32_t ny, float* integrals, float* mcdf, uint32_t* monotone ) {
    if ( blockIdx.x || threadIdx.x ) return;
    integrals[ny] = distribution_row_init ( integrals, ny, mcdf, monotone + ny );
}
__global__ void k_dist_sample_1d ( const float* f, const float* cdf, uint32_t n, const float* integral, const uint32_t* monotone, const float* e, int m, float* x, float* pdf, uint32_t* idx ) {
    int i = blockIdx.x * blockDim.x + threadIdx.x;
    if ( i >= m ) return;
    DevDistribution1D d = { f, cdf, n, integral[0], monotone[0] };
    float p = 0.f; uint32_t k = 0;
    x[i] = distribution_sample ( d, e[i], &p, &k );
    pdf[i] = p; idx[i] = k;
}
__global__ void k_dist_sample_2d ( const float* f, const float* cdf, uint32_t nx, uint32_t ny, const float* integrals, const float* mcdf, const uint32_t* monotone, const float* e12, int m, float* xy2, float* pdf ) {
    int i = blockIdx.x * blockDim.x + threadIdx.x;
    if ( i >= m ) return;
    DevDistribution1D marginal = { integrals, mcdf, ny, integrals[ny], monotone[ny] };
    float p0 = 0.f, p1 = 0.f; uint32_t row = 0;
    const float s1 = distribution_sample ( marginal, e12[2 * i], &p0, &row );
    if ( s1 == FLT_MAX ) { xy2[2 * i] = xy2[2 * i + 1] = FLT_MAX; pdf[i] = 0.f; return; }
    DevDistribution1D cond = { f + ( size_t ) nx * row, cdf + ( size_t ) nx * row, nx, integrals[row], monotone[row] };
    const float s2 = distribution_sample ( cond, e12[2 * i + 1], &p1, nullptr );
    xy2[2 * i] = s1; xy2[2 * i + 1] = s2; pdf[i] = p0 * p1;
}
hipError_t terra_unit_distribution_1d ( const float* f, uint32_t n, float* cdf, float* integral, uint32_t* monotone, const float* e, int m, float* x, float* pdf, uint32_t* idx ) {
    hipLaunchKernelGGL ( k_dist_rows, dim3 ( 1 ), dim3 ( 64 ), 0, 0, f, n, 1u, cdf, integral, monotone );
    if ( m > 0 ) hipLaunchKernelGGL ( k_dist_sample_1d, UNIT_GRID ( m ), 0, 0, f, cdf, n, integral, monotone, e, m, x, pdf, idx );
    return hipGetLastError();
}
hipError_t terra_unit_distribution_2d ( const float* f, uint32_t nx, uint32_t ny, float* cdf, float* integrals, float* mcdf, uint32_t* monotone, const float* e12, int m, float* xy2, float* pdf ) {
    hipLaunchKernelGGL ( k_dist_rows, UNIT_GRID ( ny ), 0, 0, f, nx, ny, cdf, integrals, monotone );
    hipLaunchKernelGGL ( k_dist_marginal, dim3 ( 1 ), dim3 ( 64 ), 0, 0, ny, integrals, mcdf, monotone );
    if ( m > 0 ) hipLaunchKernelGGL ( k_dist_sample_2d, UNIT_GRID ( m ), 0, 0, f, cdf, nx, ny, integrals, mcdf, monotone, e12, m, xy2, pdf );
    return hipGetLastError();
}
__global__ void k_dist_pdf_2d ( const float* f, uint32_t nx, uint32_t ny, const float* integrals, const float* xy2, int m, float* pdf ) {
    int i = blockIdx.x * blockDim.x + threadIdx.x;
    if ( i >= m ) return;
    const float v = xy2[2 * i], u = xy2[2 * i + 1];
    uint32_t row = v > 0.f ? ( uint32_t ) ( v * ( float ) ny ) : 0u, col = u > 0.f ? ( uint32_t ) ( u * ( float ) nx ) : 0u;
    row = row < ny - 1u ? row : ny - 1u; col = col < nx - 1u ? col : nx - 1u;
    pdf[i] = distribution_2d_prob ( f, integrals, nx, integrals[ny], row, col );
}
hipError_t terra_unit_distribution_2d_pdf ( const float* f, uint32_t nx, uint32_t ny, float* cdf, float* integrals, float* mcdf, uint32_t* monotone, const float* xy2, int m, float* pdf ) {
    hipLaunchKernelGGL ( k_dist_rows, UNIT_GRID ( ny ), 0, 0, f, nx, ny, cdf, integrals, monotone );
    hipLaunchKernelGGL ( k_dist_marginal, dim3 ( 1 ), dim3 ( 64 ), 0, 0, ny, integrals, mcdf, monotone );
    if ( m > 0 ) hipLaunchKernelGGL ( k_dist_pdf_2d, UNIT_GRID ( m ), 0, 0, f, nx, ny, integrals, xy2, m, pdf );
    return hipGetLastError();
}

__global__ __launch_bounds__ ( 256 ) void terra_sincos24_kernel ( float2* table ) {
    const uint32_t k = blockIdx.x * 256u + threadIdx.x;
    float sn, cs;
    tdm_sincosf_pair ( 2 * TERRA_PI_F * ( ( float ) k * 0x1p-24f ), sn, cs );
    table[k] = make_float2 ( cs, sn );
}
hipError_t terra_fill_sincos24 ( float2* table, hipStream_t stream ) {
    hipLaunchKernelGGL ( terra_sincos24_kernel, dim3 ( ( 1u << 24 ) / 256u ), dim3 ( 256 ), 0, stream, table );
    return hipGetLastError();
}
```

### terra_amd/runtime.py

```python
from __future__ import annotations

import ctypes as C
from pathlib import Path
from typing import Optional, Tuple

import numpy as np

from . import api, scenes

HERE = Path(__file__).resolve().parent
import os as _os
LIB_PATH = Path(_os.environ.get("TERRA_AMD_LIB", HERE / "libterra_amd.so"))

_lib: Optional[api.TerraLib] = None


class TerraAmdError(RuntimeError):
    pass


class Stats(C.Structure):
    _fields_ = [(n, C.c_uint64) for n in ("rays", "nodes", "box_tests", "tri_tests", "hits", "samples", "rand_calls", "attr_fetches", "pixels", "launches", "tri_culled")]

    def as_dict(self):
        return {n: int(getattr(self, n)) for n, _ in self._fields_}


class TraversalInfo(C.Structure):
    _fields_ = [("tree_mode", C.c_int), ("fast_tree", C.c_int), ("fast_tree_built_on_device", C.c_int), ("leaf_cull", C.c_int), ("lds_resident", C.c_int), ("max_coordinate", C.c_float), ("max_coordinate_allowed", C.c_float), ("note", C.c_char * 256),
                ("last_call", C.c_int), ("camera_limit", C.c_float)]


CALL_TRAVERSAL = {0: "none", 1: "reference tree, replica traversal", 2: "reference tree + leaf-box cull", 3: "fast tree", 4: "fast tree + reachability replay"}


class SceneInfo(C.Structure):
    _fields_ = [("triangles", C.c_uint32), ("nodes", C.c_uint32), ("objects", C.c_uint32), ("lights", C.c_uint32),
                ("lights_triangles_count", C.c_uint32), ("max_stack", C.c_int32), ("device_bytes", C.c_uint64)]


_CAM = C.POINTER(api.TerraCamera)
_SZ = C.c_size_t
_EXTRA = {
    "terra_amd_last_error": (C.c_char_p, []),
    "terra_amd_clear_error": (None, []),
    "terra_amd_first_error": (C.c_int, [C.c_char_p, C.c_size_t]),
    "terra_amd_clear_first_error": (None, []),
    "terra_amd_thread_staging_bytes": (C.c_size_t, []),
    "terra_amd_device_count": (C.c_int, []),
    "terra_amd_set_device": (C.c_int, [C.c_int]),
    "terra_amd_get_device": (C.c_int, []),
    "terra_amd_set_frame_seed": (None, [C.c_void_p, C.c_uint64]),
    "terra_amd_debug_shrink_reference_boxes": (C.c_int, [C.c_void_p, C.c_float]),
    "terra_amd_debug_pad_stack": (C.c_int, [C.c_void_p, C.c_int]),
    "terra_amd_debug_fast_stack_lds": (C.c_int, [C.c_void_p, C.c_int]),
    "terra_amd_scene_supported": (C.c_int, [C.c_void_p, C.c_char_p, C.c_size_t]),
    "terra_amd_init": (C.c_int, []),
    "terra_amd_set_commit_timing": (None, [C.c_int]),
    "terra_amd_set_build_threads": (C.c_int, [C.c_int]),
    "terra_amd_set_azimuth_table": (None, [C.c_int]),
    "terra_amd_set_devices": (C.c_int, [C.POINTER(C.c_int), C.c_int]),
    "terra_amd_get_devices": (C.c_int, [C.POINTER(C.c_int), C.c_int]),
    "terra_amd_shard_owner": (C.c_int, [C.c_size_t, C.c_int]),
    "terra_amd_render_multi": (C.c_int, [C.POINTER(api.TerraCamera), C.c_void_p, C.POINTER(api.TerraFramebuffer)] + [C.c_size_t] * 5),
    "terra_amd_multi_info": (C.c_int, [C.c_void_p, C.c_void_p]),
    "terra_amd_debug_replicas_share_device": (C.c_int, [C.c_int]),
    "terra_amd_set_work_counters": (C.c_int, [C.c_void_p, C.c_int]),
    "terra_amd_get_work_counters": (C.c_int, [C.c_void_p]),
    "terra_amd_set_sampler_integration": (C.c_int, [C.c_void_p, C.c_int]),
    "terra_amd_get_sampler_integration": (C.c_int, [C.c_void_p]),
    "terra_amd_set_environment_sampling": (C.c_int, [C.c_void_p, C.c_int]),
    "terra_amd_get_environment_sampling": (C.c_int, [C.c_void_p]),
    "terra_amd_set_environment_mis": (C.c_int, [C.c_void_p, C.c_int]),
    "terra_amd_get_environment_mis": (C.c_int, [C.c_void_p]),
    "terra_amd_unit_distribution_2d_pdf": (C.c_int, [C.c_void_p, C.c_size_t, C.c_size_t, C.c_void_p, C.c_int, C.c_void_p]),
    "terra_amd_get_frame_seed": (C.c_uint64, [C.c_void_p]),
    "terra_amd_set_tree_mode": (C.c_int, [C.c_void_p, C.c_int]),
    "terra_amd_get_tree_mode": (C.c_int, [C.c_void_p]),
    "terra_amd_traversal_info": (C.c_int, [C.c_void_p, C.POINTER(TraversalInfo)]),
    "terra_amd_set_tree_builder": (C.c_int, [C.c_void_p, C.c_int]),
    "terra_amd_get_tree_builder": (C.c_int, [C.c_void_p]),
    "terra_amd_set_job_order": (C.c_int, [C.c_void_p, C.c_int]),
    "terra_amd_get_job_order": (C.c_int, [C.c_void_p]),
    "terra_amd_set_empty_skip": (C.c_int, [C.c_void_p, C.c_int]),
    "terra_amd_get_empty_skip": (C.c_int, [C.c_void_p]),
    "terra_amd_empty_skip_info": (C.c_int, [C.c_void_p, C.POINTER(C.c_uint32)]),
    "terra_amd_set_leaf_box_test": (C.c_int, [C.c_void_p, C.c_int]),
    "terra_amd_get_leaf_box_test": (C.c_int, [C.c_void_p]),
    "terra_amd_leaf_box_info": (C.c_int, [C.c_void_p, C.POINTER(C.c_uint32)]),
    "terra_amd_scene_leaf_boxes": (C.c_int, [C.c_void_p, C.c_void_p, C.c_int]),
    "terra_amd_set_leaf_pairs": (C.c_int, [C.c_void_p, C.c_int]),
    "terra_amd_get_leaf_pairs": (C.c_int, [C.c_void_p]),
    "terra_amd_leaf_pair_info": (C.c_int, [C.c_void_p, C.POINTER(C.c_uint32)]),
    "terra_amd_set_leaf_nearest_first": (C.c_int, [C.c_void_p, C.c_int]),
    "terra_amd_get_leaf_nearest_first": (C.c_int, [C.c_void_p]),
    "terra_amd_scene_leaf_pairs": (C.c_int, [C.c_void_p, C.c_void_p, C.c_int]),
    "terra_amd_scene_leaf_pair_masks": (C.c_int, [C.c_void_p, C.c_void_p, C.c_int]),
    "terra_amd_leaf_pair_offsets": (C.c_int, [C.c_uint32, C.c_void_p, C.c_void_p]),
    "terra_amd_empty_proof": (C.c_int, [C.c_void_p, C.c_void_p, C.c_float, C.c_float, C.c_float] + [C.c_uint32] * 6 + [C.c_void_p, C.c_size_t]),
    "terra_amd_set_sample_split": (C.c_int, [C.c_void_p, C.c_int]),
    "terra_amd_get_sample_split": (C.c_int, [C.c_void_p]),
    "terra_amd_auto_sample_split": (C.c_int, [C.c_size_t, C.c_size_t, C.c_size_t, C.c_int, C.c_size_t, C.c_int]),
    "terra_amd_set_environment_lighting": (C.c_int, [C.c_void_p, C.c_int]),
    "terra_amd_get_environment_lighting": (C.c_int, [C.c_void_p]),
    "terra_amd_get_stats": (C.c_int, [C.c_void_p, C.POINTER(Stats)]),
    "terra_amd_reset_stats": (C.c_int, [C.c_void_p]),
    "terra_amd_scene_info": (C.c_int, [C.c_void_p, C.POINTER(SceneInfo)]),
    "terra_amd_scene_bvh_nodes": (C.c_int, [C.c_void_p, C.c_void_p, C.c_int]),
    "terra_amd_scene_leaf_ranks": (C.c_int, [C.c_void_p, C.c_void_p, C.c_int]),
    "terra_amd_render_device": (C.c_int, [_CAM, C.c_void_p, C.c_void_p, C.c_void_p] + [_SZ] * 6 + [C.c_void_p, C.c_void_p]),
    "terra_amd_render_device_sharded": (C.c_int, [_CAM, C.c_void_p, C.c_void_p, C.c_void_p] + [_SZ] * 7 + [C.c_int, C.c_int, C.c_void_p, C.c_void_p]),
    "terra_amd_shard_tile_count": (C.c_int, [_SZ, _SZ, _SZ, C.c_int, C.c_int]),
    "terra_amd_shard_packed_bytes": (_SZ, [_SZ, _SZ, _SZ, C.c_int]),
    "terra_amd_pack_tiles": (C.c_int, [C.c_void_p, C.c_void_p] + [_SZ] * 7 + [C.c_int, C.c_int, C.c_void_p, C.c_void_p]),
    "terra_amd_unpack_tiles": (C.c_int, [C.c_void_p, C.c_void_p] + [_SZ] * 7 + [C.c_int, C.c_int, C.c_void_p, C.c_void_p]),
    "terra_amd_synchronize": (C.c_int, [C.c_void_p]),
    "terra_amd_time_render_device": (C.c_int, [_CAM, C.c_void_p, C.c_void_p, C.c_void_p] + [_SZ] * 6 + [C.c_int, C.c_void_p, C.POINTER(C.c_float)]),
    "terra_amd_render_aov_device": (C.c_int, [_CAM, C.c_void_p, C.c_void_p] + [_SZ] * 6 + [C.c_void_p]),
    "terra_amd_render_aov": (C.c_int, [_CAM, C.c_void_p, C.c_void_p] + [_SZ] * 6),
    "terra_amd_denoise_device": (C.c_int, [C.c_void_p, C.c_void_p, C.c_void_p] + [_SZ] * 6 + [C.c_int, C.c_void_p, C.c_void_p, C.c_void_p]),
    "terra_amd_denoise": (C.c_int, [C.c_void_p, C.POINTER(api.TerraFramebuffer), C.c_void_p] + [_SZ] * 4 + [C.c_int, C.c_void_p, C.c_void_p]),
    "terra_amd_accumulate_moments_device": (C.c_int, [C.c_void_p, C.c_void_p, C.c_void_p] + [_SZ] * 6 + [C.c_void_p]),
    "terra_amd_accumulate_moments": (C.c_int, [C.c_void_p, C.POINTER(api.TerraFramebuffer), C.c_void_p] + [_SZ] * 4),
    "terra_amd_tile_error_device": (C.c_int, [C.c_void_p, C.c_void_p] + [_SZ] * 7 + [C.c_void_p, C.c_void_p]),
    "terra_amd_tile_error": (C.c_int, [C.POINTER(api.TerraFramebuffer), C.c_void_p] + [_SZ] * 5 + [C.c_void_p]),
    "terra_amd_denoise_variance_device": (C.c_int, [C.c_void_p, C.c_void_p, C.c_void_p, C.c_void_p] + [_SZ] * 6 + [C.c_int, C.c_void_p, C.c_void_p, C.c_void_p]),
    "terra_amd_denoise_variance": (C.c_int, [C.c_void_p, C.POINTER(api.TerraFramebuffer), C.c_void_p, C.c_void_p] + [_SZ] * 4 + [C.c_int, C.c_void_p, C.c_void_p]),
    "terra_amd_render_adaptive_device": (C.c_int, [_CAM, C.c_void_p, C.c_void_p, C.c_void_p, C.c_void_p, C.c_void_p] + [_SZ] * 6 +
                                         [C.POINTER(api.TerraAmdAdaptiveOptions), C.POINTER(api.TerraAmdAdaptiveReport), C.c_void_p]),
    "terra_amd_render_adaptive": (C.c_int, [_CAM, C.c_void_p, C.POINTER(api.TerraFramebuffer), C.c_void_p, C.c_void_p] + [_SZ] * 4 +
                                  [C.POINTER(api.TerraAmdAdaptiveOptions), C.POINTER(api.TerraAmdAdaptiveReport)]),
    "terra_amd_reproject_device": (C.c_int, [C.c_void_p, _CAM, _CAM] + [C.c_void_p] * 6 + [_SZ] * 6 + [C.POINTER(api.TerraAmdTemporalOptions), C.c_void_p]),
    "terra_amd_reproject": (C.c_int, [C.c_void_p, _CAM, _CAM, C.POINTER(api.TerraFramebuffer)] + [C.c_void_p] * 5 + [_SZ] * 4 + [C.POINTER(api.TerraAmdTemporalOptions)]),
    **api.RAY_QUERY_SIGNATURES,
    **api.RAY_SOURCE_SIGNATURES,
    **api.MASKED_SIGNATURES,
    **api.LENS_SIGNATURES,
    **api.POINT_SIGNATURES,
    **api.BAKE_SIGNATURES,
    **api.PROBE_SIGNATURES,
    **api.EXACT_SQRT_SIGNATURES,
}


def load(need_torch: bool = True) -> api.TerraLib:
    global _lib
    if _lib is not None:
        return _lib
    if need_torch:
        import torch
    if not LIB_PATH.exists():
        raise TerraAmdError(f"{LIB_PATH} is missing: run `python -m terra_amd.build` (there is no CPU fallback)")
    lib = api.TerraLib(LIB_PATH, "terra_")
    if lib.missing:
        raise TerraAmdError(f"{LIB_PATH} lacks Terra.h entry points: {lib.missing}")
    for name, (res, args) in _EXTRA.items():
        if lib.has(name):
            setattr(lib, name[len("terra_amd_"):] if name.startswith("terra_amd_") else name, lib.fn(name, res, args))
# ... 626 lines not shown
```

Before: 36870 Msamples/s.

## Compute 24-bit azimuth sincos inline instead of reading a 16M-entry table

Adds tdm_azimuth24, which computes the sine and cosine of a 24-bit azimuth index with integer quadrant thresholds and a double-precision polynomial. It is meant to match the precomputed table bit for bit, and a unit kernel is added to count mismatches. The table is now off by default, so BSDF sampling computes the value in registers instead of doing a random global load from a 128 MB table. Path draws always use the integer-index route. This trades a likely cache-missing memory access for FP64 arithmetic, which is relatively fast on MI355X, and it relies on the inline routine exactly reproducing the table.

```diff
diff --git a/include/terra_amd.h b/include/terra_amd.h
--- a/include/terra_amd.h
+++ b/include/terra_amd.h
@@ -26,6 +26,8 @@
 void terra_amd_set_commit_timing ( int on );
 int  terra_amd_set_build_threads ( int threads );
 void terra_amd_set_azimuth_table ( int on );
+int  terra_amd_get_azimuth_table ( void );
+int  terra_amd_azimuth_table_info ( HTerraScene scene );
 
 int  terra_amd_device_count ( void );
 int  terra_amd_set_device ( int device );
@@ -475,6 +477,7 @@
 int terra_amd_unit_distribution_1d ( const float* f, size_t n, const float* e, int m, float* x, float* pdf, uint32_t* idx, float* cdf_out, float* integral_out );
 int terra_amd_unit_distribution_2d ( const float* f, size_t nx, size_t ny, const float* e12, int m, float* xy2, float* pdf, float* marginal_cdf_out );
 int terra_amd_unit_distribution_2d_pdf ( const float* f, size_t nx, size_t ny, const float* xy2, int m, float* pdf );
+int terra_amd_unit_azimuth24 ( uint32_t* mismatches );
 int terra_amd_unit_texture_sample ( const TerraTexture* texture, int n, const float* uv2, float* out3 );
 int terra_amd_unit_texture_latlong ( const TerraTexture* texture, int n, const float* dir3, float* out3 );
 
diff --git a/terra_amd/csrc/dev_math.h b/terra_amd/csrc/dev_math.h
--- a/terra_amd/csrc/dev_math.h
+++ b/terra_amd/csrc/dev_math.h
@@ -68,6 +68,34 @@
 }
 TDM_FN float tdm_sinf ( float y ) { return tdm_sincosf ( y, 0 ); }
 TDM_FN float tdm_cosf ( float y ) { return tdm_sincosf ( y, 1 ); }
+
+#define TDM_AZIMUTH_SCALE ( 2 * 3.1416926535f )
+TDM_FN uint32_t tdm_azimuth24_quadrant ( uint32_t k ) {
+    return ( uint32_t ) ( k >= 0x1fffbeu ) + ( uint32_t ) ( k >= 0x5fff38u ) + ( uint32_t ) ( k >= 0x9ffeb3u ) + ( uint32_t ) ( k >= 0xdffe2eu );
+}
+TDM_FN void tdm_azimuth24 ( uint32_t k, float& sn, float& cs ) {
+    const float y = TDM_AZIMUTH_SCALE * ( ( float ) k * 0x1p-24f );
+    const uint32_t n = tdm_azimuth24_quadrant ( k );
+    const double x = ( double ) y - ( double ) ( int32_t ) n * 0x1.921FB54442D18p0;
+    const double x2 = x * x;
+    const double S1 = -0x1.555545995a603p-3, S2 = 0x1.1107605230bc4p-7, S3 = -0x1.994eb3774cf24p-13;
+    const double x3 = x * x2;
+    const double t = S2 + x2 * S3;
+    const double x7 = x3 * x2;
+    const double s = x + x3 * S1;
+    const float sine = ( float ) ( s + x7 * t );
+    const double C0 = 0x1p0, C1 = -0x1.ffffffd0c621cp-2, C2 = 0x1.55553e1068f19p-5, C3 = -0x1.6c087e89a359dp-10, C4 = 0x1.99343027bf8c3p-16;
+    const double x4 = x2 * x2;
+    const double t2 = C3 + x2 * C4;
+    const double t1 = C0 + x2 * C1;
+    const double x6 = x4 * x2;
+    const double c = t1 + x4 * C2;
+    const float cosine = ( float ) ( c + x6 * t2 );
+    const bool odd = ( n & 1u ) != 0;
+    sn = tdm_float ( tdm_bits ( odd ? cosine : sine ) ^ ( ( n & 2u ) << 30 ) );
+    cs = tdm_float ( tdm_bits ( odd ? sine : cosine ) ^ ( ( ( n + 1u ) & 2u ) << 30 ) );
+    if ( k < 652u ) { sn = y; cs = 1.0f; }
+}
 
 TDM_FN uint64_t tdm_bits64 ( double f ) { return __builtin_bit_cast ( uint64_t, f ); }
 TDM_FN double   tdm_double ( uint64_t u ) { return __builtin_bit_cast ( double, u ); }
diff --git a/terra_amd/csrc/integrators_device.h b/terra_amd/csrc/integrators_device.h
--- a/terra_amd/csrc/integrators_device.h
+++ b/terra_amd/csrc/integrators_device.h
@@ -152,8 +152,8 @@
     const DevScene& sc = T.sc;
     V3 Lo = v3 ( 0, 0, 0 );
     if ( bounce == 0 && dot ( wo, sf.normal ) > 0 ) Lo = Lo + sf.emissive;
-    float e1 = randf ( rb, c, COUNT ), e2 = randf ( rb, c, COUNT ), e3 = randf ( rb, c, COUNT );
-    V3 bsdf_dir = bsdf_sample<KINDS> ( sf, e1, e2, e3, wo, azimuth_fetch ( sc.sincos24, e2 ) );
+    const float e1 = randf ( rb, c, COUNT ); const uint32_t k2 = randf_bits ( rb, c, COUNT ); const float e2 = trng_b_from_bits ( k2 ), e3 = randf ( rb, c, COUNT );
+    V3 bsdf_dir = bsdf_sample<KINDS> ( sf, e1, e2, e3, wo, azimuth_fetch_index ( azimuth_table<MODE> ( sc ), k2 ) );
     LightSample ls = draw_light_sample<COUNT, MODE> ( sc, rb, c, &T );
     MisPending m;
     m.a_hid = Lo; m.a_vis = Lo; m.expected = ls.tri; m.p = p; m.light_object = ls.light_object; m.t_before = throughput;
@@ -208,8 +208,8 @@
     V3 Lo = v3 ( 0, 0, 0 );
     if ( DEBUG_WEIGHTS ) { if ( bounce != 0 ) return Lo; }
     else if ( bounce == 0 && dot ( wo, sf.normal ) > 0 ) Lo = Lo + sf.emissive;
-    float e1 = randf ( rb, c, COUNT ), e2 = randf ( rb, c, COUNT ), e3 = randf ( rb, c, COUNT );
-    V3 bsdf_dir = bsdf_sample<KINDS> ( sf, e1, e2, e3, wo, azimuth_fetch ( sc.sincos24, e2 ) );
+    const float e1 = randf ( rb, c, COUNT ); const uint32_t k2 = randf_bits ( rb, c, COUNT ); const float e2 = trng_b_from_bits ( k2 ), e3 = randf ( rb, c, COUNT );
+    V3 bsdf_dir = bsdf_sample<KINDS> ( sf, e1, e2, e3, wo, azimuth_fetch_index ( azimuth_table<MODE> ( sc ), k2 ) );
     LightSample ls = draw_light_sample<COUNT, MODE> ( sc, rb, c, &T );
     {
         V3 p_to_light = ls.pos - p;
@@ -318,21 +318,15 @@
     }
 }
 
-template <int COUNT, bool INDEX>
+template <int COUNT>
 TD PathDraws path_draw ( const float2* sincos24, Pcg32& rb, Counters& c ) {
     PathDraws d;
-    if constexpr ( INDEX ) {
-        d.e0 = randf ( rb, c, COUNT );
-        const uint32_t k1 = randf_bits ( rb, c, COUNT );
-        d.e1 = trng_b_from_bits ( k1 );
-        d.e2 = randf ( rb, c, COUNT );
-        d.az = azimuth_fetch_index ( sincos24, k1 );
-        d.e3 = randf ( rb, c, COUNT );
-    } else {
-        d.e0 = randf ( rb, c, COUNT ); d.e1 = randf ( rb, c, COUNT ); d.e2 = randf ( rb, c, COUNT );
-        d.az = azimuth_fetch ( sincos24, d.e1 );
-        d.e3 = randf ( rb, c, COUNT );
-    }
+    d.e0 = randf ( rb, c, COUNT );
+    const uint32_t k1 = randf_bits ( rb, c, COUNT );
+    d.e1 = trng_b_from_bits ( k1 );
+    d.e2 = randf ( rb, c, COUNT );
+    d.az = azimuth_fetch_index ( sincos24, k1 );
+    d.e3 = randf ( rb, c, COUNT );
     return d;
 }
 template <int KINDS>
diff --git a/terra_amd/csrc/kernels.h b/terra_amd/csrc/kernels.h
--- a/terra_amd/csrc/kernels.h
+++ b/terra_amd/csrc/kernels.h
@@ -77,6 +77,7 @@
 hipError_t terra_launch_sh_irradiance ( const void* sh, uint32_t probes, const DevProbeGrid& grid, const void* points, const int* index, uint32_t n, void* out, hipStream_t stream );
 
 hipError_t terra_fill_sincos24 ( float2* table, hipStream_t stream );
+hipError_t terra_unit_azimuth24 ( const float2* table, float2* computed, uint32_t* mismatches );
 
 hipError_t terra_unit_pcg ( const uint32_t* seeds, int nseeds, int n, float* out );
 hipError_t terra_unit_stream_keys ( uint64_t frame_seed, const uint64_t* pix, const uint64_t* k, int n, uint64_t* out3 );
diff --git a/terra_amd/csrc/render_kernels.hip b/terra_amd/csrc/render_kernels.hip
--- a/terra_amd/csrc/render_kernels.hip
+++ b/terra_amd/csrc/render_kernels.hip
@@ -595,7 +595,7 @@
                 if ( have_ray ) {
                     if ( lt.best.tri != 0xffffffffu ) {
                         Surface sf;
-                        PathDraws pd = path_draw<COUNT> ( T.sc.sincos24, rs.b, c );
+                        PathDraws pd = path_draw<COUNT> ( azimuth_table<MODE> ( T.sc ), rs.b, c );
                         if constexpr ( ( KINDS & TERRA_KIND_SAMPLER ) != 0 ) path_apply_sampler ( pd, sp, bounce );
                         V3 point = shade_surface<COUNT, MODE, KINDS> ( T, ray, lt.best, sf, c );
                         V3 wo = neg ( ray.d ), wi;
@@ -667,7 +667,7 @@
                 if constexpr ( SPLIT_DIRECT ) {
                     Ray shadow_ray;
                     const DirectPending pend = direct_prepare<COUNT, KINDS, MODE> ( T, sf, h.point, wo, throughput, bounce, rs.b, c, shadow_ray );
-                    pd = path_draw<COUNT, ray_start_masks_for ( COUNT, MODE, KINDS )> ( T.sc.sincos24, rs.b, c );
+                    pd = path_draw<COUNT> ( azimuth_table<MODE> ( T.sc ), rs.b, c );
                     end = !path_continue<KINDS> ( sf, wo, throughput, bounce, p.bounces, pd, wi );
                     if ( !end ) { ro = surface_origin ( sf, h.point ); rd = wi; }
                     const uint32_t tri = scene_raycast_triangle<COUNT, MODE, ray_start_masks_for ( COUNT, MODE, KINDS )> ( T, shadow_ray, c, pend.expected );
@@ -685,7 +685,7 @@
                     lo_add ( mis_finish_b<MODE> ( T, pend, lo_a, hb.hit, hb.object, hb.tri, hb.point, lsf, b_d ) );
                 } else {
                 lo_add ( integrate<INTEGRATOR, COUNT, MODE, KINDS> ( T, ray, sf, h.point, wo, throughput, bounce, rs.b, c ) );
-                if ( !pre_draw ) pd = path_draw<COUNT, ray_start_masks_for ( COUNT, MODE, KINDS )> ( T.sc.sincos24, rs.b, c );
+                if ( !pre_draw ) pd = path_draw<COUNT> ( azimuth_table<MODE> ( T.sc ), rs.b, c );
                 if constexpr ( ( KINDS & TERRA_KIND_SAMPLER ) != 0 ) path_apply_sampler ( pd, sp, bounce );
                 end = !path_continue<KINDS> ( sf, wo, throughput, bounce, p.bounces, pd, wi );
                 if ( !end ) { ro = surface_origin ( sf, h.point ); rd = wi; }
diff --git a/terra_amd/csrc/scene_host.cpp b/terra_amd/csrc/scene_host.cpp
--- a/terra_amd/csrc/scene_host.cpp
+++ b/terra_amd/csrc/scene_host.cpp
@@ -311,6 +311,7 @@
     int tree_builder = 0;
     TreeChoice tree;
     std::atomic<int> last_call { 0 };
+    std::atomic<int> last_azimuth_table { 0 };
     uint32_t sample_split = 1;
     bool env_lighting = false;
     bool work_counters = false;
@@ -713,8 +714,10 @@
     }
 }
 
-static std::atomic<bool> g_azimuth_table { true };
+static std::atomic<bool> g_azimuth_table { false };
 extern "C" void terra_amd_set_azimuth_table ( int on ) { g_azimuth_table.store ( on != 0, std::memory_order_relaxed ); }
+extern "C" int terra_amd_get_azimuth_table ( void ) { return g_azimuth_table.load ( std::memory_order_relaxed ) ? 1 : 0; }
+extern "C" int terra_amd_azimuth_table_info ( HTerraScene h ) { return S ( h )->last_azimuth_table.load ( std::memory_order_relaxed ); }
 static const float2* sincos_table_of ( int device ) {
     static std::mutex lock; static const float2* tables[64]; static bool tried[64];
     if ( device < 0 || device >= 64 || !g_azimuth_table.load ( std::memory_order_relaxed ) ) return nullptr;
@@ -1401,6 +1404,7 @@
     if ( s->leaf_pair_form && r.d_blob && !s->leaf_pairs.empty() && p.lds_mode == 1 && p.leaf_rank ) p.leaf_pairs = ( uint32_t ) ( s->blob.sec[kSecLeafPairs].offset - s->blob.sec[kSecTris].offset );
     if ( p.leaf_pairs && ! ( p.leaf_pairs & 3u ) && p.n_leaf_boxes && s->leaf_nearest_first && s->pair_per_box ) p.leaf_pairs |= TERRA_LEAF_PAIRS_NEAREST;
     if ( p.lds_mode != 1 ) p.scene.sincos24 = nullptr;
+    s->last_azimuth_table.store ( p.scene.sincos24 ? 1 : 0, std::memory_order_relaxed );
     s->last_call.store ( p.lds_mode == 2 ? ( r.dev.reach ? kTerraAmdCallFastTreeReach : kTerraAmdCallFastTree ) : ( p.leaf_cull ? kTerraAmdCallLeafCull : kTerraAmdCallReplica ), std::memory_order_relaxed );
     p.bsdf_kinds = s->bsdf_kinds;
     p.sampler_mode = 0; p.sampler_strata = ( uint32_t ) s->opts.strata;
@@ -2929,6 +2933,23 @@
     return u.finish ( u.ok ? terra_unit_distribution_2d_pdf ( df, ( uint32_t ) nx, ( uint32_t ) ny, dc, di, dmc, dm, dxy, m, dp ) : hipSuccess );
 }
 
+extern "C" int terra_amd_unit_azimuth24 ( uint32_t* mismatches ) {
+    if ( need_device() ) return kTerraAmdErrNoDevice;
+    if ( !mismatches ) return fail ( kTerraAmdErrBadArgument, "unit azimuth: null count" );
+    float2* table = nullptr; float2* computed = nullptr; uint32_t* count = nullptr;
+    hipError_t e = hipMalloc ( ( void** ) &table, sizeof ( float2 ) << 24 );
+    if ( e == hipSuccess ) e = hipMalloc ( ( void** ) &computed, sizeof ( float2 ) << 24 );
+    if ( e == hipSuccess ) e = hipMalloc ( ( void** ) &count, sizeof ( uint32_t ) );
+    if ( e == hipSuccess ) e = hipMemset ( count, 0, sizeof ( uint32_t ) );
+    if ( e == hipSuccess ) e = terra_fill_sincos24 ( table, nullptr );
+    if ( e == hipSuccess ) e = terra_unit_azimuth24 ( table, computed, count );
+    if ( e == hipSuccess ) e = hipDeviceSynchronize();
+    if ( e == hipSuccess ) e = hipMemcpy ( mismatches, count, sizeof ( uint32_t ), hipMemcpyDeviceToHost );
+    ( void ) hipFree ( table ); ( void ) hipFree ( computed ); ( void ) hipFree ( count );
+    if ( e != hipSuccess ) { ( void ) hipGetLastError(); return fail ( kTerraAmdErrLaunch, "unit azimuth: %s", hipGetErrorString ( e ) ); }
+    return 0;
+}
+
 static int unit_texture ( const TerraTexture* t, int n, const float* in, int in_width, float* out3, hipError_t ( *launch ) ( const DevTexture*, int, const float*, float* ) ) {
     if ( need_device() ) return kTerraAmdErrNoDevice;
     if ( !t || !texture_ok ( t ) || n < 0 || ( n && ( !in || !out3 ) ) ) return fail ( kTerraAmdErrBadArgument, "unit texture lookup: invalid texture or null array" );
diff --git a/terra_amd/csrc/shading_device.h b/terra_amd/csrc/shading_device.h
--- a/terra_amd/csrc/shading_device.h
+++ b/terra_amd/csrc/shading_device.h
@@ -109,9 +109,10 @@
 
 struct RaycastResult { bool hit; uint32_t object, tri_in_object, tri; V3 point; };
 
-struct Azimuth { float sn, cs; bool have; };
+struct Azimuth { float sn, cs; uint32_t k; int kind; };
 struct PathDraws { float e0, e1, e2, e3; Azimuth az; };
-template <int COUNT, bool INDEX = false> TD PathDraws path_draw ( const float2* sincos24, Pcg32& rb, Counters& c );
+template <int MODE> TD const float2* azimuth_table ( const DevScene& sc ) { return MODE == 1 ? sc.sincos24 : nullptr; }
+template <int COUNT> TD PathDraws path_draw ( const float2* sincos24, Pcg32& rb, Counters& c );
 
 template <int COUNT, int MODE, int KINDS>
 TD RaycastResult scene_raycast ( const Tracer& T, const Ray& in, Surface& sf, Counters& c, PathDraws* pre = nullptr, Pcg32* rb = nullptr, bool guarded = false ) {
@@ -130,7 +131,7 @@
     res.point = res.hit ? r.o + r.d * best.depth : v3 ( FLT_MAX, FLT_MAX, FLT_MAX );
     if ( res.hit ) {
         uint32_t nattr;
-        if ( pre ) *pre = path_draw<COUNT, MASKS> ( T.sc.sincos24, *rb, c );
+        if ( pre ) *pre = path_draw<COUNT> ( azimuth_table<MODE> ( T.sc ), *rb, c );
         surface_init<MODE, KINDS> ( T, best.tri, res.point, sf, res.object, res.tri_in_object, nattr );
         if ( MODE >= 2 ) res.tri = T.sc.mats[res.object].first_tri + res.tri_in_object;
         if ( COUNT ) ++c.hits;
@@ -187,23 +188,25 @@
 TD Ray surface_ray ( const Surface& sf, V3 p, V3 d ) { return make_ray ( surface_origin ( sf, p ), d ); }
 
 
-TD Azimuth azimuth_none() { Azimuth a; a.sn = 0.f; a.cs = 1.f; a.have = false; return a; }
-TD Azimuth azimuth_fetch ( const float2* tab, float e ) {
-    Azimuth a = azimuth_none();
-    const float x = e * 16777216.f;
-    if ( tab && e >= 0.f && x < 16777216.f ) {
-        const uint32_t k = ( uint32_t ) x;
-        if ( ( float ) k == x ) { const float2 v = tab[k]; a.cs = v.x; a.sn = v.y; a.have = true; }
-    }
-    return a;
-}
+static_assert ( TDM_AZIMUTH_SCALE == 2 * TERRA_PI_F, "tdm_azimuth24's scale is the samplers' 2 * terra_PI" );
+TD Azimuth azimuth_none() { Azimuth a; a.sn = 0.f; a.cs = 1.f; a.k = 0u; a.kind = 0; return a; }
 TD Azimuth azimuth_fetch_index ( const float2* tab, uint32_t k ) {
     Azimuth a = azimuth_none();
-    if ( tab ) { const float2 v = tab[k]; a.cs = v.x; a.sn = v.y; a.have = true; }
+    if ( tab ) { const float2 v = tab[k]; a.cs = v.x; a.sn = v.y; a.kind = 1; }
+    else { a.k = k; a.kind = 2; }
     return a;
 }
+TD Azimuth azimuth_fetch ( const float2* tab, float e ) {
+    const float x = e * 16777216.f;
+    if ( e >= 0.f && x < 16777216.f ) {
+        const uint32_t k = ( uint32_t ) x;
+        if ( ( float ) k == x ) return azimuth_fetch_index ( tab, k );
+    }
+    return azimuth_none();
+}
 TD void azimuth_sincos ( const Azimuth& az, float e, float& sn, float& cs ) {
-    if ( az.have ) { sn = az.sn; cs = az.cs; }
+    if ( az.kind == 1 ) { sn = az.sn; cs = az.cs; }
+    else if ( az.kind == 2 ) tdm_azimuth24 ( az.k, sn, cs );
     else tdm_sincosf_pair ( 2 * TERRA_PI_F * e, sn, cs );
 }
 
diff --git a/terra_amd/csrc/unit_kernels.hip b/terra_amd/csrc/unit_kernels.hip
--- a/terra_amd/csrc/unit_kernels.hip
+++ b/terra_amd/csrc/unit_kernels.hip
@@ -212,7 +212,7 @@
     for ( int a = 0; a < 4; ++a ) sf.attr[a] = v3p ( q + 23 + 3 * a );
     sf.bsdf = kind; sf.ior = q[22];
     V3 wo = v3p ( wo3 + 3 * i );
-    V3 wi = bsdf_sample<TERRA_KINDS_ALL> ( sf, e3[3 * i], e3[3 * i + 1], e3[3 * i + 2], wo, azimuth_none() );
+    V3 wi = bsdf_sample<TERRA_KINDS_ALL> ( sf, e3[3 * i], e3[3 * i + 1], e3[3 * i + 2], wo, azimuth_fetch ( nullptr, e3[3 * i + 1] ) );
     float p = bsdf_pdf<TERRA_KINDS_ALL> ( sf, wi, wo );
     V3 f = bsdf_eval<TERRA_KINDS_ALL> ( sf, wi, wo );
     wi3[3 * i] = wi.x; wi3[3 * i + 1] = wi.y; wi3[3 * i + 2] = wi.z;
@@ -506,3 +506,15 @@
     hipLaunchKernelGGL ( terra_sincos24_kernel, dim3 ( ( 1u << 24 ) / 256u ), dim3 ( 256 ), 0, stream, table );
     return hipGetLastError();
 }
+__global__ __launch_bounds__ ( 256 ) void k_azimuth24 ( const float2* table, float2* computed, uint32_t* mismatches ) {
+    const uint32_t k = blockIdx.x * 256u + threadIdx.x;
+    float sn, cs;
+    tdm_azimuth24 ( k, sn, cs );
+    computed[k] = make_float2 ( cs, sn );
+    const float2 t = table[k];
+    if ( __float_as_uint ( t.x ) != __float_as_uint ( cs ) || __float_as_uint ( t.y ) != __float_as_uint ( sn ) ) atomicAdd ( mismatches, 1u );
+}
+hipError_t terra_unit_azimuth24 ( const float2* table, float2* computed, uint32_t* mismatches ) {
+    hipLaunchKernelGGL ( k_azimuth24, dim3 ( ( 1u << 24 ) / 256u ), dim3 ( 256 ), 0, 0, table, computed, mismatches );
+    return hipGetLastError();
+}
diff --git a/terra_amd/runtime.py b/terra_amd/runtime.py
--- a/terra_amd/runtime.py
+++ b/terra_amd/runtime.py
@@ -59,6 +59,8 @@
     "terra_amd_set_commit_timing": (None, [C.c_int]),
     "terra_amd_set_build_threads": (C.c_int, [C.c_int]),
     "terra_amd_set_azimuth_table": (None, [C.c_int]),
+    "terra_amd_get_azimuth_table": (C.c_int, []),
+    "terra_amd_azimuth_table_info": (C.c_int, [C.c_void_p]),
     "terra_amd_set_devices": (C.c_int, [C.POINTER(C.c_int), C.c_int]),
     "terra_amd_get_devices": (C.c_int, [C.POINTER(C.c_int), C.c_int]),
     "terra_amd_shard_owner": (C.c_int, [C.c_size_t, C.c_int]),
@@ -74,6 +76,7 @@
     "terra_amd_set_environment_mis": (C.c_int, [C.c_void_p, C.c_int]),
     "terra_amd_get_environment_mis": (C.c_int, [C.c_void_p]),
     "terra_amd_unit_distribution_2d_pdf": (C.c_int, [C.c_void_p, C.c_size_t, C.c_size_t, C.c_void_p, C.c_int, C.c_void_p]),
+    "terra_amd_unit_azimuth24": (C.c_int, [C.POINTER(C.c_uint32)]),
     "terra_amd_get_frame_seed": (C.c_uint64, [C.c_void_p]),
     "terra_amd_set_tree_mode": (C.c_int, [C.c_void_p, C.c_int]),
     "terra_amd_get_tree_mode": (C.c_int, [C.c_void_p]),
```

After: 37560 Msamples/s (median of 6 runs). +1.9%, better.
